# brudfors/UniRes

Hardware: AMD Instinct MI355X
Metric: cg_iters_per_sec (higher is better)
Workload: dtype f32; 1 GPU; cfg3_256c3_thick6z; channels=3, cg_iters_per_channel=20, cg_mode=fixed-iteration (tol=0), identity preconditioner, step=one y-update of one subject: C x (RHS + 20 CG iterations), channel_streams=True, channel_streams_setting=auto, parallelism=one subject per GPU, no data-path collective

## Files before the change

include/unires_hip.h:

```cpp
#ifndef UNIRES_HIP_H
#define UNIRES_HIP_H

#include <stdint.h>

#ifdef __cplusplus
extern "C" {
#endif

#define UNIRES_HIP_ABI_VERSION 1
#define UNIRES_MAX_TAPS 32

enum unires_status {
  UNIRES_OK = 0,
  UNIRES_ERR_NULL = 1,
  UNIRES_ERR_DIM = 2,
  UNIRES_ERR_ARG = 3,
  UNIRES_ERR_HIP = 4,
  UNIRES_ERR_ALLOC = 5,
  UNIRES_ERR_UNSUPPORTED = 6
};

enum unires_operator { UNIRES_OP_A = 0, UNIRES_OP_AT = 1, UNIRES_OP_ATA = 2 };

enum unires_regime {
  UNIRES_REGIME_IDENTITY = 0,
  UNIRES_REGIME_DENOISE = 1,
  UNIRES_REGIME_SUPERRES = 2
};

enum unires_cg_stop {
  UNIRES_STOP_RESIDUAL = 0,
  UNIRES_STOP_MAXGAIN = 1,
  UNIRES_STOP_MAXGAIN_RECURRED = 2,
  UNIRES_STOP_MAXGAIN_GUARDED = 3
};

enum unires_precond {
  UNIRES_PRECOND_IDENTITY = 0,
  UNIRES_PRECOND_JACOBI = 1,
  UNIRES_PRECOND_FFT = 2
};

const char *unires_last_error(void);
int unires_abi_version(void);


int unires_pull3d_affine(const float *src, const int32_t sdim[3], const float M[12], float *dst,
                         const int32_t gdim[3], float fov_tol, void *stream);

int unires_warp_label(const float *label, const int32_t ldim[3], const float M[12], float *dst,
                      const int32_t gdim[3], float fov_tol, void *stream);

int unires_pull3d_nearest(const float *src, const int32_t sdim[3], const float M[12], float *dst,
                          const int32_t gdim[3], float fov_tol, void *stream);

int unires_noise_hist(int32_t n_obs, const float *const *ptrs, const int64_t *sizes, const int32_t *ct,
                      uint32_t *counts, float *range, void *stream);

int unires_noise_fit(int32_t n_obs, const uint32_t *counts, const float *range, int32_t max_iter,
                     double *out, void *stream);

int unires_coreg_quantise(int32_t n_obs, const float *const *ptrs, const int64_t *sizes,
                          uint8_t *const *outs, uint32_t *counts, float *params, void *stream);

typedef struct {
  const uint8_t *G;
  const uint8_t *F;
  int32_t dim_g[3];
  int32_t dim_f[3];
  float M[12];
  float step[3];
} unires_coreg_job_t;

int unires_coreg_hist(int32_t n_jobs, const unires_coreg_job_t *jobs, uint64_t *hist, void *stream);

int unires_coreg_cost(int32_t n, const uint64_t *hist, int32_t cost_fun, double fwhm, double *work,
                      double *cost, void *stream);

int unires_pull_grad3d_affine(const float *src, const int32_t sdim[3], const float M[12],
                              float *dst3, const int32_t gdim[3], float fov_tol, void *stream);

int unires_push3d_affine(const float *src, const int32_t gdim[3], const float M[12], float *dst,
                         const int32_t ddim[3], float alpha, float fov_tol, int accumulate,
                         void *stream);

int unires_conv_down3d(const float *src, const int32_t sdim[3], const float *const taps[3],
                       const int32_t ntaps[3], const int32_t stride[3], float *dst,
                       const int32_t ddim[3], float scl, int32_t scl_dim, void *stream);

int unires_conv_up3d(const float *src, const int32_t sdim[3], const float *const taps[3],
                     const int32_t ntaps[3], const int32_t stride[3], float *dst,
                     const int32_t ddim[3], float scl, int32_t scl_dim, void *stream);

int unires_grad_fwd_zero(const float *src, const int32_t dim[3], const float vx[3], float *dst3,
                         void *stream);

int unires_div_fwd_zero(const float *src3, const int32_t dim[3], const float vx[3], float *dst,
                        void *stream);

int unires_dtd(const float *src, const int32_t dim[3], const float vx[3], float a, float c,
               float *dst, void *stream);

#define UNIRES_DIFF_FORWARD 0
#define UNIRES_DIFF_BACKWARD 1
#define UNIRES_DIFF_CENTRAL 2

int unires_grad_which(const float *src, const int32_t dim[3], const float vx[3], int32_t which,
                      float *dst3, void *stream);
int unires_div_which(const float *src3, const int32_t dim[3], const float vx[3], int32_t which,
                     float *dst, void *stream);
int unires_dtd_which(const float *src, const int32_t dim[3], const float vx[3], int32_t which, float a,
                     float c, float *dst, void *stream);


typedef struct unires_repeat {
  int32_t dim_x[3];
  int32_t dim_g[3];
  float M[12];
  int32_t ratio[3];
  int32_t ntaps[3];
  const float *taps[3];
  float scl;
  int32_t dim_thick;
  float tau;
} unires_repeat_t;

typedef struct unires_plan unires_plan_t;

int unires_plan_create(unires_plan_t **plan, const int32_t dim_y[3], const float vx_y[3],
                       int32_t regime, int32_t n_repeats, const unires_repeat_t *repeats,
                       float fov_tol);
int unires_plan_destroy(unires_plan_t *plan);
int unires_plan_set_repeat(unires_plan_t *plan, int32_t n, const unires_repeat_t *repeat);
int unires_plan_set_concurrency(unires_plan_t *plan, int32_t n_concurrent);
int unires_plan_set_diff(unires_plan_t *plan, int32_t which);
int unires_plan_set_missing(unires_plan_t *plan, int32_t n, const float *x, void *stream);
int unires_plan_set_slice_weights(unires_plan_t *plan, int32_t n, int32_t axis, const float *u_dev, void *stream);
int64_t unires_plan_workspace_bytes(const unires_plan_t *plan);
int unires_plan_repeat_info(const unires_plan_t *plan, int32_t n, int32_t info[8]);
int unires_orient_of(const float M[12], int32_t perm[3], int32_t flip[3]);
int unires_plan_time_matvecs(unires_plan_t *plan, int32_t on);
int unires_plan_matvec_time(unires_plan_t *plan, int32_t *launches, double *total_us);
int unires_plan_cg_ring(unires_plan_t *plan, int32_t k, int32_t *last);
int unires_plan_cg_ends(unires_plan_t *plan, int32_t *trimmed, int32_t *start_fused);

int unires_proj_apply(unires_plan_t *plan, int32_t n, int32_t op, const float *in, float *out,
                      void *stream);

int unires_ata_matvec(unires_plan_t *plan, float rho, float lam, const float *p, float *q,
                      double *dot_dev, void *stream);

int unires_rhs_assemble(unires_plan_t *plan, const float *const *x_ptrs, const float *w_c,
                        const float *z_c, float rho, float lam, float *b, void *stream);

int unires_atx_assemble(unires_plan_t *plan, const float *const *x_ptrs, float *atx,
                        void *stream);

int unires_rhs_from_atx(unires_plan_t *plan, const float *atx, const float *w_c,
                        const float *z_c, float rho, float lam, float *b, void *stream);

int unires_precond_build(unires_plan_t *plan, int32_t precond_mode, float rho, float lam,
                         float *m_out, void *stream);

int unires_precond_apply(unires_plan_t *plan, const float *in, float *out, void *stream);

int unires_cg_solve(unires_plan_t *plan, float rho, float lam, const float *b, float *x,
                    int32_t max_iter, double tol, int32_t stop_mode, int32_t precond_mode,
                    int32_t *iters_out, double *obj_trace, void *stream);

int unires_cg_solve_many(int32_t n, unires_plan_t *const *plans, const float *rho, const float *lam,
                         const float *const *b, float *const *x, int32_t max_iter, double tol,
                         int32_t stop_mode, int32_t precond_mode, int32_t *iters_out,
                         double *obj_trace, void *const *streams);


int unires_zw_update(const float *const *y_ptrs, const float *lam, int32_t n_channels,
                     const int32_t dim[3], const float vx[3], float rho, float alpha, float *z,
                     float *w, float *jtv, void *stream);

int unires_nll_prior(const float *const *y_ptrs, const float *lam, int32_t n_channels,
                     const int32_t dim[3], const float vx[3], double *out_dev, void *stream);

int unires_zw_update_which(const float *const *y_ptrs, const float *lam, int32_t n_channels,
                           const int32_t dim[3], const float vx[3], int32_t which, float rho, float alpha,
                           float *z, float *w, float *jtv, void *stream);
int unires_nll_prior_which(const float *const *y_ptrs, const float *lam, int32_t n_channels,
                           const int32_t dim[3], const float vx[3], int32_t which, double *out_dev,
                           void *stream);

int unires_masked_sse(const float *x, const float *ay, int64_t n, double *out_dev, void *stream);

int unires_slice_sums(const float *x, const float *ay, const int32_t dim[3], int32_t dim_thick, double *out_dev,
                      void *stream);

int unires_rigid_sums(const float *gr3, const float *diff, const float *ctc, const int32_t dim[3],
                      const float d_rigid[72], double *out_dev, void *stream);

int unires_clean_fov(float *y, const int32_t dim_y[3], const float M[12], const int32_t dim_x[3],
                     void *stream);

int unires_scaling_sums(const float *x, const float *ay, const int32_t dim[3], int32_t dim_thick,
                        double *out_dev, void *stream);

typedef struct unires_mark unires_mark_t;
int unires_mark_create(unires_mark_t **out);
int unires_mark_destroy(unires_mark_t *mark);
int unires_mark_signal(unires_mark_t *mark, uint64_t value, void *stream);
int unires_mark_read(const unires_mark_t *mark, uint64_t *value);

#ifdef __cplusplus
}
#endif
#endif
```

unires_amd/_lib.py:

```python
import ctypes as C
import os

_HERE = os.path.dirname(os.path.abspath(__file__))
LIB_PATH = os.environ.get('UNIRES_LIB') or os.path.join(_HERE, 'libunires_hip.so')

UNIRES_MAX_TAPS = 32
OP = {'A': 0, 'At': 1, 'AtA': 2}
REGIME_IDENTITY, REGIME_DENOISE, REGIME_SUPERRES = 0, 1, 2
STOP = {'e': 0, 'max_gain': 3, 'max_gain_guarded': 3, 'max_gain_fresh': 1, 'max_gain_recurred': 2}
PRECOND = {'none': 0, 'identity': 0, 'jacobi': 1, 'fft': 2}

c_i32x3 = C.c_int32 * 3
c_f32x3 = C.c_float * 3
c_f32x12 = C.c_float * 12
c_fptrx3 = C.POINTER(C.c_float) * 3


class Repeat(C.Structure):
    _fields_ = [('dim_x', c_i32x3), ('dim_g', c_i32x3), ('M', c_f32x12), ('ratio', c_i32x3),
                ('ntaps', c_i32x3), ('taps', c_fptrx3), ('scl', C.c_float),
                ('dim_thick', C.c_int32), ('tau', C.c_float)]


SIGNATURES = {
    'unires_last_error': (C.c_char_p, []),
    'unires_abi_version': (C.c_int, []),
    'unires_pull3d_affine': (C.c_int, [C.c_void_p, c_i32x3, c_f32x12, C.c_void_p, c_i32x3,
                                       C.c_float, C.c_void_p]),
    'unires_warp_label': (C.c_int, [C.c_void_p, c_i32x3, c_f32x12, C.c_void_p, c_i32x3,
                                    C.c_float, C.c_void_p]),
    'unires_pull3d_nearest': (C.c_int, [C.c_void_p, c_i32x3, c_f32x12, C.c_void_p, c_i32x3,
                                        C.c_float, C.c_void_p]),
    'unires_noise_hist': (C.c_int, [C.c_int32, C.POINTER(C.c_void_p), C.POINTER(C.c_int64),
                                    C.POINTER(C.c_int32), C.c_void_p, C.c_void_p, C.c_void_p]),
    'unires_noise_fit': (C.c_int, [C.c_int32, C.c_void_p, C.c_void_p, C.c_int32, C.c_void_p,
                                   C.c_void_p]),
    'unires_coreg_quantise': (C.c_int, [C.c_int32, C.POINTER(C.c_void_p), C.POINTER(C.c_int64),
                                        C.POINTER(C.c_void_p), C.c_void_p, C.c_void_p, C.c_void_p]),
    'unires_coreg_hist': (C.c_int, [C.c_int32, C.c_void_p, C.c_void_p, C.c_void_p]),
    'unires_coreg_cost': (C.c_int, [C.c_int32, C.c_void_p, C.c_int32, C.c_double, C.c_void_p,
                                    C.c_void_p, C.c_void_p]),
    'unires_pull_grad3d_affine': (C.c_int, [C.c_void_p, c_i32x3, c_f32x12, C.c_void_p, c_i32x3,
                                            C.c_float, C.c_void_p]),
    'unires_push3d_affine': (C.c_int, [C.c_void_p, c_i32x3, c_f32x12, C.c_void_p, c_i32x3,
                                       C.c_float, C.c_float, C.c_int, C.c_void_p]),
    'unires_conv_down3d': (C.c_int, [C.c_void_p, c_i32x3, c_fptrx3, c_i32x3, c_i32x3, C.c_void_p,
                                     c_i32x3, C.c_float, C.c_int32, C.c_void_p]),
    'unires_conv_up3d': (C.c_int, [C.c_void_p, c_i32x3, c_fptrx3, c_i32x3, c_i32x3, C.c_void_p,
                                   c_i32x3, C.c_float, C.c_int32, C.c_void_p]),
    'unires_grad_fwd_zero': (C.c_int, [C.c_void_p, c_i32x3, c_f32x3, C.c_void_p, C.c_void_p]),
    'unires_div_fwd_zero': (C.c_int, [C.c_void_p, c_i32x3, c_f32x3, C.c_void_p, C.c_void_p]),
    'unires_dtd': (C.c_int, [C.c_void_p, c_i32x3, c_f32x3, C.c_float, C.c_float, C.c_void_p,
                             C.c_void_p]),
    'unires_grad_which': (C.c_int, [C.c_void_p, c_i32x3, c_f32x3, C.c_int32, C.c_void_p, C.c_void_p]),
    'unires_div_which': (C.c_int, [C.c_void_p, c_i32x3, c_f32x3, C.c_int32, C.c_void_p, C.c_void_p]),
    'unires_dtd_which': (C.c_int, [C.c_void_p, c_i32x3, c_f32x3, C.c_int32, C.c_float, C.c_float, C.c_void_p,
                                   C.c_void_p]),
    'unires_plan_create': (C.c_int, [C.POINTER(C.c_void_p), c_i32x3, c_f32x3, C.c_int32,
                                     C.c_int32, C.POINTER(Repeat), C.c_float]),
    'unires_plan_destroy': (C.c_int, [C.c_void_p]),
    'unires_plan_set_repeat': (C.c_int, [C.c_void_p, C.c_int32, C.POINTER(Repeat)]),
    'unires_plan_set_concurrency': (C.c_int, [C.c_void_p, C.c_int32]),
    'unires_plan_set_diff': (C.c_int, [C.c_void_p, C.c_int32]),
    'unires_plan_set_missing': (C.c_int, [C.c_void_p, C.c_int32, C.c_void_p, C.c_void_p]),
    'unires_plan_set_slice_weights': (C.c_int, [C.c_void_p, C.c_int32, C.c_int32, C.c_void_p, C.c_void_p]),
    'unires_plan_workspace_bytes': (C.c_int64, [C.c_void_p]),
    'unires_orient_of': (C.c_int, [c_f32x12, c_i32x3, c_i32x3]),
    'unires_plan_repeat_info': (C.c_int, [C.c_void_p, C.c_int32, C.c_int32 * 8]),
    'unires_plan_time_matvecs': (C.c_int, [C.c_void_p, C.c_int32]),
    'unires_plan_matvec_time': (C.c_int, [C.c_void_p, C.POINTER(C.c_int32), C.POINTER(C.c_double)]),
    'unires_plan_cg_ring': (C.c_int, [C.c_void_p, C.c_int32, C.POINTER(C.c_int32)]),
    'unires_plan_cg_ends': (C.c_int, [C.c_void_p, C.POINTER(C.c_int32), C.POINTER(C.c_int32)]),
    'unires_proj_apply': (C.c_int, [C.c_void_p, C.c_int32, C.c_int32, C.c_void_p, C.c_void_p,
                                    C.c_void_p]),
    'unires_ata_matvec': (C.c_int, [C.c_void_p, C.c_float, C.c_float, C.c_void_p, C.c_void_p,
                                    C.c_void_p, C.c_void_p]),
    'unires_rhs_assemble': (C.c_int, [C.c_void_p, C.POINTER(C.c_void_p), C.c_void_p, C.c_void_p,
                                      C.c_float, C.c_float, C.c_void_p, C.c_void_p]),
    'unires_atx_assemble': (C.c_int, [C.c_void_p, C.POINTER(C.c_void_p), C.c_void_p, C.c_void_p]),
    'unires_rhs_from_atx': (C.c_int, [C.c_void_p, C.c_void_p, C.c_void_p, C.c_void_p, C.c_float,
                                      C.c_float, C.c_void_p, C.c_void_p]),
    'unires_precond_build': (C.c_int, [C.c_void_p, C.c_int32, C.c_float, C.c_float, C.c_void_p,
                                       C.c_void_p]),
    'unires_precond_apply': (C.c_int, [C.c_void_p, C.c_void_p, C.c_void_p, C.c_void_p]),
    'unires_cg_solve': (C.c_int, [C.c_void_p, C.c_float, C.c_float, C.c_void_p, C.c_void_p,
                                  C.c_int32, C.c_double, C.c_int32, C.c_int32,
                                  C.POINTER(C.c_int32), C.POINTER(C.c_double), C.c_void_p]),
    'unires_cg_solve_many': (C.c_int, [C.c_int32, C.POINTER(C.c_void_p), C.POINTER(C.c_float),
                                       C.POINTER(C.c_float), C.POINTER(C.c_void_p), C.POINTER(C.c_void_p),
                                       C.c_int32, C.c_double, C.c_int32, C.c_int32, C.POINTER(C.c_int32),
                                       C.POINTER(C.c_double), C.POINTER(C.c_void_p)]),
    'unires_zw_update': (C.c_int, [C.POINTER(C.c_void_p), C.POINTER(C.c_float), C.c_int32, c_i32x3,
                                   c_f32x3, C.c_float, C.c_float, C.c_void_p, C.c_void_p,
                                   C.c_void_p, C.c_void_p]),
    'unires_nll_prior': (C.c_int, [C.POINTER(C.c_void_p), C.POINTER(C.c_float), C.c_int32, c_i32x3,
                                   c_f32x3, C.c_void_p, C.c_void_p]),
    'unires_zw_update_which': (C.c_int, [C.POINTER(C.c_void_p), C.POINTER(C.c_float), C.c_int32, c_i32x3,
                                         c_f32x3, C.c_int32, C.c_float, C.c_float, C.c_void_p, C.c_void_p,
                                         C.c_void_p, C.c_void_p]),
    'unires_nll_prior_which': (C.c_int, [C.POINTER(C.c_void_p), C.POINTER(C.c_float), C.c_int32, c_i32x3,
                                         c_f32x3, C.c_int32, C.c_void_p, C.c_void_p]),
    'unires_scaling_sums': (C.c_int, [C.c_void_p, C.c_void_p, c_i32x3, C.c_int32, C.c_void_p,
                                      C.c_void_p]),
    'unires_rigid_sums': (C.c_int, [C.c_void_p, C.c_void_p, C.c_void_p, c_i32x3, C.c_float * 72,
                                    C.c_void_p, C.c_void_p]),
    'unires_clean_fov': (C.c_int, [C.c_void_p, c_i32x3, c_f32x12, c_i32x3, C.c_void_p]),
    'unires_masked_sse': (C.c_int, [C.c_void_p, C.c_void_p, C.c_int64, C.c_void_p, C.c_void_p]),
    'unires_slice_sums': (C.c_int, [C.c_void_p, C.c_void_p, c_i32x3, C.c_int32, C.c_void_p, C.c_void_p]),
    'unires_mark_create': (C.c_int, [C.POINTER(C.c_void_p)]),
    'unires_mark_destroy': (C.c_int, [C.c_void_p]),
    'unires_mark_signal': (C.c_int, [C.c_void_p, C.c_uint64, C.c_void_p]),
    'unires_mark_read': (C.c_int, [C.c_void_p, C.POINTER(C.c_uint64)]),
}

DIFF = {'forward': 0, 'backward': 1, 'central': 2}


def diff_code(which, arg='diff'):
    try:
        return DIFF[which]
    except (KeyError, TypeError):
        raise ValueError("%s must be 'forward', 'backward' or 'central', not %r" % (arg, which)) from None


_lib = None

_EXC = {1: ValueError, 2: ValueError, 3: ValueError, 4: RuntimeError, 5: MemoryError,
        6: NotImplementedError}


def load():
    global _lib
    if _lib is not None:
        return _lib
    if not os.path.exists(LIB_PATH):
        raise RuntimeError(
            'unires_amd: %s is missing. Build it with `python -c "import __graft_entry__ as g; '
            'g.build()"` (hipcc --offload-arch=gfx950). There is no CPU fallback.' % LIB_PATH)
    lib = C.CDLL(LIB_PATH)
    for name, (res, args) in SIGNATURES.items():
        fn = getattr(lib, name)
        fn.restype = res
        fn.argtypes = args
    if lib.unires_abi_version() != 1:
        raise RuntimeError('unires_amd: ABI version mismatch')
    _lib = lib
    return lib


def check(status):
    if status != 0:
        msg = load().unires_last_error().decode()
        raise _EXC.get(status, RuntimeError)(msg)


def i3(v):
    return c_i32x3(*[int(t) for t in v])


def f3(v):
    return c_f32x3(*[float(t) for t in v])


def f12(v):
    return c_f32x12(*[float(t) for t in v])
```

unires_amd/_plan.py:

```python
import ctypes as C

import numpy as np
import torch

from . import _lib
from ._lib import (REGIME_DENOISE, REGIME_IDENTITY, REGIME_SUPERRES, Repeat, check, f3, i3)
from ._ops import FOV_TOL, _ptr, _stream, _vol, on_device
from .spatial import _m12, voxel_size


def proj_matrix(po, method):
    if method == 'super-resolution':
        return torch.linalg.solve(po.mat_y, po.rigid.mm(po.mat_yx)), tuple(po.dim_yx)
    if method == 'denoising':
        return torch.linalg.solve(po.mat_y, po.rigid.mm(po.mat_x)), tuple(po.dim_x)
    raise ValueError('Undefined method')


def regime_of(method, do_proj):
    if method not in ('denoising', 'super-resolution'):
        raise ValueError('Undefined method')
    if not do_proj:
        return REGIME_IDENTITY
    return REGIME_SUPERRES if method == 'super-resolution' else REGIME_DENOISE


def _repeat_desc(po, tau, method, regime, keep):
    r = Repeat()
    r.tau = float(tau)
    if regime == REGIME_IDENTITY:
        return r
    mat, dim_g = proj_matrix(po, method)
    r.dim_x = i3(po.dim_x)
    r.dim_g = i3(dim_g)
    r.M = _lib.c_f32x12(*_m12(mat).tolist())
    if regime == REGIME_SUPERRES:
        taps = [np.ascontiguousarray(np.asarray(k, dtype=np.float32)) for k in po.smo_ker_1d]
        keep.extend(taps)
        r.ratio = i3(po.ratio)
        r.ntaps = i3([len(k) for k in taps])
        r.taps = _lib.c_fptrx3(*[k.ctypes.data_as(C.POINTER(C.c_float)) for k in taps])
        r.scl = float(po.scl)
        r.dim_thick = int(po.dim_thick)
    else:
        r.ratio = i3((1, 1, 1))
        r.ntaps = i3((1, 1, 1))
    return r


class ChannelPlan:

    def __init__(self, dim_y, vx_y, repeats, method, do_proj, fov_tol=FOV_TOL, device=None, diff='forward'):
        _lib.diff_code(diff, 'diff')
        self.lib = _lib.load()
        self.device = torch.device(device) if device is not None else torch.device('cuda', torch.cuda.current_device())
        if self.device.index is None:
            self.device = torch.device('cuda', torch.cuda.current_device())
        with torch.cuda.device(self.device):
            self._create(dim_y, vx_y, repeats, method, do_proj, fov_tol)
        self.set_diff(diff)

    def _create(self, dim_y, vx_y, repeats, method, do_proj, fov_tol):
        self.dim_y = tuple(int(d) for d in dim_y)
        self.regime = regime_of(method, do_proj)
        self.method = method
        self.n_repeats = len(repeats)
        keep = []
        arr = (Repeat * len(repeats))(*[_repeat_desc(po, tau, method, self.regime, keep)
                                       for po, tau in repeats])
        self._h = C.c_void_p()
        self._concurrency = 1
        self.diff = 'forward'
        self._missing = [None] * len(repeats)
        self.mask_zeros = False
        self._slice_w = [None] * len(repeats)
        self.weights = False
        check(self.lib.unires_plan_create(C.byref(self._h), i3(self.dim_y), f3(vx_y), self.regime,
                                          len(repeats), arr, fov_tol))
        self.dims_x = [self.dim_y if self.regime == REGIME_IDENTITY else tuple(po.dim_x)
                       for po, _ in repeats]

    def rhs_buffer(self, like):
        buf = getattr(self, '_rhs_buf', None)
        if buf is None or buf.shape != like.shape or buf.device != like.device:
            buf = torch.empty_like(like)
            self._rhs_buf = buf
        return buf

    def close(self):
        if getattr(self, '_h', None) is not None and self._h:
            try:
                with torch.cuda.device(self.device):
                    self.lib.unires_plan_destroy(self._h)
            except Exception:
                self.lib.unires_plan_destroy(self._h)
            self._h = None

    __del__ = close

    @property
    def workspace_bytes(self):
        return int(self.lib.unires_plan_workspace_bytes(self._h))

    def repeat_info(self, n):
        info = (C.c_int32 * 8)()
        check(self.lib.unires_plan_repeat_info(self._h, int(n), info))
        v = list(info)
        return dict(perm=tuple(v[:3]), flip=tuple((v[3] >> j) & 1 for j in range(3)), pull2=bool(v[4]),
                    splat2_axis=None if v[5] == 0 else v[5] - 2, shift=bool(v[6] & 1), separable=bool(v[7]),
                    fused=bool(v[6] & 2), masked=bool(v[6] & 4), weighted=bool(v[6] & 8))

    @on_device
    def time_matvecs(self, on=True):
        check(self.lib.unires_plan_time_matvecs(self._h, 2 if on == 2 else (1 if on else 0)))

    def cg_ring(self, k=0):
        last = C.c_int32(0)
        check(self.lib.unires_plan_cg_ring(self._h, int(k), C.byref(last)))
        return int(last.value)

    @on_device
    def matvec_time(self):
        n, us = C.c_int32(0), C.c_double(0.0)
        check(self.lib.unires_plan_matvec_time(self._h, C.byref(n), C.byref(us)))
        return int(n.value), float(us.value)

    @on_device
    def set_repeat(self, n, po, tau):
        keep = []
        r = _repeat_desc(po, tau, self.method, self.regime, keep)
        check(self.lib.unires_plan_set_repeat(self._h, n, C.byref(r)))

    @on_device
    def set_missing(self, n, dat):
        import weakref
        self._missing[n] = None
        if dat is None:
            check(self.lib.unires_plan_set_missing(self._h, int(n), None, _stream()))
            return
        d = _vol(dat, 'x')[0]
        if tuple(d.shape) != tuple(self.dims_x[n]):
            raise ValueError('unires_amd: observation shape mismatch')
        check(self.lib.unires_plan_set_missing(self._h, int(n), _ptr(d), _stream()))
        self._missing[n] = (weakref.ref(dat), dat._version)

    def sync_missing(self, x_dats):
        for n in range(self.n_repeats):
            if x_dats is None:
                if self._missing[n] is not None:
                    self.set_missing(n, None)
                continue
            t, key = x_dats[n], self._missing[n]
            if key is not None and key[0]() is t and key[1] == t._version:
                continue
            self.set_missing(n, t)

    @on_device
    def set_slice_weights(self, n, axis, w):
        import weakref
        n, axis = int(n), int(axis)
        if not 0 <= n < self.n_repeats:
            raise ValueError('unires_amd: repeat index out of range')
        if axis not in (0, 1, 2):
            raise ValueError('unires_amd: slice axis must be 0, 1 or 2')
        if w is not None and (not w.is_cuda or w.dtype != torch.float32
                              or tuple(w.shape) != (int(self.dims_x[n][axis]),)):
            raise ValueError('unires_amd: slice weights must be a float32 device tensor of shape (%d,)'
                             % int(self.dims_x[n][axis]))
        self._slice_w[n] = None
        self._atx = None
        if w is None:
            check(self.lib.unires_plan_set_slice_weights(self._h, n, axis, None, _stream()))
            return
        wc = w.contiguous()
        check(self.lib.unires_plan_set_slice_weights(self._h, int(n), axis, _ptr(wc), _stream()))
        self._slice_w[n] = (weakref.ref(w), w._version, axis)

    def sync_slice_weights(self, ws):
        for n in range(self.n_repeats):
            want = None if ws is None else ws[n]
            key = self._slice_w[n]
            if want is None:
                if key is not None:
                    self.set_slice_weights(n, key[2], None)
                continue
            axis, t = want
            if key is not None and key[0]() is t and key[1] == t._version and key[2] == int(axis):
                continue
            self.set_slice_weights(n, axis, t)

    def _slice_key(self):
        return tuple(None if k is None else (id(k[0]()), k[1]) for k in self._slice_w)

    def set_concurrency(self, n):
        n = max(1, int(n))
        if n != self._concurrency:
            check(self.lib.unires_plan_set_concurrency(self._h, n))
            self._concurrency = n

    def set_diff(self, diff):
        code = _lib.diff_code(diff, 'diff')
        if diff != self.diff:
            with torch.cuda.device(self.device):
                check(self.lib.unires_plan_set_diff(self._h, code))
            self.diff = diff

    def _y(self, t, name):
        v, _ = _vol(t, name)
        if tuple(v.shape) != self.dim_y:
            raise ValueError('unires_amd: %s has shape %s, expected %s'
                             % (name, tuple(v.shape), self.dim_y))
        return v

    @on_device
    def proj_apply(self, n, operator, dat):
        if operator not in _lib.OP:
            raise ValueError('Undefined operator')
        d, lead = _vol(dat)
        out_dim = self.dims_x[n] if operator == 'A' else self.dim_y
        in_dim = self.dims_x[n] if operator == 'At' else self.dim_y
        if tuple(d.shape) != tuple(in_dim):
            raise ValueError('unires_amd: input has shape %s, expected %s'
                             % (tuple(d.shape), tuple(in_dim)))
        out = torch.empty(out_dim, dtype=torch.float32, device=d.device)
        check(self.lib.unires_proj_apply(self._h, n, _lib.OP[operator], _ptr(d), _ptr(out),
                                         _stream()))
        return out.reshape(lead + tuple(out_dim))

    @on_device
    def matvec(self, p, rho, lam, out=None, dot=None):
        p = self._y(p, 'p')
        if out is None:
            out = torch.empty_like(p)
        check(self.lib.unires_ata_matvec(self._h, float(rho), float(lam), _ptr(p), _ptr(out),
                                         _ptr(dot) if dot is not None else None, _stream()))
        return out

    @on_device
    def rhs(self, x_dats, w_c, z_c, rho, lam, out=None):
        xs = [_vol(t, 'x')[0] for t in x_dats]
        for t, dx in zip(xs, self.dims_x):
            if tuple(t.shape) != tuple(dx):
                raise ValueError('unires_amd: observation shape mismatch')
        if len(xs) != self.n_repeats:
            raise ValueError('unires_amd: need one observation per repeat')
        for t in (w_c, z_c):
            if tuple(t.shape) != (3,) + self.dim_y or not t.is_cuda or t.dtype != torch.float32:
                raise ValueError('unires_amd: w/z must be (3,X,Y,Z) float32 device tensors')
        w_c, z_c = w_c.contiguous(), z_c.contiguous()
        if out is None:
            out = torch.empty(self.dim_y, dtype=torch.float32, device=w_c.device)
        ptrs = (C.c_void_p * len(xs))(*[t.data_ptr() for t in xs])
        check(self.lib.unires_rhs_assemble(self._h, ptrs, _ptr(w_c), _ptr(z_c), float(rho),
                                           float(lam), _ptr(out), _stream()))
        return out

    @on_device
    def rhs_cached(self, x_dats, w_c, z_c, rho, lam, out):
        xs = [_vol(t, 'x')[0] for t in x_dats]
        import weakref
        copied = any(v is not t and v.data_ptr() != t.data_ptr() for v, t in zip(xs, x_dats))
        key = None if copied else (tuple((id(t), t._version) for t in x_dats), self._slice_key())
        cache = getattr(self, '_atx', None)
        alive = cache is not None and all(r() is t for r, t in zip(cache[2], x_dats)) \
            and len(cache[2]) == len(x_dats)
        if cache is None or key is None or not alive or cache[0] != key:
            atx = cache[1] if cache is not None else torch.empty(self.dim_y, dtype=torch.float32,
                                                                 device=xs[0].device)
            ptrs = (C.c_void_p * len(xs))(*[t.data_ptr() for t in xs])
            check(self.lib.unires_atx_assemble(self._h, ptrs, _ptr(atx), _stream()))
            refs = [] if key is None else [weakref.ref(t) for t in x_dats]
            self._atx = cache = (key, atx, refs)
        w_c, z_c = w_c.contiguous(), z_c.contiguous()
        check(self.lib.unires_rhs_from_atx(self._h, _ptr(cache[1]), _ptr(w_c), _ptr(z_c),
                                           float(rho), float(lam), _ptr(out), _stream()))
        return out

    @on_device
    def precond_build(self, rho, lam, mode='jacobi', out=None):
        if mode not in _lib.PRECOND:
            raise ValueError('Undefined preconditioner')
        if out is not None:
            out = self._y(out, 'out')
        check(self.lib.unires_precond_build(self._h, _lib.PRECOND[mode], float(rho), float(lam),
                                            _ptr(out) if out is not None else None, _stream()))
        return out

    @on_device
    def precond_apply(self, v, out=None):
        v = self._y(v, 'v')
        if out is None:
            out = torch.empty_like(v)
        check(self.lib.unires_precond_apply(self._h, _ptr(v), _ptr(out), _stream()))
        return out

    @on_device
    def cg(self, b, x, rho, lam, max_iter=20, tolerance=1e-3, stop='max_gain', sync=True,
           precond='none'):
        if precond not in _lib.PRECOND:
            raise ValueError('Undefined preconditioner')
        pm = _lib.PRECOND[precond]
        b = self._y(b, 'b')
        if not x.is_contiguous():
            raise ValueError('unires_amd: cg updates x in place and needs it contiguous')
        self._y(x, 'x')
        s = stop if stop in _lib.STOP else stop[0].lower()
        mode = _lib.STOP[s] if s in _lib.STOP else (0 if s == 'e' else 3)
        max_iter = int(max_iter)
        if sync:
            it = C.c_int32(0)
            obj = (C.c_double * (min(max_iter, 4096) + 1))()
            check(self.lib.unires_cg_solve(self._h, float(rho), float(lam), _ptr(b), _ptr(x),
                                           int(max_iter), float(tolerance), mode, pm, C.byref(it),
                                           obj, _stream()))
            trace = _trace(list(obj), it.value) if tolerance else None
            return it.value, trace
        check(self.lib.unires_cg_solve(self._h, float(rho), float(lam), _ptr(b), _ptr(x),
                                       int(max_iter), float(tolerance), mode, pm, None, None,
                                       _stream()))
        return None


def _trace(ring, it):
    n = len(ring)
    if it < n:
        return ring[:it + 1]
    start = (it + 1) % n
    return ring[start:] + ring[:start]


def cg_many(plans, bs, xs, rho, lams, streams, max_iter=20, tolerance=1e-3, stop='max_gain', precond='none',
            sync=False):
    if precond not in _lib.PRECOND:
        raise ValueError('Undefined preconditioner')
    n = len(plans)
    lib = plans[0].lib
    s = stop if stop in _lib.STOP else stop[0].lower()
    mode = _lib.STOP[s] if s in _lib.STOP else (0 if s == 'e' else 3)
    for pl, b, x in zip(plans, bs, xs):
        pl._y(b, 'b')
        if not x.is_contiguous():
            raise ValueError('unires_amd: cg updates x in place and needs it contiguous')
        pl._y(x, 'x')
    max_iter = int(max_iter)
    nobj = min(max_iter, 4096) + 1
    it = (C.c_int32 * n)() if sync else None
    obj = (C.c_double * (n * nobj))() if sync else None
    with torch.cuda.device(plans[0].device):
        check(lib.unires_cg_solve_many(
            n, (C.c_void_p * n)(*[pl._h.value for pl in plans]), (C.c_float * n)(*[float(rho)] * n),
            (C.c_float * n)(*[float(v) for v in lams]), (C.c_void_p * n)(*[b.data_ptr() for b in bs]),
            (C.c_void_p * n)(*[x.data_ptr() for x in xs]), max_iter, float(tolerance), mode,
            _lib.PRECOND[precond], it, obj, (C.c_void_p * n)(*[st.cuda_stream for st in streams])))
    if not sync:
        return None
    return [(it[c], _trace(list(obj[c * nobj:(c + 1) * nobj]), it[c]) if tolerance else None) for c in range(n)]
```

unires_amd/csrc/api_cg.hip:

```cpp
#include <time.h>

#include <functional>

#include "api_internal.hpp"

using namespace unires;

static bool cg_start_fused_on() {
  static const bool on = !(getenv("UNIRES_CG_START_FUSED") && getenv("UNIRES_CG_START_FUSED")[0] == '0');
  return on;
}

static int cg_enqueue_start(unires_plan *pl, const CgSolve &s, unsigned long long *hostw, hipStream_t st) {
  const size_t ny = pl->dy.numel();
  const bool check = s.tol != 0.0;
  CgState *S = pl->state;
  const int gv = vec_num_blocks(ny);
  HIP_TRY(hipMemsetAsync(&S->done, 0, sizeof(int), st));
  const bool want_obj0 = check && s.stop != UNIRES_STOP_RESIDUAL;
  StartResidual res = {s.b, pl->r, pl->p, s.M, pl->part0, want_obj0 ? pl->part1 : nullptr, false};
  const bool ask = cg_start_fused_on() && !s.fft;
  int g0 = matvec(pl, s.rho, s.lam, s.x, pl->ap, nullptr, nullptr, st, nullptr, ask ? &res : nullptr);
  pl->last_fused = ask && res.served;
  if (!(ask && res.served)) {
    launch_residual_init(s.b, pl->ap, s.x, pl->r, pl->p, ny, pl->part0, want_obj0 ? pl->part1 : nullptr, s.M, st);
    g0 = gv;
  }
  if (s.fft) {
    if (fftpre_apply(pl->fft, pl->r, pl->fft.z, st)) return fail(UNIRES_ERR_HIP, "hipFFT execution failed");
    HIP_TRY(hipMemcpyAsync(pl->p, pl->fft.z, ny * sizeof(float), hipMemcpyDeviceToDevice, st));
    launch_dot(pl->r, pl->fft.z, ny, pl->part0, nullptr, st);
  }
  launch_sc_init(S, pl->part0, pl->part1, g0, s.stop, check ? 1 : 0, hostw, st);
  return UNIRES_OK;
}

static float *ring_slot(unires_plan *pl, int j) {
  return j == 0 ? pl->p : pl->ring + (size_t)(j - 1) * (align_up(pl->dy.numel() * 4) / 4);
}

static bool cg_trim_on() {
  static const bool on = !(getenv("UNIRES_CG_TRIM") && getenv("UNIRES_CG_TRIM")[0] == '0');
  return on;
}

static int cg_enqueue_iters(unires_plan *pl, const CgSolve &s, int k_first, int count, bool dev_k,
                            unsigned long long *hostw, hipStream_t st) {
  const size_t ny = pl->dy.numel();
  const bool check = s.tol != 0.0;
  const int ring = s.ring;
  CgState *S = pl->state;
  const int *done = &S->done;
  const int gv = vec_num_blocks(ny);
  if (ring > 1 && (check || s.fft || dev_k || ring > kMaxRing || ring - 1 > pl->ring_slots))
    return fail(UNIRES_ERR_ARG, "deferred iterate update outside its scope");
  const bool trim = cg_trim_on() && !check && !s.fft && !dev_k && k_first == 1 && count == s.max_iter;
  pl->last_trim = trim && count > 0;
  RingPtrs rp = {};
  for (int j = 0; j < ring && ring > 1; ++j) rp.p[j] = ring_slot(pl, j);
  for (int k = k_first; k < k_first + count; ++k) {
    const int kk = dev_k ? -1 : k;
    const int slot = ring > 1 ? (k - k_first) % ring : 0;
    float *p = ring > 1 ? ring_slot(pl, slot) : pl->p;
    hipEvent_t ev0 = nullptr, ev1 = nullptr;
    if (pl->timing && hipEventCreate(&ev0) == hipSuccess) {
      if (hipEventCreate(&ev1) == hipSuccess) {
        (void)hipEventRecord(ev0, st);
      } else {
        (void)hipEventDestroy(ev0);
        ev0 = nullptr;
      }
    }
    if (pl->twice) (void)matvec(pl, s.rho, s.lam, p, pl->ap, pl->part0, done, st);
    const int g = matvec(pl, s.rho, s.lam, p, pl->ap, pl->part0, done, st);
    if (ev0 && ev1) {
      (void)hipEventRecord(ev1, st);
      if (pl->tev.size() >= 65536) {
        (void)hipEventDestroy(pl->tev.front().first), (void)hipEventDestroy(pl->tev.front().second);
        pl->tev.erase(pl->tev.begin());
      }
      pl->tev.emplace_back(ev0, ev1);
    }
    const bool guarded = check && s.stop == UNIRES_STOP_MAXGAIN_GUARDED;
    const bool recur = check && (s.stop == UNIRES_STOP_MAXGAIN_RECURRED || guarded);
    int obj_kind = 0;
    if (check && s.stop == UNIRES_STOP_RESIDUAL) obj_kind = 1;
    if (recur) obj_kind = 2;
    const bool lazy_x = obj_kind == 0;
    if (trim && k == k_first + count - 1) {
      launch_sc_alpha(S, pl->part0, g, st, k);
      if (ring > 1)
        launch_update_x_flush(S, rp, slot + 1, ny, s.x, st);
      else
        launch_update_x(S, p, ny, s.x, st);
      break;
    }
    launch_sc_alpha(S, pl->part0, g, st);
    launch_update_xr(S, p, pl->ap, lazy_x ? nullptr : s.x, pl->r, s.b, ny, pl->part0,
                     recur ? pl->part1 : nullptr, s.M, st);
    if (s.fft) {
      if (fftpre_apply(pl->fft, pl->r, pl->fft.z, st)) return fail(UNIRES_ERR_HIP, "hipFFT execution failed");
      launch_dot(pl->r, pl->fft.z, ny, pl->part0, done, st);
    }
    if (guarded)
      launch_sc_beta_guarded(S, pl->part0, pl->part1, gv, kk, s.tol, hostw, st);
    else
      launch_sc_beta(S, pl->part0, pl->part1, gv, kk, obj_kind, s.tol, obj_kind ? hostw : nullptr, st);
    if (ring > 1 && (slot == ring - 1 || k == k_first + count - 1))
      launch_update_p_flush(S, pl->r, rp, slot + 1, ring_slot(pl, (slot + 1) % ring), ny, s.M, s.x, st);
    else if (ring > 1)
      launch_update_p_ring(S, pl->r, p, ring_slot(pl, slot + 1), slot, ny, s.M, st);
    else
      launch_update_p(S, s.fft ? pl->fft.z : pl->r, pl->p, ny, s.M, lazy_x ? s.x : nullptr, st);
    if (check && s.stop == UNIRES_STOP_MAXGAIN) {
      const int go = matvec(pl, s.rho, s.lam, s.x, pl->ax, pl->part1, done, st, s.b);
      launch_sc_obj(S, pl->part1, go, kk, s.tol, hostw, st);
    }
    if (guarded) {
      const int go = matvec(pl, s.rho, s.lam, s.x, pl->ax, pl->part1, &S->skip_fresh, st, s.b);
      launch_sc_obj_guarded(S, pl->part1, go, kk, s.tol, hostw, st);
    }
  }
  return UNIRES_OK;
}

static int cg_enqueue(unires_plan *pl, const CgSolve &s, hipStream_t st) {
  const int rc = cg_enqueue_start(pl, s, nullptr, st);
  if (rc) return rc;
  return cg_enqueue_iters(pl, s, 1, s.max_iter, false, nullptr, st);
}

static int cg_ring_prepare(unires_plan *pl, hipStream_t st) {
  static const int env_k = [] {
    const char *e = getenv("UNIRES_CG_RING");
    return e ? atoi(e) : 8;
  }();
  int want = pl->ring_req > 0 ? pl->ring_req : env_k;
  want = std::max(1, std::min(want, kMaxRing));
  if (want <= 1) return 1;
  if (!pl->ring_tried) {
    if (stream_capturing(st)) return 1;
    pl->ring_tried = true;
    const size_t slot = align_up(pl->dy.numel() * 4);
    size_t budget = 0;
    if (const char *e = getenv("UNIRES_CG_RING_MB")) {
      budget = (size_t)std::max(0.0, atof(e) * 1048576.0);
    } else {
      size_t free_b = 0, total_b = 0;
      if (hipMemGetInfo(&free_b, &total_b) == hipSuccess) budget = free_b / 8;
      (void)hipGetLastError();
    }
    const int n = (int)std::min<size_t>((size_t)(want - 1), budget / slot);
    if (n < 1) return 1;
    if (hipMalloc((void **)&pl->ring, (size_t)n * slot) != hipSuccess) {
      (void)hipGetLastError();
      pl->ring = nullptr;
      return 1;
    }
    pl->ring_slots = n;
  }
  return std::min(want, pl->ring_slots + 1);
}

struct CgRun {
  unires_plan *pl = nullptr;
  CgSolve s;
  hipStream_t st = nullptr;
  int enqueued = 0;
  unsigned gen = 0;
  bool finished = false;
  bool use_graph = false;
};

static void cg_resync_gen(unires_plan *pl) {
  (void)hipDeviceSynchronize();
  (void)hipGetLastError();
  unsigned g = pl->cg_gen;
  if (pl->state && hipMemcpy(&g, &pl->state->gen, sizeof(g), hipMemcpyDeviceToHost) == hipSuccess) pl->cg_gen = g;
  (void)hipGetLastError();
}

static int cg_chunk_env() {
  static const int v = [] {
    const char *e = getenv("UNIRES_CG_CHUNK");
    return e ? atoi(e) : 2;
  }();
  return v;
}
static int cg_chunk_size() { return std::max(1, std::min(cg_chunk_env(), 64)); }

static int capture_graph(hipStream_t st, hipGraphExec_t *exec, const std::function<int()> &body) {
  *exec = nullptr;
  if (hipStreamBeginCapture(st, hipStreamCaptureModeThreadLocal) != hipSuccess) {
    (void)hipGetLastError();
    return -1;
  }
  const int rc = body();
  hipGraph_t graph = nullptr;
  const hipError_t ce = hipStreamEndCapture(st, &graph);
  if (rc) {
    if (graph) (void)hipGraphDestroy(graph);
    return rc;
  }
  if (ce != hipSuccess || !graph) return fail(UNIRES_ERR_HIP, "hipStreamEndCapture failed");
  const hipError_t ge = hipGraphInstantiate(exec, graph, nullptr, nullptr, 0);
  (void)hipGraphDestroy(graph);
  if (ge != hipSuccess) {
    *exec = nullptr;
    return fail(UNIRES_ERR_HIP, "hipGraphInstantiate failed");
  }
  return UNIRES_OK;
}

static int cg_run_enqueue_chunk(CgRun &R) {
  unires_plan *pl = R.pl;
  const int n = std::min(R.s.chunk, R.s.max_iter - R.enqueued);
  if (n <= 0) return UNIRES_OK;
  if (R.use_graph && n == R.s.chunk && pl->cg_chunk_exec) {
    HIP_TRY(hipGraphLaunch(pl->cg_chunk_exec, R.st));
  } else {
    const int rc = cg_enqueue_iters(pl, R.s, R.enqueued + 1, n, true, pl->progress_dev, R.st);
    if (rc) return rc;
  }
  R.enqueued += n;
  return UNIRES_OK;
}

static int cg_run_start_impl(CgRun &R) {
  unires_plan *pl = R.pl;
  if (!pl->progress) {
    HIP_TRY(hipHostMalloc((void **)&pl->progress, 64, hipHostMallocMapped));
    *pl->progress = 0ull;
    HIP_TRY(hipHostGetDevicePointer((void **)&pl->progress_dev, (void *)pl->progress, 0));
  }
  R.gen = ++pl->cg_gen;
  R.enqueued = 0;
  R.finished = false;
  CgSolve key = R.s;
  key.max_iter = 0;
  key.pre = R.s.M ? UNIRES_PRECOND_JACOBI : UNIRES_PRECOND_IDENTITY;
  if (R.use_graph && !(pl->cg_start_exec && pl->cg_chunk_exec && pl->cg_chunk_key.same_graph(key))) {
    drop_cg_chunk_graphs(pl);
    int rc = capture_graph(R.st, &pl->cg_start_exec, [&] { return cg_enqueue_start(pl, R.s, pl->progress_dev, R.st); });
    if (rc > 0) return rc;
    if (rc == 0)
      rc = capture_graph(R.st, &pl->cg_chunk_exec, [&] {
        return cg_enqueue_iters(pl, R.s, 1, R.s.chunk, true, pl->progress_dev, R.st);
      });
    if (rc > 0) return rc;
    if (rc < 0 || !pl->cg_start_exec || !pl->cg_chunk_exec) {
      drop_cg_chunk_graphs(pl);
      R.use_graph = false;
    } else {
      pl->cg_chunk_key = key;
      pl->chunk_fused = pl->last_fused;
    }
  }
  pl->last_trim = 0;
  if (R.use_graph) {
    pl->last_fused = pl->chunk_fused;
    HIP_TRY(hipGraphLaunch(pl->cg_start_exec, R.st));
  } else {
    const int rc = cg_enqueue_start(pl, R.s, pl->progress_dev, R.st);
    if (rc) return rc;
  }
  int rc = cg_run_enqueue_chunk(R);
  if (!rc) rc = cg_run_enqueue_chunk(R);
  if (rc) return rc;
  if (R.enqueued >= R.s.max_iter) R.finished = true;
  pl->last_trim = 0;
  return UNIRES_OK;
}

static int cg_run_start(CgRun &R) {
  const int rc = cg_run_start_impl(R);
  if (rc) cg_resync_gen(R.pl);
  return rc;
}

static int cg_run_poll(CgRun &R) {
  if (R.finished) return UNIRES_OK;
  const unsigned long long w = __atomic_load_n(R.pl->progress, __ATOMIC_ACQUIRE);
  if ((unsigned)(w >> 32) != R.gen) return UNIRES_OK;
  if (w & 0x80000000ull) {
    R.finished = true;
    return UNIRES_OK;
  }
  const int iters = (int)(w & 0x7fffffffull);
  while (!R.finished && iters >= R.enqueued - R.s.chunk) {
    const int rc = cg_run_enqueue_chunk(R);
    if (rc) return rc;
    if (R.enqueued >= R.s.max_iter) R.finished = true;
  }
  return UNIRES_OK;
}

static int cg_runs_drive(std::vector<CgRun> &runs) {
  unsigned spins = 0;
  for (;;) {
    bool all = true;
    for (CgRun &R : runs) {
      if (R.finished) continue;
      const int rc = cg_run_poll(R);
      if (rc) return rc;
      all = all && R.finished;
    }
    if (all) return UNIRES_OK;
    if (++spins > 256) {
      const struct timespec nap = {0, 50000};
      (void)nanosleep(&nap, nullptr);
    }
    if ((spins <= 256 && (spins & 0xff) == 0) || (spins > 256 && (spins & 0x1ff) == 0)) {
      for (CgRun &R : runs) {
        if (R.finished) continue;
        const hipError_t q = hipStreamQuery(R.st);
        if (q == hipSuccess) {
          const int before = R.enqueued;
          const int rc = cg_run_poll(R);
          if (rc) return rc;
          if (!R.finished && R.enqueued == before)
            return fail(UNIRES_ERR_HIP, "chunked CG: the stream drained without the expected progress");
        } else if (q != hipErrorNotReady) {
          g_err = std::string("chunked CG: ") + hipGetErrorString(q);
          return UNIRES_ERR_HIP;
        }
      }
    }
  }
}

static int cg_check_args(unires_plan *plan, float rho, float lam, const float *b, float *x, int32_t max_iter,
                         double tol, int32_t stop_mode, int32_t precond_mode) {
  if (!plan || !b || !x) return fail(UNIRES_ERR_NULL, "null argument");
  if (b == x) return fail(UNIRES_ERR_ARG, "b and x must not alias");
  if (max_iter < 0) return fail(UNIRES_ERR_ARG, "max_iter out of range");
  if (max_iter > kMaxCgIter && !(tol > 0.0))
    return fail(UNIRES_ERR_ARG, "max_iter beyond 4096 needs a tolerance (the solve is then enqueued in chunks)");
  if (stop_mode < 0 || stop_mode > 3) return fail(UNIRES_ERR_ARG, "bad stop mode");
  if (precond_mode < UNIRES_PRECOND_IDENTITY || precond_mode > UNIRES_PRECOND_FFT)
    return fail(UNIRES_ERR_UNSUPPORTED, "preconditioner modes: identity (0), Jacobi (1), FFT (2)");
  if (precond_mode != UNIRES_PRECOND_IDENTITY &&
      (!plan->prec_ready || plan->prec_mode != precond_mode || plan->prec_rho != rho ||
       plan->prec_lam != lam))
    return fail(UNIRES_ERR_ARG, "call unires_precond_build with this mode, rho and lam first");
  if (!(tol >= 0.0)) return fail(UNIRES_ERR_ARG, "tolerance must be >= 0");
  return UNIRES_OK;
}

static bool cg_graphs_on() {
  static const bool on = !(getenv("UNIRES_CG_GRAPH") && getenv("UNIRES_CG_GRAPH")[0] == '0');
  return on;
}

static bool cg_chunked(double tol, int max_iter) {
  const bool off = cg_chunk_env() == 0;
  return tol != 0.0 && max_iter > 0 && (!off || max_iter > kMaxCgIter);
}

static CgSolve cg_describe(const unires_plan *pl, float rho, float lam, const float *b, float *x, int max_iter,
                           double tol, int stop_mode, int precond_mode) {
  CgSolve s;
  s.b = b, s.x = x, s.rho = rho, s.lam = lam, s.max_iter = max_iter, s.stop = stop_mode, s.pre = precond_mode;
  s.tol = tol;
  s.M = precond_mode == UNIRES_PRECOND_JACOBI ? pl->precM : nullptr;
  s.fft = precond_mode == UNIRES_PRECOND_FFT;
  return s;
}

static CgRun cg_make_run(unires_plan *pl, CgSolve s, hipStream_t st) {
  CgRun R;
  R.pl = pl, R.s = s, R.st = st;
  R.s.chunk = cg_chunk_size();
  R.use_graph = cg_graphs_on() && !s.fft && !pl->timing;
  return R;
}

static int cg_read_back(unires_plan *pl, int max_iter, double tol, int32_t *iters_out, double *obj_trace,
                        hipStream_t st) {
  CgState *S = pl->state;
  int it = 0;
  HIP_TRY(hipMemcpyAsync(&it, &S->iters, sizeof(int), hipMemcpyDeviceToHost, st));
  if (obj_trace && tol != 0.0)
    HIP_TRY(hipMemcpyAsync(obj_trace, S->obj, sizeof(double) * (size_t)(std::min(max_iter, kMaxCgIter) + 1),
                           hipMemcpyDeviceToHost, st));
  HIP_TRY(hipStreamSynchronize(st));
  *iters_out = it;
  return UNIRES_OK;
}

extern "C" int unires_cg_solve(unires_plan_t *plan, float rho, float lam, const float *b, float *x,
                               int32_t max_iter, double tol, int32_t stop_mode,
                               int32_t precond_mode, int32_t *iters_out, double *obj_trace,
                               void *stream) {
  int rc = cg_check_args(plan, rho, lam, b, x, max_iter, tol, stop_mode, precond_mode);
  if (rc) return rc;
  hipStream_t st = (hipStream_t)stream;
  unires_plan *pl = plan;
  CgSolve s = cg_describe(pl, rho, lam, b, x, max_iter, tol, stop_mode, precond_mode);
  mark_use(pl, st);

  if (stream_capturing(st) && tol != 0.0 && max_iter > kMaxCgIter)
    return fail(UNIRES_ERR_ARG, "a solve with a tolerance and more than 4096 iterations cannot join a stream capture "
                                "(it is fed to the device chunk by chunk, following its progress)");
  if (cg_chunked(tol, max_iter) && !(stream_capturing(st) && max_iter <= kMaxCgIter)) {
    pl->last_ring = 1;
    std::vector<CgRun> runs(1, cg_make_run(pl, s, st));
    if ((rc = cg_run_start(runs[0]))) return rc;
    if ((rc = cg_runs_drive(runs))) return rc;
    mark_use(pl, st);
    CHECK_LAUNCH();
    return iters_out ? cg_read_back(pl, max_iter, tol, iters_out, obj_trace, st) : UNIRES_OK;
  }
  ++pl->cg_gen;
  s.ring = tol == 0.0 && !s.fft && max_iter > 0 ? cg_ring_prepare(pl, st) : 1;
  pl->last_ring = s.ring;

  const bool graphable = cg_graphs_on() && !s.fft && max_iter > 0 && !pl->timing;
  if (graphable && pl->cg_exec && pl->cg_key.same_graph(s)) {
    pl->last_trim = pl->graph_trim, pl->last_fused = pl->graph_fused;
    HIP_TRY(hipGraphLaunch(pl->cg_exec, st));
  } else {
    if (graphable && pl->cg_exec) drop_cg_graph(pl);
    rc = graphable ? capture_graph(st, &pl->cg_exec, [&] { return cg_enqueue(pl, s, st); }) : -1;
    if (rc > 0) {
      cg_resync_gen(pl);
      return rc;
    }
    if (rc == 0) {
      pl->cg_key = s;
      pl->graph_trim = pl->last_trim, pl->graph_fused = pl->last_fused;
      if (hipGraphLaunch(pl->cg_exec, st) != hipSuccess) {
        cg_resync_gen(pl);
        return fail(UNIRES_ERR_HIP, "hipGraphLaunch failed");
      }
    } else if ((rc = cg_enqueue(pl, s, st))) {
      cg_resync_gen(pl);
      return rc;
    }
  }
  mark_use(pl, st);
  CHECK_LAUNCH();
  return iters_out ? cg_read_back(pl, max_iter, tol, iters_out, obj_trace, st) : UNIRES_OK;
}

extern "C" int unires_cg_solve_many(int32_t n, unires_plan_t *const *plans, const float *rho, const float *lam,
                                    const float *const *b, float *const *x, int32_t max_iter, double tol,
                                    int32_t stop_mode, int32_t precond_mode, int32_t *iters_out,
                                    double *obj_trace, void *const *streams) {
  if (n < 1 || !plans || !rho || !lam || !b || !x || !streams) return fail(UNIRES_ERR_NULL, "null argument");
  for (int c = 0; c < n; ++c) {
    const int rc = cg_check_args(plans[c], rho[c], lam[c], b[c], x[c], max_iter, tol, stop_mode, precond_mode);
    if (rc) return rc;
    for (int d = 0; d < c; ++d)
      if (plans[d] == plans[c]) return fail(UNIRES_ERR_ARG, "one plan per solve");
  }
  bool capturing = false;
  for (int c = 0; c < n; ++c) capturing = capturing || stream_capturing((hipStream_t)streams[c]);
  if (capturing && tol != 0.0 && max_iter > kMaxCgIter)
    return fail(UNIRES_ERR_ARG, "a solve with a tolerance and more than 4096 iterations cannot join a stream capture "
                                "(it is fed to the device chunk by chunk, following its progress)");
  for (int c = 0; c < n; ++c) mark_use(plans[c], (hipStream_t)streams[c]);
  if (!cg_chunked(tol, max_iter) || (capturing && max_iter <= kMaxCgIter)) {
    for (int c = 0; c < n; ++c) {
      const int rc = unires_cg_solve(plans[c], rho[c], lam[c], b[c], x[c], max_iter, tol, stop_mode, precond_mode,
                                     nullptr, nullptr, streams[c]);
      if (rc) return rc;
    }
  } else {
    std::vector<CgRun> runs;
    for (int c = 0; c < n; ++c) plans[c]->last_ring = 1;
    for (int c = 0; c < n; ++c)
      runs.push_back(cg_make_run(plans[c], cg_describe(plans[c], rho[c], lam[c], b[c], x[c], max_iter, tol, stop_mode,
                                                       precond_mode), (hipStream_t)streams[c]));
    for (CgRun &R : runs) {
      const int rc = cg_run_start(R);
      if (rc) return rc;
    }
    const int rc = cg_runs_drive(runs);
    if (rc) return rc;
    for (int c = 0; c < n; ++c) mark_use(plans[c], (hipStream_t)streams[c]);
    CHECK_LAUNCH();
  }
  if (iters_out)
    for (int c = 0; c < n; ++c) {
      const int rc = cg_read_back(plans[c], max_iter, tol, iters_out + c,
                                  obj_trace ? obj_trace + (size_t)c * (std::min(max_iter, kMaxCgIter) + 1) : nullptr,
                                  (hipStream_t)streams[c]);
      if (rc) return rc;
    }
  return UNIRES_OK;
}
```

unires_amd/csrc/api_internal.hpp:

```cpp
#pragma once
#include <math.h>
#include <stdlib.h>
#include <string.h>

#include <algorithm>
#include <string>
#include <utility>
#include <vector>

#include "../../include/unires_hip.h"
#include "ata1.hpp"
#include "cg.hpp"
#include "fftpre.hpp"
#include "fused.hpp"
#include "mask.hpp"
#include "orient.hpp"
#include "pull2.hpp"
#include "shift.hpp"
#include "slice.hpp"
#include "splat2.hpp"

namespace unires {

extern thread_local std::string g_err;

inline int fail(int code, const char *msg) {
  g_err = msg;
  return code;
}

#define HIP_TRY(expr)                                                               \
  do {                                                                              \
    hipError_t e_ = (expr);                                                         \
    if (e_ != hipSuccess) {                                                         \
      unires::g_err = std::string(#expr) + ": " + hipGetErrorString(e_);            \
      return UNIRES_ERR_HIP;                                                        \
    }                                                                               \
  } while (0)

#define CHECK_LAUNCH()                                                              \
  do {                                                                              \
    hipError_t e_ = hipGetLastError();                                              \
    if (e_ != hipSuccess) {                                                         \
      unires::g_err = std::string("kernel launch: ") + hipGetErrorString(e_);       \
      return UNIRES_ERR_HIP;                                                        \
    }                                                                               \
  } while (0)

inline bool dims_ok(const int32_t d[3]) {
  return d[0] > 0 && d[1] > 0 && d[2] > 0 && d[0] <= 65535 &&
         (long long)d[0] * d[1] * d[2] < (1ll << 40);
}
inline bool vx_ok(const float vx[3]) { return vx && vx[0] > 0 && vx[1] > 0 && vx[2] > 0; }
inline Dim3i mk(const int32_t d[3]) { return Dim3i{d[0], d[1], d[2]}; }
inline size_t align_up(size_t v) { return (v + 255) & ~(size_t)255; }

int make_taps(const float *const taps[3], const int32_t ntaps[3], const int32_t stride[3], Taps &T);
int check_conv_dims(const Dim3i &hi, const Dim3i &lo, const Taps &T);
bool invert_affine(const Affine &A, Affine &out);

inline Scaling make_scaling(float scl, int dim) {
  if (scl == 0.f) return kNoScaling;
  return Scaling{expf(scl), expf(-scl), dim};
}

enum class PushMode { kDefault, kTile, kNoSchedule };
inline PushMode push_mode() {
  static const PushMode mode = [] {
    const char *e = getenv("UNIRES_PUSH");
    return !e ? PushMode::kDefault : !strcmp(e, "tile") ? PushMode::kTile : PushMode::kNoSchedule;
  }();
  return mode;
}

struct RepeatDesc {
  Orient orient;
  bool oriented = false;
  Dim3i dim_xu;
  Dim3i dim_x, dim_g;
  Affine A;
  Taps T;
  float scl;
  int dim_thick;
  float tau;
  Dim3i dim_gf;
  Affine Af, Afinv;
  Taps Tf;
  SplatSafety safe;
  bool sep = false;
  bool sep0 = false;
  bool hyb = false;
  bool hybf = false;
  Taps Tz, Txy;
  Dim3i dim_h;
};

struct RepeatTables {
  SplatSched sched;
  float *ctab_dev[2] = {nullptr, nullptr};
  int ctab_n = 0, ctab_cap = 0;
  unsigned ctab_step = 1, src_stride = 1;
  float *xytab_dev[2] = {nullptr, nullptr};
  int xytab_cap[2] = {0, 0};
  PullPlan pplan;
  ShiftPlan shift;
  F1Sched f1;
};

struct RepeatMask {
  bool masked = false;
  uint8_t *mask_u = nullptr, *mask_c = nullptr;
  size_t mask_cap = 0;
};

struct RepeatWeights {
  bool weighted = false;
  float *w_dev = nullptr;
  int w_axis = 0;
  size_t w_cap = 0;
};

struct Repeat : RepeatDesc, RepeatTables, RepeatMask, RepeatWeights {
  const uint8_t *mask() const { return oriented ? mask_c : mask_u; }
  bool mid() const { return masked || weighted; }
  int w_caxis() const {
    for (int j = 0; j < 3; ++j)
      if (orient.perm[j] == w_axis) return j;
    return w_axis;
  }
  bool w_flip() const { return orient.flip[w_caxis()] != 0; }
};

struct CgSolve {
  const float *b = nullptr;
  float *x = nullptr;
  float rho = 0.f, lam = 0.f;
  int max_iter = -1, stop = -1, pre = -1;
  double tol = -1.0;
  int ring = 1;
  int chunk = 0;
  const float *M = nullptr;
  bool fft = false;
  bool same_graph(const CgSolve &o) const {
    return b == o.b && x == o.x && rho == o.rho && lam == o.lam && max_iter == o.max_iter && stop == o.stop &&
           pre == o.pre && ring == o.ring && chunk == o.chunk && tol == o.tol;
  }
};

}

struct unires_plan {
  unires::Dim3i dy;
  float vx[3];
  int regime;
  float fov_tol;
  int diff = UNIRES_DIFF_FORWARD;
  std::vector<unires::Repeat> reps;
  char *ws = nullptr;
  size_t ws_bytes = 0;
  float *r = nullptr, *p = nullptr, *ap = nullptr, *ax = nullptr;
  bool timing = false;
  bool twice = false;
  std::vector<std::pair<hipEvent_t, hipEvent_t>> tev;
  float *gbuf = nullptr;
  float *gbuf2 = nullptr;
  float *xbuf = nullptr;
  float *xperm = nullptr;
  double *part0 = nullptr, *part1 = nullptr;
  unires::CgState *state = nullptr;
  size_t cap_g = 0, cap_x = 0;
  unires::CgSolve cg_key;
  hipGraphExec_t cg_exec = nullptr;
  unires::CgSolve cg_chunk_key;
  hipGraphExec_t cg_start_exec = nullptr, cg_chunk_exec = nullptr;
  unsigned long long *progress = nullptr, *progress_dev = nullptr;
  unsigned cg_gen = 0;
  float *precM = nullptr;
  float *ring = nullptr;
  int ring_slots = 0;
  bool ring_tried = false;
  int ring_req = 0;
  int last_ring = 1;
  int last_trim = 0, last_fused = 0, graph_trim = 0, graph_fused = 0, chunk_fused = 0;
  unires::FftPre fft;
  float prec_rho = 0.f, prec_lam = 0.f;
  int prec_mode = UNIRES_PRECOND_IDENTITY;
  bool prec_ready = false;
  hipEvent_t last_use = nullptr;
  std::vector<hipStream_t> use_streams;
  bool captured_use = false;
  int concurrency = 1;
  int cap_s2 = 0, cap_f1 = 0;
};

namespace unires {

bool stream_capturing(hipStream_t st);
void mark_use(unires_plan *pl, hipStream_t st);
void await_use(unires_plan *pl);
void drop_cg_chunk_graphs(unires_plan *pl);
void drop_cg_graph(unires_plan *pl);

struct StartResidual {
  const float *b;
  float *r, *p;
  const float *M;
  double *partials;
  double *obj_partials;
  bool served;
};
int matvec(unires_plan *pl, float rho, float lam, const float *p, float *q, double *part, const int *done,
           hipStream_t st, const float *objb = nullptr, StartResidual *res = nullptr);

}
```

unires_amd/csrc/api_operator.hip:

```cpp
#include "aligned.hpp"
#include "api_internal.hpp"
#include "conv.hpp"
#include "pull.hpp"
#include "stencil.hpp"

using namespace unires;

static PushSrc push_src(const Repeat &R, const float *data, bool convup, float scl) {
  PushSrc src;
  src.data = data;
  src.convup = convup ? 1 : 0;
  src.xd = R.dim_x;
  src.gd = convup ? R.dim_gf : R.dim_g;
  src.T = R.Tf;
  src.S = make_scaling(scl, R.dim_thick);
  return src;
}

static Scaling scaling_z(const Scaling &S) { return S.dim == 2 ? S : kNoScaling; }
static Scaling scaling_xy(const Scaling &S) { return S.dim == 2 ? kNoScaling : S; }

static void forward(unires_plan *pl, const Repeat &R, const float *in, const Scaling &S, float *out,
                    const int *done, hipStream_t st) {
  if (pl->regime == UNIRES_REGIME_DENOISE) {
    if (launch_pull_conv2(R.pplan, in, pl->dy, R.A, R.T, kNoScaling, out, R.dim_g, R.dim_g, pl->fov_tol, done, st))
      launch_pull(in, pl->dy, R.A, out, R.dim_g, pl->fov_tol, done, st);
    return;
  }
  if ((R.hyb || R.hybf) && pl->gbuf2 && R.pplan.valid &&
      !launch_pull_conv2(R.pplan, in, pl->dy, R.Af, R.Tz, scaling_z(S), pl->gbuf, R.dim_h, R.dim_gf, pl->fov_tol,
                         done, st)) {
    launch_conv_down_sep(pl->gbuf, R.dim_h, R.Txy, scaling_xy(S), out, R.dim_x, pl->gbuf, pl->gbuf2, done, st);
    return;
  }
  if (R.sep && pl->gbuf2) {
    launch_pull(in, pl->dy, R.Af, pl->gbuf, R.dim_gf, pl->fov_tol, done, st);
    launch_conv_down_sep(pl->gbuf, R.dim_gf, R.Tf, S, out, R.dim_x, pl->gbuf, pl->gbuf2, done, st);
    return;
  }
  if (launch_pull_conv2(R.pplan, in, pl->dy, R.Af, R.Tf, S, out, R.dim_x, R.dim_gf, pl->fov_tol, done, st) &&
      launch_pull_conv(in, pl->dy, R.Af, R.Tf, S, out, R.dim_x, R.dim_gf, pl->fov_tol, done, st)) {
    launch_pull(in, pl->dy, R.A, pl->gbuf, R.dim_g, pl->fov_tol, done, st);
    launch_conv_down(pl->gbuf, R.dim_g, R.T, S, out, R.dim_x, done, st);
  }
}

static void mid_pass(const Repeat &R, float *buf, bool weights, const int *done, hipStream_t st) {
  if (R.weighted && weights)
    launch_slice_apply(buf, buf, R.masked ? R.mask() : nullptr, R.w_dev, R.dim_x, R.w_caxis(), R.w_flip(), done, st);
  else if (R.masked)
    launch_mask_apply(buf, R.mask(), R.dim_x.numel(), done, st);
}

static PushSrc ata_forward(unires_plan *pl, const Repeat &R, const float *in, const int *done,
                           hipStream_t st, bool weights = true) {
  if (pl->regime == UNIRES_REGIME_DENOISE) {
    forward(pl, R, in, kNoScaling, pl->gbuf, done, st);
    mid_pass(R, pl->gbuf, weights, done, st);
    return push_src(R, pl->gbuf, false, 0.f);
  }
  const Scaling S2 = make_scaling(2.f * R.scl, R.dim_thick);
  const bool fwd_only = R.hybf && !R.hyb && R.sep && !(R.sched.valid && R.sched.axis >= 0);
  const bool both = R.hyb && R.sched.valid && R.sched.axis == 2 && R.Tf.s[1] == 2;
  if (!R.mid() && push_mode() == PushMode::kDefault && (fwd_only || both) && pl->gbuf2 && R.pplan.valid && R.Tf.s[0] == 2 &&
      !(R.Tf.n[0] == 1)) {
    Taps Ty = R.Txy;
    set_dirac(Ty, 0);
    const Dim3i dxy = Dim3i{R.dim_h.x, R.dim_x.y, R.dim_x.z};
    const Scaling Sx = S2.dim == 0 ? S2 : kNoScaling, Srest = S2.dim == 0 ? kNoScaling : S2;
    const bool y_active = !is_dirac(Ty, 1) || Srest.dim == 1;
    if (y_active && !launch_pull_conv2(R.pplan, in, pl->dy, R.Af, R.Tz, scaling_z(Srest), pl->gbuf, R.dim_h, R.dim_gf,
                                       pl->fov_tol, done, st)) {
      const int gy = both ? R.dim_h.y : 0;
      if (!launch_conv_ydown_xdownup2(pl->gbuf, R.dim_h, R.Txy, scaling_xy(S2), R.dim_x.x, R.dim_x.y, gy, pl->gbuf2,
                                      done, st)) {
        PushSrc src = push_src(R, pl->gbuf2, true, 0.f);
        src.xd = both ? Dim3i{R.dim_h.x, R.dim_h.y, R.dim_x.z} : dxy;
        set_dirac(src.T, 0);
        if (both) set_dirac(src.T, 1);
        return src;
      }
      if (both && R.Tf.n[0] * R.Tf.n[1] <= 16) {
        launch_conv_down_sep(pl->gbuf, R.dim_h, R.Txy, scaling_xy(S2), pl->xbuf, R.dim_x, pl->gbuf, pl->gbuf2, done, st);
        return push_src(R, pl->xbuf, true, 0.f);
      }
      launch_conv_down_sep(pl->gbuf, R.dim_h, Ty, scaling_xy(Srest), pl->gbuf2, dxy, pl->gbuf, pl->gbuf2, done, st);
      if (!launch_conv_downup2(pl->gbuf2, dxy, R.Tf, Sx, 0, R.dim_x.x, pl->gbuf, done, st)) {
        PushSrc src = push_src(R, pl->gbuf, true, 0.f);
        src.xd = dxy;
        set_dirac(src.T, 0);
        return src;
      }
      Taps Tx = R.Txy;
      set_dirac(Tx, 1);
      launch_conv_down_sep(pl->gbuf2, dxy, Tx, Sx, pl->xbuf, R.dim_x, pl->gbuf, pl->gbuf, done, st);
      return push_src(R, pl->xbuf, true, 0.f);
    }
  }
  forward(pl, R, in, S2, pl->xbuf, done, st);
  mid_pass(R, pl->xbuf, weights, done, st);
  return push_src(R, pl->xbuf, true, 0.f);
}

static PushEpilogue without_residual(PushEpilogue ep) {
  if (ep.res_r) ep.partials = nullptr;
  ep.res_b = nullptr, ep.res_r = nullptr, ep.res_p = nullptr, ep.res_M = nullptr, ep.res_obj = nullptr;
  return ep;
}

static int push_any(unires_plan *pl, const PushSrc &src, const Repeat &R, float alpha,
                     const PushEpilogue &ep_in, float *out, const int *done, hipStream_t st, bool *served = nullptr) {
  const Affine &A = src.convup ? R.Af : R.A;
  const PushEpilogue ep = without_residual(ep_in);
  const PushEpilogue &ep2 = R.mid() ? ep : ep_in;
  const auto s2_done = [&] {
    if (served) *served = ep2.res_r != nullptr;
    return ep2.partials ? splat2_blocks(pl->dy, ep2.grid_cap) : 0;
  };
  if (served) *served = false;
  const bool use_tile = push_mode() == PushMode::kTile, sched_ok = push_mode() == PushMode::kDefault;
  if (sched_ok && R.hyb && src.convup && R.sched.valid && R.sched.axis == 2 && pl->gbuf2) {
    Taps Txy = src.T;
    set_dirac(Txy, 2);
    const Scaling Sxy = scaling_xy(src.S);
    const bool xy_done = Sxy.dim < 0 && is_dirac(Txy, 0) && is_dirac(Txy, 1);
    const float *h = xy_done ? src.data : launch_conv_up_sep(src.data, src.xd, Txy, Sxy, R.dim_h, pl->gbuf, pl->gbuf2, st);
    const float4 *tab = (const float4 *)R.ctab_dev[src.S.dim == 2 ? 1 : 0];
    if (!launch_splat2(R.sched, h, R.dim_h.numel(), tab, R.ctab_n, R.src_stride, R.ctab_step, R.src_stride,
                       R.ctab_step, A, alpha, ep2, out, pl->dy, done, st))
      return s2_done();
  }
  if (sched_ok && !R.hyb && R.sched.valid && (src.convup != 0) == (R.sched.axis >= 0)) {
    const float4 *tab = src.convup ? (const float4 *)R.ctab_dev[src.S.dim >= 0 ? 1 : 0] : nullptr;
    const size_t numel = src.convup ? src.xd.numel() : src.gd.numel();
    if (!launch_splat2(R.sched, src.data, numel, tab, R.ctab_n, R.src_stride, R.ctab_step, R.src_stride,
                       R.ctab_step, A, alpha, ep2, out, pl->dy, done, st))
      return s2_done();
  }
  if (!use_tile &&
      !launch_splat(src, A, R.Afinv, R.safe, alpha, pl->fov_tol, ep, out, pl->dy, done, st))
    return ep.partials ? splat_blocks(pl->dy, A) : 0;
  if (!use_tile && src.convup && R.sep && pl->gbuf2) {
    PushSrc d = src;
    d.data = launch_conv_up_sep(src.data, src.xd, src.T, src.S, src.gd, pl->gbuf, pl->gbuf2, st);
    d.convup = 0;
    if (sched_ok && R.sched.valid && R.sched.axis < 0 &&
        !launch_splat2(R.sched, d.data, d.gd.numel(), nullptr, 0, R.src_stride, 1, 0, 0, A, alpha, ep2, out,
                       pl->dy, done, st))
      return s2_done();
    if (!launch_splat(d, A, R.Afinv, R.safe, alpha, pl->fov_tol, ep, out, pl->dy, done, st))
      return ep.partials ? splat_blocks(pl->dy, A) : 0;
    (void)launch_push_tile(d, A, R.Afinv, R.safe, alpha, pl->fov_tol, ep, out, pl->dy, done, st);
    return ep.partials ? push_tile_blocks(pl->dy) : 0;
  }
  if (launch_push_tile(src, A, R.Afinv, R.safe, alpha, pl->fov_tol, ep, out, pl->dy, done, st)) {
    launch_conv_up(src.data, src.xd, src.T, src.S, pl->gbuf, src.gd, st);
    PushSrc d = src;
    d.data = pl->gbuf;
    d.convup = 0;
    (void)launch_push_tile(d, A, R.Afinv, R.safe, alpha, pl->fov_tol, ep, out, pl->dy, done, st);
  }
  return ep.partials ? push_tile_blocks(pl->dy) : 0;
}

static void at_accumulate(unires_plan *pl, const Repeat &R, const float *x, float *out, float alpha,
                          bool accumulate, hipStream_t st, bool weights = false) {
  if (pl->regime == UNIRES_REGIME_IDENTITY) {
    launch_axpy(alpha, x, out, pl->dy.numel(), st);
    return;
  }
  const bool w = weights && R.weighted;
  if (R.oriented) {
    launch_to_canonical(R.orient, x, R.dim_xu, pl->xperm, st);
    if (w) launch_slice_apply(pl->xperm, pl->xperm, nullptr, R.w_dev, R.dim_x, R.w_caxis(), R.w_flip(), nullptr, st);
    x = pl->xperm;
  } else if (w) {
    launch_slice_apply(x, pl->xperm, nullptr, R.w_dev, R.dim_x, R.w_axis, false, nullptr, st);
    x = pl->xperm;
  }
  PushEpilogue ep;
  ep.accumulate = accumulate ? 1 : 0;
  ep.grid_cap = pl->cap_s2;
  const bool sr = pl->regime == UNIRES_REGIME_SUPERRES;
  push_any(pl, push_src(R, x, sr, sr ? R.scl : 0.f), R, alpha, ep, out, nullptr, st);
}

static int ata_apply(unires_plan *pl, const Repeat &R, const float *in, float alpha, PushEpilogue ep, bool share,
                     float *out, const int *done, hipStream_t st, bool *served = nullptr, bool weights = true) {
  if (served) *served = false;
  if (pl->regime == UNIRES_REGIME_DENOISE && R.f1.valid && !R.mid()) {
    PushEpilogue e1 = without_residual(ep);
    e1.grid_cap = share ? pl->cap_f1 : 0;
    if (!launch_ata1(R.f1, in, R.Af, alpha, e1, out, pl->dy, done, st)) return e1.partials ? ata1_blocks(pl->dy, e1.grid_cap) : 0;
  }
  ep.grid_cap = share ? pl->cap_s2 : 0;
  const PushSrc src = ata_forward(pl, R, in, done, st, weights);
  return push_any(pl, src, R, alpha, ep, out, done, st, served);
}

extern "C" int unires_proj_apply(unires_plan_t *plan, int32_t n, int32_t op, const float *in,
                                 float *out, void *stream) {
  if (!plan || !in || !out) return fail(UNIRES_ERR_NULL, "null argument");
  if (n < 0 || n >= (int)plan->reps.size()) return fail(UNIRES_ERR_ARG, "repeat index");
  if (op != UNIRES_OP_A && op != UNIRES_OP_AT && op != UNIRES_OP_ATA)
    return fail(UNIRES_ERR_ARG, "Undefined operator");
  if (in == out) return fail(UNIRES_ERR_ARG, "proj_apply cannot run in place");
  hipStream_t st = (hipStream_t)stream;
  mark_use(plan, st);
  const Repeat &R = plan->reps[n];
  const size_t ny = plan->dy.numel();
  if (plan->regime == UNIRES_REGIME_IDENTITY) {
    HIP_TRY(hipMemcpyAsync(out, in, ny * sizeof(float), hipMemcpyDeviceToDevice, st));
    return UNIRES_OK;
  }
  if (op == UNIRES_OP_A) {
    forward(plan, R, in, make_scaling(R.scl, R.dim_thick), R.oriented ? plan->xperm : out, nullptr, st);
    if (R.oriented) launch_from_canonical(R.orient, plan->xperm, out, R.dim_xu, st);
  } else if (op == UNIRES_OP_AT) {
    at_accumulate(plan, R, in, out, 1.f, false, st);
  } else {
    ata_apply(plan, R, in, 1.f, PushEpilogue(), false, out, nullptr, st, nullptr, false);
  }
  CHECK_LAUNCH();
  return UNIRES_OK;
}

static bool no_aligned() {
  static const bool v = getenv("UNIRES_NO_ALIGNED") != nullptr;
  return v;
}

static int stencil_close(unires_plan *pl, float c, const float wr[3], const float wq[3], float a0, bool accumulate,
                         const float *p, float *q, double *part, const int *done, hipStream_t st, const float *objb) {
  static const bool no_flat = getenv("UNIRES_NO_FLAT") != nullptr;
  const bool fwd = !diff_nonforward(pl->diff);
  const float h = diff_dtd_scale(pl->diff);
  if (!(fwd && no_flat) && !launch_dtd_flat(pl->diff, accumulate, p, q, pl->dy, a0, wr[0] * h, wr[1] * h, wr[2] * h, part,
                                            objb, done, st))
    return part ? dtd_flat_blocks(pl->dy, pl->diff) : 0;
  if (fwd && !no_aligned() && !launch_dtd_lines(p, q, pl->dy, a0, wq[0], wq[1], wq[2], part, objb, done, st))
    return part ? aligned_blocks(pl->dy) : 0;
  launch_dtd(p, pl->dy, pl->vx, a0, c, q, part, objb, done, st, pl->diff, accumulate);
  return part ? dtd_num_blocks(pl->dy) : 0;
}

int unires::matvec(unires_plan *pl, float rho, float lam, const float *p, float *q, double *part, const int *done,
                   hipStream_t st, const float *objb, StartResidual *res) {
  if (res) res->served = false;
  const float c = rho * (lam * lam);
  float wr[3], wq[3];
  for (int d = 0; d < 3; ++d) {
    const float v2 = pl->vx[d] * pl->vx[d];
    wr[d] = c * (1.f / v2), wq[d] = c / v2;
  }
  if (pl->regime == UNIRES_REGIME_IDENTITY) {
    float a0 = 0.f;
    for (const Repeat &R : pl->reps) a0 += R.tau;
    return stencil_close(pl, c, wr, wq, a0, false, p, q, part, done, st, objb);
  }
  const bool fwd = !diff_nonforward(pl->diff);
  const float zero[3] = {0.f, 0.f, 0.f};
  const float *kw = fwd ? wr : zero;
  double *kpart = fwd ? part : nullptr;
  const float *kobjb = fwd ? objb : nullptr;
  const size_t nrep = pl->reps.size();
  const auto one_kernel = [&]() -> int {
    const Repeat &R = pl->reps[0];
    if (nrep != 1 || no_aligned() || R.mid()) return -1;
    const auto shift = [&] {
      return launch_ata_shift(R.shift, p, q, pl->dy, R.Af, R.tau, 0.f, kw[0], kw[1], kw[2], kpart, kobjb, done, st);
    };
    if (shift_fast(R.shift, pl->dy) && !shift()) return kpart ? shift_blocks(pl->dy) : 0;
    if (!launch_ata_aligned(p, q, pl->dy, R.dim_gf, R.dim_x, R.Tf, make_scaling(2.f * R.scl, R.dim_thick), R.Af, R.tau,
                            0.f, kw[0], kw[1], kw[2], kpart, kobjb, done, st))
      return kpart ? aligned_blocks(pl->dy) : 0;
    if (!shift()) return kpart ? shift_blocks(pl->dy) : 0;
    return -1;
  };
  const bool ask = res && fwd && !part && !objb;
  int npart = one_kernel();
  if (npart < 0) {
    npart = 0;
    for (size_t n = 0; n < nrep; ++n) {
      const Repeat &R = pl->reps[n];
      PushEpilogue ep;
      ep.accumulate = n > 0;
      if (fwd) {
        ep.p = p;
        if (n == 0) ep.cx = wq[0], ep.cy = wq[1], ep.cz = wq[2];
        if (n + 1 == nrep) ep.partials = part, ep.objb = objb;
        if (n + 1 == nrep && ask)
          ep.partials = res->partials, ep.res_obj = res->obj_partials, ep.res_b = res->b, ep.res_r = res->r,
          ep.res_p = res->p, ep.res_M = res->M;
      }
      npart = ata_apply(pl, R, p, R.tau, ep, true, q, done, st, n + 1 == nrep && ask ? &res->served : nullptr);
    }
  }
  return fwd ? npart : stencil_close(pl, c, wr, wq, 0.f, true, p, q, part, done, st, objb);
}

extern "C" int unires_ata_matvec(unires_plan_t *plan, float rho, float lam, const float *p,
                                 float *q, double *dot_dev, void *stream) {
  if (!plan || !p || !q) return fail(UNIRES_ERR_NULL, "null argument");
  if (p == q) return fail(UNIRES_ERR_ARG, "matvec cannot run in place");
  hipStream_t st = (hipStream_t)stream;
  mark_use(plan, st);
  const int g = matvec(plan, rho, lam, p, q, dot_dev ? plan->part0 : nullptr, nullptr, st);
  if (dot_dev) launch_sum_to(plan->part0, g, dot_dev, st);
  CHECK_LAUNCH();
  return UNIRES_OK;
}

extern "C" int unires_precond_build(unires_plan_t *plan, int32_t precond_mode, float rho,
                                    float lam, float *m_out, void *stream) {
  if (!plan) return fail(UNIRES_ERR_NULL, "null plan");
  if (precond_mode == UNIRES_PRECOND_IDENTITY) {
    plan->prec_ready = false;
    return UNIRES_OK;
  }
  if (plan->prec_ready && plan->prec_mode == precond_mode && plan->prec_rho == rho && plan->prec_lam == lam &&
      !m_out)
    return UNIRES_OK;
  if (precond_mode != UNIRES_PRECOND_JACOBI && precond_mode != UNIRES_PRECOND_FFT)
    return fail(UNIRES_ERR_UNSUPPORTED, "preconditioner modes: identity (0), Jacobi (1), FFT (2)");
  hipStream_t st = (hipStream_t)stream;
  mark_use(plan, st);
  const size_t ny = plan->dy.numel();
  if (precond_mode == UNIRES_PRECOND_FFT) {
    if (int rc = fftpre_setup(plan->fft, plan->dy, plan->diff))
      return fail(rc == 2 ? UNIRES_ERR_ALLOC : UNIRES_ERR_HIP, "hipFFT plan / buffer creation failed");
    FftPre &F = plan->fft;
    double a = 0.0;
    if (plan->regime == UNIRES_REGIME_IDENTITY) {
      for (const Repeat &R : plan->reps) a += R.tau;
    } else {
      launch_fill(1.f, plan->ax, ny, st);
      for (size_t n = 0; n < plan->reps.size(); ++n) {
        const Repeat &R = plan->reps[n];
        const PushSrc src = ata_forward(plan, R, plan->ax, nullptr, st);
        PushEpilogue ep;
        ep.accumulate = n > 0;
        push_any(plan, src, R, R.tau, ep, F.z, nullptr, st);
      }
      launch_dot(F.z, plan->ax, ny, plan->part0, nullptr, st);
      launch_sum_to(plan->part0, vec_num_blocks(ny), &plan->state->rz, st);
      HIP_TRY(hipMemcpyAsync(&a, &plan->state->rz, sizeof(double), hipMemcpyDeviceToHost, st));
      HIP_TRY(hipStreamSynchronize(st));
      a /= (double)ny;
    }
    if (!(a > 0.0)) return fail(UNIRES_ERR_ARG, "data term has an empty diagonal");
    F.a = (float)a;
    for (int d = 0; d < 3; ++d) F.c[d] = rho * (lam * lam) / (plan->vx[d] * plan->vx[d]);
    if (m_out) return fail(UNIRES_ERR_ARG, "m_out is only defined for the Jacobi diagonal");
    CHECK_LAUNCH();
    plan->prec_rho = rho, plan->prec_lam = lam, plan->prec_mode = precond_mode, plan->prec_ready = true;
    return UNIRES_OK;
  }
  if (plan->reps.size() != 1)
    return fail(UNIRES_ERR_ARG, "CG pre-conditioning only supports one repeat per contrast.");
  if (!plan->precM) HIP_TRY(hipMalloc((void **)&plan->precM, ny * sizeof(float)));
  const Repeat &R = plan->reps[0];
  float c = 0.f;
  for (int d = 0; d < 3; ++d) c += 1.f / (plan->vx[d] * plan->vx[d]);
  c = 2.f * rho * (lam * lam) * c;
  if (plan->regime == UNIRES_REGIME_IDENTITY) {
    launch_fill(R.tau + c, plan->precM, ny, st);
  } else {
    launch_fill(1.f, plan->ax, ny, st);
    const PushSrc src = ata_forward(plan, R, plan->ax, nullptr, st);
    push_any(plan, src, R, 1.f, PushEpilogue(), plan->precM, nullptr, st);
    launch_scale_shift(R.tau, c, plan->precM, ny, st);
  }
  if (m_out)
    HIP_TRY(hipMemcpyAsync(m_out, plan->precM, ny * sizeof(float), hipMemcpyDeviceToDevice, st));
  CHECK_LAUNCH();
  plan->prec_rho = rho, plan->prec_lam = lam, plan->prec_mode = precond_mode, plan->prec_ready = true;
  return UNIRES_OK;
}

extern "C" int unires_precond_apply(unires_plan_t *plan, const float *in, float *out, void *stream) {
  if (!plan || !in || !out) return fail(UNIRES_ERR_NULL, "null argument");
  if (in == out) return fail(UNIRES_ERR_ARG, "precond_apply cannot run in place");
  hipStream_t st = (hipStream_t)stream;
  mark_use(plan, st);
  const size_t ny = plan->dy.numel();
  if (!plan->prec_ready || plan->prec_mode == UNIRES_PRECOND_IDENTITY) {
    HIP_TRY(hipMemcpyAsync(out, in, ny * sizeof(float), hipMemcpyDeviceToDevice, st));
  } else if (plan->prec_mode == UNIRES_PRECOND_FFT) {
    if (fftpre_apply(plan->fft, in, out, st)) return fail(UNIRES_ERR_HIP, "hipFFT execution failed");
  } else {
    launch_div(in, plan->precM, out, ny, st);
  }
  CHECK_LAUNCH();
  return UNIRES_OK;
}

extern "C" int unires_rhs_assemble(unires_plan_t *plan, const float *const *x_ptrs,
                                   const float *w_c, const float *z_c, float rho, float lam,
                                   float *b, void *stream) {
  if (!plan || !x_ptrs || !w_c || !z_c || !b) return fail(UNIRES_ERR_NULL, "null argument");
  for (size_t n = 0; n < plan->reps.size(); ++n)
    if (!x_ptrs[n]) return fail(UNIRES_ERR_NULL, "null observation pointer");
  hipStream_t st = (hipStream_t)stream;
  mark_use(plan, st);
  launch_div(w_c, z_c, 1.f, -rho, plan->dy, plan->vx, -lam, nullptr, b, st, plan->diff);
  for (size_t n = 0; n < plan->reps.size(); ++n)
    at_accumulate(plan, plan->reps[n], x_ptrs[n], b, plan->reps[n].tau, true, st, true);
  CHECK_LAUNCH();
  return UNIRES_OK;
}

extern "C" int unires_atx_assemble(unires_plan_t *plan, const float *const *x_ptrs, float *atx,
                                   void *stream) {
  if (!plan || !x_ptrs || !atx) return fail(UNIRES_ERR_NULL, "null argument");
  for (size_t n = 0; n < plan->reps.size(); ++n)
    if (!x_ptrs[n]) return fail(UNIRES_ERR_NULL, "null observation pointer");
  hipStream_t st = (hipStream_t)stream;
  mark_use(plan, st);
  if (plan->regime == UNIRES_REGIME_IDENTITY)
// ... 17 lines not shown
```

unires_amd/csrc/api_plan.hip:

```cpp
#include <stdio.h>
#include <time.h>

#include <new>

#include "api_internal.hpp"

using namespace unires;

static void drop_timing(unires_plan *pl) {
  for (auto &e : pl->tev) (void)hipEventDestroy(e.first), (void)hipEventDestroy(e.second);
  pl->tev.clear();
}

bool unires::stream_capturing(hipStream_t st) {
  hipStreamCaptureStatus cs = hipStreamCaptureStatusNone;
  if (hipStreamIsCapturing(st, &cs) != hipSuccess) {
    (void)hipGetLastError();
    return false;
  }
  return cs != hipStreamCaptureStatusNone;
}

void unires::mark_use(unires_plan *pl, hipStream_t st) {
  if (stream_capturing(st)) {
// ... 148 lines not shown
  out.dim_thick = in->dim_thick;
  if (pl->regime == UNIRES_REGIME_IDENTITY) {
    out.dim_x = out.dim_xu = pl->dy;
    out.dim_g = pl->dy;
    return UNIRES_OK;
  }
  if (!dims_ok(in->dim_x) || !dims_ok(in->dim_g)) return fail(UNIRES_ERR_DIM, "bad repeat dims");
  out.dim_x = mk(in->dim_x);
  out.dim_g = mk(in->dim_g);
  memcpy(out.A.m, in->M, sizeof(out.A.m));
  for (int i = 0; i < 12; ++i)
    if (!isfinite(out.A.m[i])) return fail(UNIRES_ERR_ARG, "non-finite affine");
  if (pl->regime == UNIRES_REGIME_SUPERRES) {
    int rc = make_taps(in->taps, in->ntaps, in->ratio, out.T);
    if (rc) return rc;
    if ((rc = check_conv_dims(out.dim_g, out.dim_x, out.T))) return rc;
    if (out.scl != 0.f && (out.dim_thick < 0 || out.dim_thick > 2))
      return fail(UNIRES_ERR_ARG, "bad dim_thick");
  } else {
    if (out.dim_g.x != out.dim_x.x || out.dim_g.y != out.dim_x.y || out.dim_g.z != out.dim_x.z)
      return fail(UNIRES_ERR_DIM, "denoising regime needs dim_g == dim_x");
    for (int d = 0; d < 3; ++d) set_dirac(out.T, d);
  }
  out.dim_xu = out.dim_x;
  canonicalise(out);
  trim_taps(out.T, out.A, out.dim_g, out.Tf, out.Af, out.dim_gf);
  choose_family(pl, out, masked);
  if (!invert_affine(out.Af, out.Afinv)) return fail(UNIRES_ERR_ARG, "singular affine");
  splat_safety(out.Af, out.safe.row_sep, out.safe.use_atomics);
  return UNIRES_OK;
}

static int build_sched(unires_plan *pl, Repeat &R, bool tables_only = false) {
  const bool was_valid = R.sched.valid;
  R.sched.valid = false;
  if (pl->regime == UNIRES_REGIME_IDENTITY) return UNIRES_OK;
  int axis = -1;
  int rows_y = R.dim_gf.y;
  R.src_stride = (unsigned)R.dim_gf.z;
  R.ctab_step = 1;
  const bool direct = pl->regime == UNIRES_REGIME_DENOISE || R.sep;
  if (!direct) {
    int nconv = 0;
    for (int d = 0; d < 3; ++d) {
      if (is_dirac(R.Tf, d)) continue;
      ++nconv;
      axis = d;
    }
    const int xdv[3] = {R.dim_x.x, R.dim_x.y, R.dim_x.z}, gdv[3] = {R.dim_gf.x, R.dim_gf.y, R.dim_gf.z};
    if (R.dim_x.numel() >= (1ull << 30)) return UNIRES_OK;
    if (R.hyb) {
      axis = 2;
    } else if (nconv > 1) {
      for (int d = 0; d < 3; ++d)
        if (fan_in(R.Tf, d) > 2 || xdv[d] < 2) return UNIRES_OK;
      if (R.scl != 0.f && R.dim_thick != 2) return UNIRES_OK;
      axis = 3;
    } else {
      if (axis < 0) axis = 2;
      if (fan_in(R.Tf, axis) > 2 || xdv[axis] < 2) return UNIRES_OK;
      if (R.scl != 0.f && R.dim_thick != axis && !R.hyb) return UNIRES_OK;
    }
    const unsigned xyz = (unsigned)R.dim_x.y * (unsigned)R.dim_x.z, xz = (unsigned)R.dim_x.z;
    const int taxis = axis == 3 ? 2 : axis;
    if (axis == 2) rows_y = R.hyb ? R.dim_h.y : R.dim_x.y, R.src_stride = xz, R.ctab_step = 1;
    if (axis == 1) R.src_stride = xyz, R.ctab_step = xz;
    if (axis == 0) R.src_stride = xz, R.ctab_step = xyz;
    if (axis == 3) R.src_stride = xz, R.ctab_step = xyz;
    const int gn = gdv[taxis];
    if (gn + 128 > 1400) return UNIRES_OK;
    std::vector<float> host((size_t)gn * 4);
    for (int v = 0; v < 2; ++v) {
      if (!R.ctab_dev[v] || R.ctab_cap < gn) {
        if (R.ctab_dev[v]) (void)hipFree(R.ctab_dev[v]);
        R.ctab_dev[v] = nullptr;
        if (hipMalloc((void **)&R.ctab_dev[v], host.size() * sizeof(float)) != hipSuccess)
          return fail(UNIRES_ERR_ALLOC, "hipMalloc conv table");
      }
      splat2_convtab(R.Tf, v ? make_scaling(R.scl, R.dim_thick) : kNoScaling, taxis, gn, xdv[taxis], host.data());
      if (hipMemcpy(R.ctab_dev[v], host.data(), host.size() * sizeof(float), hipMemcpyHostToDevice) !=
          hipSuccess)
        return fail(UNIRES_ERR_HIP, "hipMemcpy conv table");
    }
    R.ctab_n = gn;
    R.ctab_cap = std::max(R.ctab_cap, gn);
    if (axis == 3) {
      for (int d = 0; d < 2; ++d) {
        std::vector<float> hx((size_t)gdv[d] * 4);
        if (!R.xytab_dev[d] || R.xytab_cap[d] < gdv[d]) {
          if (R.xytab_dev[d]) (void)hipFree(R.xytab_dev[d]);
          R.xytab_dev[d] = nullptr;
          if (hipMalloc((void **)&R.xytab_dev[d], hx.size() * sizeof(float)) != hipSuccess)
            return fail(UNIRES_ERR_ALLOC, "hipMalloc conv table");
          R.xytab_cap[d] = gdv[d];
        }
        splat2_convtab(R.Tf, kNoScaling, d, gdv[d], xdv[d], hx.data());
        if (hipMemcpy(R.xytab_dev[d], hx.data(), hx.size() * sizeof(float), hipMemcpyHostToDevice) != hipSuccess)
          return fail(UNIRES_ERR_HIP, "hipMemcpy conv table");
      }
    }
  }
  if (tables_only) {
    R.sched.valid = was_valid;
    return UNIRES_OK;
  }
  (void)splat2_build(R.sched, R.Af, R.Afinv, R.dim_gf, pl->dy, pl->fov_tol, R.safe, axis, rows_y,
                     (const float4 *)R.xytab_dev[0], (const float4 *)R.xytab_dev[1], R.dim_x);
  (void)hipGetLastError();
  return UNIRES_OK;
}

static void build_shift(unires_plan *pl, Repeat &R) {
  R.shift.valid = false;
  if (pl->reps.size() == 1 && pl->regime != UNIRES_REGIME_IDENTITY)
    (void)shift_build(R.shift, pl->dy, R.dim_gf, R.dim_x, R.Tf, make_scaling(2.f * R.scl, R.dim_thick), R.Af,
                      pl->fov_tol);
  (void)hipGetLastError();
}

static void build_pull(unires_plan *pl, Repeat &R) {
  R.pplan.valid = false;
  if (pl->regime == UNIRES_REGIME_DENOISE)
    (void)pull2_build(R.pplan, pl->dy, R.A, R.T, R.dim_g, R.dim_g, pl->fov_tol);
  else if (pl->regime == UNIRES_REGIME_SUPERRES && (R.hyb || R.hybf))
    (void)pull2_build(R.pplan, pl->dy, R.Af, R.Tz, R.dim_h, R.dim_gf, pl->fov_tol);
  else if (pl->regime == UNIRES_REGIME_SUPERRES && !R.sep)
    (void)pull2_build(R.pplan, pl->dy, R.Af, R.Tf, R.dim_x, R.dim_gf, pl->fov_tol);
  build_shift(pl, R);
}

static int build_repeat_kernels(unires_plan *pl, Repeat &R) {
  int rc = build_sched(pl, R);
  if (rc) return rc;
  build_pull(pl, R);
  R.f1.valid = false;
  if (pl->regime == UNIRES_REGIME_DENOISE) {
    (void)ata1_build(R.f1, R.Af, R.Afinv, R.dim_gf, pl->dy, pl->fov_tol, R.safe);
    (void)hipGetLastError();
  }
  if (R.hyb && !(R.pplan.valid && R.sched.valid && R.sched.axis == 2)) {
    R.hyb = false;
    R.sep = R.sep0;
    R.hybf = R.sep0 && R.pplan.valid;
    rc = build_sched(pl, R);
    if (rc) return rc;
    if (!R.hybf) build_pull(pl, R);
  }
  return UNIRES_OK;
}

static void free_tables(RepeatTables &R) {
  splat2_free(R.sched);
  pull2_free(R.pplan);
  shift_free(R.shift);
  ata1_free(R.f1);
  for (int v = 0; v < 2; ++v) {
    if (R.ctab_dev[v]) (void)hipFree(R.ctab_dev[v]), R.ctab_dev[v] = nullptr;
    if (R.xytab_dev[v]) (void)hipFree(R.xytab_dev[v]), R.xytab_dev[v] = nullptr;
    R.xytab_cap[v] = 0;
  }
  R.ctab_n = R.ctab_cap = 0;
}

static void free_mask(RepeatMask &R) {
  if (R.mask_u) (void)hipFree(R.mask_u);
  if (R.mask_c) (void)hipFree(R.mask_c);
  R.mask_u = R.mask_c = nullptr;
  R.mask_cap = 0, R.masked = false;
}

static void free_weights(RepeatWeights &R) {
  if (R.w_dev) (void)hipFree(R.w_dev);
  R.w_dev = nullptr;
  R.w_cap = 0, R.weighted = false;
}

static int canonical_mask(Repeat &R, hipStream_t st) {
  if (!R.masked || !R.oriented) return UNIRES_OK;
  if (!R.mask_c && hipMalloc((void **)&R.mask_c, R.mask_cap) != hipSuccess) {
    R.mask_c = nullptr;
    return fail(UNIRES_ERR_ALLOC, "hipMalloc mask");
  }
  launch_mask_permute(R.mask_u, R.orient, R.dim_xu, R.mask_c, st);
  return UNIRES_OK;
}

extern "C" int unires_plan_create(unires_plan_t **plan, const int32_t dim_y[3],
                                  const float vx_y[3], int32_t regime, int32_t n_repeats,
                                  const unires_repeat_t *repeats, float fov_tol) {
  if (!plan || !dim_y) return fail(UNIRES_ERR_NULL, "null argument");
  *plan = nullptr;
  if (!dims_ok(dim_y)) return fail(UNIRES_ERR_DIM, "bad dim_y");
  if (!vx_ok(vx_y)) return fail(UNIRES_ERR_ARG, "voxel size must be positive");
  if (regime < 0 || regime > 2) return fail(UNIRES_ERR_ARG, "Undefined method");
  if (n_repeats < 1 || !repeats) return fail(UNIRES_ERR_ARG, "need at least one repeat");
  unires_plan *pl = new (std::nothrow) unires_plan();
  if (!pl) return fail(UNIRES_ERR_ALLOC, "host allocation failed");
  pl->dy = mk(dim_y);
  memcpy(pl->vx, vx_y, sizeof(pl->vx));
  pl->regime = regime;
  pl->fov_tol = fov_tol;
  pl->reps.resize(n_repeats);
  bool need_sep = false;
  for (int n = 0; n < n_repeats; ++n) {
    if (int rc = fill_repeat(pl, &repeats[n], pl->reps[n])) {
      unires_plan_destroy(pl);
      return rc;
    }
    if (regime != UNIRES_REGIME_IDENTITY) {
      pl->cap_g = std::max(pl->cap_g, pl->reps[n].dim_g.numel());
      pl->cap_x = std::max(pl->cap_x, pl->reps[n].dim_x.numel());
    }
    need_sep = need_sep || (regime == UNIRES_REGIME_SUPERRES && (pl->reps[n].sep || pl->reps[n].hyb));
  }
  const size_t ny = pl->dy.numel();
  size_t off = 0;
  auto carve = [&](size_t bytes) {
    size_t o = off;
    off += align_up(bytes);
    return o;
  };
  const size_t o_r = carve(ny * 4), o_p = carve(ny * 4), o_ap = carve(ny * 4), o_ax = carve(ny * 4);
  const size_t o_g = carve(pl->cap_g * 4), o_x = carve(pl->cap_x * 4), o_xp = carve(pl->cap_x * 4);
  const size_t o_g2 = carve(need_sep ? pl->cap_g * 4 : 0);
  const size_t o_p0 = carve(kMaxPartials * 8), o_p1 = carve(kMaxPartials * 8);
  const size_t o_st = carve(sizeof(CgState));
  pl->ws_bytes = off;
  hipError_t e = hipMalloc((void **)&pl->ws, pl->ws_bytes);
  if (e != hipSuccess) {
    g_err = std::string("hipMalloc workspace: ") + hipGetErrorString(e);
    pl->ws = nullptr;
    unires_plan_destroy(pl);
    return UNIRES_ERR_ALLOC;
  }
  pl->r = (float *)(pl->ws + o_r);
  pl->p = (float *)(pl->ws + o_p);
  pl->ap = (float *)(pl->ws + o_ap);
  pl->ax = (float *)(pl->ws + o_ax);
  pl->gbuf = (float *)(pl->ws + o_g);
  pl->xbuf = (float *)(pl->ws + o_x);
  pl->xperm = (float *)(pl->ws + o_xp);
  pl->gbuf2 = need_sep ? (float *)(pl->ws + o_g2) : nullptr;
  pl->part0 = (double *)(pl->ws + o_p0);
  pl->part1 = (double *)(pl->ws + o_p1);
  pl->state = (CgState *)(pl->ws + o_st);
  e = hipMemset(pl->state, 0, sizeof(CgState));
  if (e != hipSuccess) {
    g_err = std::string("hipMemset: ") + hipGetErrorString(e);
    unires_plan_destroy(pl);
    return UNIRES_ERR_HIP;
  }
  for (Repeat &R : pl->reps)
    if (int rc = build_repeat_kernels(pl, R)) {
      unires_plan_destroy(pl);
      return rc;
    }
  *plan = pl;
  return UNIRES_OK;
}

extern "C" int unires_plan_destroy(unires_plan_t *plan) {
  if (!plan) return UNIRES_OK;
  if (plan->ws) (void)hipFree(plan->ws);
  if (plan->precM) (void)hipFree(plan->precM);
  if (plan->ring) (void)hipFree(plan->ring);
  if (plan->cg_exec) (void)hipGraphExecDestroy(plan->cg_exec);
  if (plan->cg_start_exec) (void)hipGraphExecDestroy(plan->cg_start_exec);
  if (plan->cg_chunk_exec) (void)hipGraphExecDestroy(plan->cg_chunk_exec);
  if (plan->progress) (void)hipHostFree(plan->progress);
  if (plan->last_use) (void)hipEventDestroy(plan->last_use);
  drop_timing(plan);
  fftpre_destroy(plan->fft);
  for (Repeat &R : plan->reps) free_tables(R), free_mask(R), free_weights(R);
  delete plan;
  return UNIRES_OK;
}

extern "C" int unires_plan_time_matvecs(unires_plan_t *plan, int32_t on) {
  if (!plan) return fail(UNIRES_ERR_NULL, "null argument");
  const bool twice = on == 2;
  if (twice != plan->twice) drop_cg_graph(plan);
  plan->twice = twice;
  plan->timing = on == 1;
  if (!plan->timing) drop_timing(plan);
  return UNIRES_OK;
}

extern "C" int unires_plan_cg_ring(unires_plan_t *plan, int32_t k, int32_t *last) {
  if (!plan) return fail(UNIRES_ERR_NULL, "null argument");
  if (k < 0) return fail(UNIRES_ERR_ARG, "ring size must be >= 0");
  if (k > 0) {
    const int v = std::min<int>(k, kMaxRing);
    if (v != plan->ring_req) drop_cg_graph(plan);
    plan->ring_req = v;
  }
  if (last) *last = plan->last_ring;
  return UNIRES_OK;
}

extern "C" int unires_plan_cg_ends(unires_plan_t *plan, int32_t *trimmed, int32_t *start_fused) {
  if (!plan) return fail(UNIRES_ERR_NULL, "null argument");
  if (trimmed) *trimmed = plan->last_trim;
  if (start_fused) *start_fused = plan->last_fused;
  return UNIRES_OK;
}

extern "C" int unires_plan_matvec_time(unires_plan_t *plan, int32_t *launches, double *total_us) {
  if (!plan || !launches || !total_us) return fail(UNIRES_ERR_NULL, "null argument");
  *launches = 0, *total_us = 0.0;
  for (auto &e : plan->tev) {
    float ms = 0.f;
    HIP_TRY(hipEventSynchronize(e.second));
    HIP_TRY(hipEventElapsedTime(&ms, e.first, e.second));
    *total_us += 1e3 * (double)ms;
    ++*launches;
  }
  drop_timing(plan);
  return UNIRES_OK;
}

static bool same_but_scaling(const RepeatDesc &a, const RepeatDesc &b) {
  auto taps_equal = [](const Taps &p, const Taps &q) {
    for (int d = 0; d < 3; ++d) {
      if (p.n[d] != q.n[d] || p.s[d] != q.s[d]) return false;
      for (int t = 0; t < p.n[d]; ++t)
        if (p.t[d][t] != q.t[d][t]) return false;
    }
    return true;
  };
  return !memcmp(&a.A, &b.A, sizeof(Affine)) && taps_equal(a.T, b.T) && !memcmp(&a.Af, &b.Af, sizeof(Affine)) &&
         taps_equal(a.Tf, b.Tf) && !memcmp(&a.dim_x, &b.dim_x, sizeof(Dim3i)) &&
         !memcmp(&a.dim_g, &b.dim_g, sizeof(Dim3i)) && !memcmp(&a.dim_gf, &b.dim_gf, sizeof(Dim3i)) &&
         !memcmp(&a.dim_xu, &b.dim_xu, sizeof(Dim3i)) && !memcmp(&a.orient, &b.orient, sizeof(Orient)) &&
         a.oriented == b.oriented && a.dim_thick == b.dim_thick && (a.scl != 0.f) == (b.scl != 0.f) &&
         a.sep0 == b.sep0;
}

extern "C" int unires_plan_set_repeat(unires_plan_t *plan, int32_t n,
                                      const unires_repeat_t *repeat) {
  if (!plan || !repeat) return fail(UNIRES_ERR_NULL, "null argument");
  if (n < 0 || n >= (int)plan->reps.size()) return fail(UNIRES_ERR_ARG, "repeat index");
  RepeatDesc tmp;
  int rc = fill_repeat(plan, repeat, tmp, plan->reps[n].mid());
  if (rc) return rc;
  if (plan->reps[n].masked && memcmp(&tmp.dim_xu, &plan->reps[n].dim_xu, sizeof(Dim3i)))
    return fail(UNIRES_ERR_DIM, "a masked repeat keeps its observation's dims (clear the mask first)");
  if (plan->reps[n].weighted && memcmp(&tmp.dim_xu, &plan->reps[n].dim_xu, sizeof(Dim3i)))
    return fail(UNIRES_ERR_DIM, "a weighted repeat keeps its observation's dims (clear the weights first)");
  if (plan->regime != UNIRES_REGIME_IDENTITY &&
      (tmp.dim_g.numel() > plan->cap_g || tmp.dim_x.numel() > plan->cap_x))
    return fail(UNIRES_ERR_DIM, "new repeat exceeds the plan's workspace");
  if (plan->regime == UNIRES_REGIME_SUPERRES && (tmp.sep || tmp.hyb) && !plan->gbuf2)
    return fail(UNIRES_ERR_DIM, "new repeat needs the separable-conv scratch the plan was built without");
  await_use(plan);
  drop_cg_graph(plan);
  plan->prec_ready = false;
  Repeat &R = plan->reps[n];
  static const bool no_fast = getenv("UNIRES_SET_REPEAT_FULL") != nullptr;
  const bool same = !no_fast && same_but_scaling(tmp, R);
  static const bool verbose = getenv("UNIRES_SET_REPEAT_VERBOSE") != nullptr;
  if (verbose) fprintf(stderr, "[set_repeat] %s (scl %g -> %g)\n", same ? "scaling only" : "full rebuild", (double)R.scl, (double)tmp.scl);
  if (same) {
    R.scl = tmp.scl, R.tau = tmp.tau;
    rc = build_sched(plan, R, true);
    if (!rc) build_shift(plan, R);
    return rc;
  }
  static_cast<RepeatDesc &>(R) = tmp;
  R.ctab_n = 0;
  sched_set_thorough(false);
  rc = build_repeat_kernels(plan, R);
  sched_set_thorough(true);
  if (!rc && R.masked && R.oriented) {
    rc = canonical_mask(R, nullptr);
    if (!rc) HIP_TRY(hipStreamSynchronize(nullptr));
  }
  return rc;
}

static int refamily(unires_plan *pl, Repeat &R) {
  const bool hyb = R.hyb, hybf = R.hybf, sep = R.sep;
  choose_family(pl, R, R.mid());
  if (hyb == R.hyb && hybf == R.hybf && sep == R.sep) return UNIRES_OK;
  R.ctab_n = 0;
  return build_repeat_kernels(pl, R);
}

extern "C" int unires_plan_set_missing(unires_plan_t *plan, int32_t n, const float *x, void *stream) {
  if (!plan) return fail(UNIRES_ERR_NULL, "null plan");
  if (n < 0 || n >= (int)plan->reps.size()) return fail(UNIRES_ERR_ARG, "repeat index");
  if (plan->regime == UNIRES_REGIME_IDENTITY)
    return fail(UNIRES_ERR_UNSUPPORTED,
                "regime A = I has no x-space intermediate to mask: build the plan in the denoising regime with the "
                "identity affine");
  Repeat &R = plan->reps[n];
  if (!x && !R.masked) return UNIRES_OK;
  hipStream_t st = (hipStream_t)stream;
  await_use(plan);
  drop_cg_graph(plan);
  plan->prec_ready = false;
  const bool was = R.masked, was_mid = R.mid();
  if (x) {
    const size_t nx = R.dim_xu.numel();
    if (R.mask_cap < nx) {
      free_mask(R);
      if (was_mid != R.mid()) (void)refamily(plan, R);
      if (hipMalloc((void **)&R.mask_u, nx) != hipSuccess) {
        R.mask_u = nullptr;
        return fail(UNIRES_ERR_ALLOC, "hipMalloc mask");
      }
      R.mask_cap = nx;
    }
    if (R.oriented && !R.mask_c && hipMalloc((void **)&R.mask_c, R.mask_cap) != hipSuccess) {
      R.mask_c = nullptr;
      return fail(UNIRES_ERR_ALLOC, "hipMalloc mask");
    }
    mark_use(plan, st);
    launch_mask_build(x, Orient(), R.dim_xu, R.mask_u, st);
    R.masked = true;
    (void)canonical_mask(R, st);
  } else {
    R.masked = false;
  }
  if (was_mid != R.mid()) {
    if (int rc = refamily(plan, R)) {
      R.masked = was;
      (void)refamily(plan, R);
      return rc;
    }
  }
  CHECK_LAUNCH();
  return UNIRES_OK;
}

extern "C" int unires_plan_set_slice_weights(unires_plan_t *plan, int32_t n, int32_t axis, const float *u_dev,
                                             void *stream) {
  if (!plan) return fail(UNIRES_ERR_NULL, "null plan");
  if (n < 0 || n >= (int)plan->reps.size()) return fail(UNIRES_ERR_ARG, "repeat index");
  if (axis < 0 || axis > 2) return fail(UNIRES_ERR_ARG, "slice axis: 0, 1 or 2");
  if (plan->regime == UNIRES_REGIME_IDENTITY)
    return fail(UNIRES_ERR_UNSUPPORTED,
                "regime A = I has no x-space intermediate to weight: build the plan in the denoising regime with the "
                "identity affine");
  Repeat &R = plan->reps[n];
  if (!u_dev && !R.weighted) return UNIRES_OK;
  hipStream_t st = (hipStream_t)stream;
  const bool was = R.weighted, was_mid = R.mid();
  const int was_axis = R.w_axis;
  const bool values_only = u_dev && was && axis == R.w_axis;
  plan->prec_ready = false;
  if (!values_only) {
    await_use(plan);
    drop_cg_graph(plan);
  }
  if (u_dev) {
    const int du[3] = {R.dim_xu.x, R.dim_xu.y, R.dim_xu.z};
    const size_t cap = (size_t)std::max(du[0], std::max(du[1], du[2]));
    if (R.w_cap < cap) {
      if (R.w_dev) (void)hipFree(R.w_dev);
      R.w_dev = nullptr, R.w_cap = 0;
      if (hipMalloc((void **)&R.w_dev, cap * sizeof(float)) != hipSuccess) {
        R.w_dev = nullptr;
        return fail(UNIRES_ERR_ALLOC, "hipMalloc slice weights");
      }
      R.w_cap = cap;
    }
    mark_use(plan, st);
    HIP_TRY(hipMemcpyAsync(R.w_dev, u_dev, (size_t)du[axis] * sizeof(float), hipMemcpyDeviceToDevice, st));
    R.weighted = true, R.w_axis = axis;
  } else {
    R.weighted = false;
  }
  if (was_mid != R.mid()) {
    if (int rc = refamily(plan, R)) {
      R.weighted = was, R.w_axis = was_axis;
      (void)refamily(plan, R);
      return rc;
    }
  }
  return UNIRES_OK;
}

extern "C" int unires_plan_set_concurrency(unires_plan_t *plan, int32_t n_concurrent) {
  if (!plan) return fail(UNIRES_ERR_NULL, "null argument");
  if (n_concurrent < 1 || n_concurrent > 64) return fail(UNIRES_ERR_ARG, "concurrency out of range (1 .. 64)");
  if (n_concurrent == plan->concurrency) return UNIRES_OK;
  int cap_s2 = 0, cap_f1 = 0;
  if (n_concurrent > 1 && plan->dy.numel() <= (1ull << 25)) {
    int dev = 0, ncu = 0;
    HIP_TRY(hipGetDevice(&dev));
    HIP_TRY(hipDeviceGetAttribute(&ncu, hipDeviceAttributeMultiprocessorCount, dev));
    static const int s2_16 = getenv("UNIRES_SHARE_S2") ? atoi(getenv("UNIRES_SHARE_S2")) : 28;
    static const int f1_16 = getenv("UNIRES_SHARE_F1") ? atoi(getenv("UNIRES_SHARE_F1")) : 48;
    cap_s2 = std::max(8, ncu * s2_16 / 16 / 8 * 8);
    cap_f1 = std::max(8, ncu * f1_16 / 16 / 8 * 8);
  }
  if (cap_s2 != plan->cap_s2 || cap_f1 != plan->cap_f1) drop_cg_graph(plan);
  plan->concurrency = n_concurrent, plan->cap_s2 = cap_s2, plan->cap_f1 = cap_f1;
  return UNIRES_OK;
}

extern "C" int unires_plan_set_diff(unires_plan_t *plan, int32_t which) {
  if (!plan) return fail(UNIRES_ERR_NULL, "null argument");
  if (!diff_ok(which)) return fail(UNIRES_ERR_ARG, "which: forward (0), backward (1) or central (2)");
  if (which == plan->diff) return UNIRES_OK;
  await_use(plan);
  drop_cg_graph(plan);
  plan->prec_ready = false;
  plan->diff = which;
  return UNIRES_OK;
}

extern "C" int64_t unires_plan_workspace_bytes(const unires_plan_t *plan) {
  return plan ? (int64_t)plan->ws_bytes : 0;
}

extern "C" int unires_orient_of(const float M[12], int32_t perm[3], int32_t flip[3]) {
  if (!M || !perm || !flip) return fail(UNIRES_ERR_NULL, "null argument");
  Affine A;
  memcpy(A.m, M, sizeof(A.m));
  for (int i = 0; i < 12; ++i)
    if (!isfinite(A.m[i])) return fail(UNIRES_ERR_ARG, "non-finite affine");
  const Orient O = orient_of(A);
  for (int j = 0; j < 3; ++j) perm[j] = O.perm[j], flip[j] = O.flip[j];
  return UNIRES_OK;
}

extern "C" int unires_plan_repeat_info(const unires_plan_t *plan, int32_t n, int32_t info[8]) {
  if (!plan || !info) return fail(UNIRES_ERR_NULL, "null argument");
  if (n < 0 || n >= (int)plan->reps.size()) return fail(UNIRES_ERR_ARG, "repeat index");
  const Repeat &R = plan->reps[n];
  const bool id = plan->regime == UNIRES_REGIME_IDENTITY;
  for (int j = 0; j < 3; ++j) info[j] = id ? j : R.orient.perm[j];
  info[3] = id ? 0 : (R.orient.flip[0] | (R.orient.flip[1] << 1) | (R.orient.flip[2] << 2));
  info[4] = R.pplan.valid ? 1 : 0;
  info[5] = R.sched.valid ? 2 + R.sched.axis : 0;
  info[6] = (R.shift.valid && !R.mid() ? 1 : 0) | (R.f1.valid && !R.mid() ? 2 : 0) | (R.masked ? 4 : 0) |
            (R.weighted ? 8 : 0);
  info[7] = R.sep ? 1 : 0;
  return UNIRES_OK;
}
```

unires_amd/csrc/cg.hip:

```cpp
#include "cg.hpp"

namespace unires {

static inline int vec_blocks(size_t n) {
  size_t b = (n / 4 + kBlock - 1) / kBlock;
  if (b < 1) b = 1;
  const size_t cap = 4096;
  return (int)(b < cap ? b : cap);
}

#define GRID_STRIDE_VEC4(n)                                                   \
  const size_t n4 = (n) / 4;                                                  \
  const size_t stride = (size_t)gridDim.x * blockDim.x;                       \
  const size_t tid0 = (size_t)blockIdx.x * blockDim.x + threadIdx.x

__device__ __forceinline__ float4 ld4(const float *p, size_t i) {
  return reinterpret_cast<const float4 *>(p)[i];
}
__device__ __forceinline__ void st4(float *p, size_t i, float4 v) {
  reinterpret_cast<float4 *>(p)[i] = v;
}
typedef float f4v __attribute__((ext_vector_type(4)));
__device__ __forceinline__ float4 ld4_stream(const float *p, size_t i) {
#ifdef UNIRES_CG_X_PLAIN
  return ld4(p, i);
#else
  const f4v v = __builtin_nontemporal_load(reinterpret_cast<const f4v *>(p) + i);
  return make_float4(v.x, v.y, v.z, v.w);
#endif
}
__device__ __forceinline__ void st4_stream(float *p, size_t i, float4 v) {
#ifdef UNIRES_CG_X_PLAIN
  st4(p, i, v);
#else
  __builtin_nontemporal_store(f4v{v.x, v.y, v.z, v.w}, reinterpret_cast<f4v *>(p) + i);
#endif
}


__device__ __forceinline__ float4 zval4(float4 r, const float *__restrict__ M, size_t i) {
  if (!M) return r;
  const float4 m = ld4(M, i);
  return make_float4(__fdiv_rn(r.x, m.x), __fdiv_rn(r.y, m.y), __fdiv_rn(r.z, m.z),
                     __fdiv_rn(r.w, m.w));
}
__device__ __forceinline__ float zval1(float r, const float *__restrict__ M, size_t i) {
  return M ? __fdiv_rn(r, M[i]) : r;
}

__global__ void __launch_bounds__(kBlock)
    k_residual_init(const float *__restrict__ b, const float *__restrict__ ax,
                    const float *__restrict__ x, float *__restrict__ r, float *__restrict__ p,
                    size_t n, double *__restrict__ part_rr, double *__restrict__ part_obj,
                    const float *__restrict__ M) {
  GRID_STRIDE_VEC4(n);
  double rr = 0.0, ob = 0.0;
  for (size_t i = tid0; i < n4; i += stride) {
    const float4 vb = ld4(b, i), va = ld4(ax, i);
    float4 vr;
    vr.x = __fsub_rn(vb.x, va.x);
    vr.y = __fsub_rn(vb.y, va.y);
    vr.z = __fsub_rn(vb.z, va.z);
    vr.w = __fsub_rn(vb.w, va.w);
    st4(r, i, vr);
    const float4 vz = zval4(vr, M, i);
    st4(p, i, vz);
    rr += (double)__fmul_rn(vr.x, vz.x) + (double)__fmul_rn(vr.y, vz.y) +
          (double)__fmul_rn(vr.z, vz.z) + (double)__fmul_rn(vr.w, vz.w);
    if (part_obj) {
      const float4 vx = ld4(x, i);
      ob += (double)obj_term(va.x, vb.x, vx.x) + (double)obj_term(va.y, vb.y, vx.y) +
            (double)obj_term(va.z, vb.z, vx.z) + (double)obj_term(va.w, vb.w, vx.w);
    }
  }
  for (size_t i = n4 * 4 + tid0; i < n; i += stride) {
    const float vr = __fsub_rn(b[i], ax[i]);
    r[i] = vr;
    const float vz = zval1(vr, M, i);
    p[i] = vz;
    rr += (double)__fmul_rn(vr, vz);
    if (part_obj) ob += (double)obj_term(ax[i], b[i], x[i]);
  }
  const double t = block_sum(rr);
  if (threadIdx.x == 0) part_rr[blockIdx.x] = t;
  if (part_obj) {
    const double t2 = block_sum(ob);
    if (threadIdx.x == 0) part_obj[blockIdx.x] = t2;
  }
}

__global__ void __launch_bounds__(kBlock)
    k_dot(const float *__restrict__ a, const float *__restrict__ b, size_t n,
          double *__restrict__ part, const int *__restrict__ done) {
  if (done && *done) return;
  GRID_STRIDE_VEC4(n);
  double acc = 0.0;
  for (size_t i = tid0; i < n4; i += stride) {
    const float4 va = ld4(a, i), vb = ld4(b, i);
    acc += (double)__fmul_rn(va.x, vb.x) + (double)__fmul_rn(va.y, vb.y) +
           (double)__fmul_rn(va.z, vb.z) + (double)__fmul_rn(va.w, vb.w);
  }
  for (size_t i = n4 * 4 + tid0; i < n; i += stride) acc += (double)__fmul_rn(a[i], b[i]);
  const double t = block_sum(acc);
  if (threadIdx.x == 0) part[blockIdx.x] = t;
}

template <bool XUPD>
__global__ void __launch_bounds__(kBlock)
    k_update_xr(const CgState *__restrict__ st, const float *__restrict__ p,
                const float *__restrict__ ap, float *__restrict__ x, float *__restrict__ r,
                const float *__restrict__ b, size_t n, double *__restrict__ part_rr,
                double *__restrict__ part_obj, const float *__restrict__ M) {
  if (st->done) return;
  const float alpha = (float)st->alpha;
  GRID_STRIDE_VEC4(n);
  double rr = 0.0, ob = 0.0;
  for (size_t i = tid0; i < n4; i += stride) {
    const float4 va = ld4(ap, i);
    float4 vx = make_float4(0.f, 0.f, 0.f, 0.f), vr = ld4(r, i);
    if (XUPD) {
      const float4 vp = ld4(p, i);
      vx = ld4(x, i);
      vx.x = __fadd_rn(vx.x, __fmul_rn(alpha, vp.x));
      vx.y = __fadd_rn(vx.y, __fmul_rn(alpha, vp.y));
      vx.z = __fadd_rn(vx.z, __fmul_rn(alpha, vp.z));
      vx.w = __fadd_rn(vx.w, __fmul_rn(alpha, vp.w));
      st4(x, i, vx);
    }
    vr.x = __fsub_rn(vr.x, __fmul_rn(alpha, va.x));
    vr.y = __fsub_rn(vr.y, __fmul_rn(alpha, va.y));
    vr.z = __fsub_rn(vr.z, __fmul_rn(alpha, va.z));
    vr.w = __fsub_rn(vr.w, __fmul_rn(alpha, va.w));
    st4(r, i, vr);
    const float4 vz = zval4(vr, M, i);
    rr += (double)__fmul_rn(vr.x, vz.x) + (double)__fmul_rn(vr.y, vz.y) +
          (double)__fmul_rn(vr.z, vz.z) + (double)__fmul_rn(vr.w, vz.w);
    if (XUPD && part_obj) {
      const float4 vb = ld4(b, i);
      ob += (double)__fmul_rn(vx.x, __fadd_rn(vb.x, vr.x)) +
            (double)__fmul_rn(vx.y, __fadd_rn(vb.y, vr.y)) +
            (double)__fmul_rn(vx.z, __fadd_rn(vb.z, vr.z)) +
            (double)__fmul_rn(vx.w, __fadd_rn(vb.w, vr.w));
    }
  }
  for (size_t i = n4 * 4 + tid0; i < n; i += stride) {
    float vx = 0.f;
    if (XUPD) {
      vx = __fadd_rn(x[i], __fmul_rn(alpha, p[i]));
      x[i] = vx;
    }
    const float vr = __fsub_rn(r[i], __fmul_rn(alpha, ap[i]));
    r[i] = vr;
    rr += (double)__fmul_rn(vr, zval1(vr, M, i));
    if (XUPD && part_obj) ob += (double)__fmul_rn(vx, __fadd_rn(b[i], vr));
  }
  const double t = block_sum(rr);
  if (threadIdx.x == 0) part_rr[blockIdx.x] = t;
  if (XUPD && part_obj) {
    const double t2 = block_sum(ob);
    if (threadIdx.x == 0) part_obj[blockIdx.x] = t2;
  }
}

template <bool XUPD>
__global__ void __launch_bounds__(kBlock)
    k_update_p(const CgState *__restrict__ st, const float *__restrict__ r, float *__restrict__ p,
               size_t n, const float *__restrict__ M, float *__restrict__ x) {
  if (st->done) return;
  const float beta = (float)st->beta, alpha = (float)st->alpha;
  GRID_STRIDE_VEC4(n);
  for (size_t i = tid0; i < n4; i += stride) {
    const float4 vr = zval4(ld4(r, i), M, i);
    float4 vp = ld4(p, i);
    if (XUPD) {
      float4 vx = ld4_stream(x, i);
      vx.x = __fadd_rn(vx.x, __fmul_rn(alpha, vp.x));
      vx.y = __fadd_rn(vx.y, __fmul_rn(alpha, vp.y));
      vx.z = __fadd_rn(vx.z, __fmul_rn(alpha, vp.z));
      vx.w = __fadd_rn(vx.w, __fmul_rn(alpha, vp.w));
      st4_stream(x, i, vx);
    }
    vp.x = __fadd_rn(__fmul_rn(beta, vp.x), vr.x);
    vp.y = __fadd_rn(__fmul_rn(beta, vp.y), vr.y);
    vp.z = __fadd_rn(__fmul_rn(beta, vp.z), vr.z);
    vp.w = __fadd_rn(__fmul_rn(beta, vp.w), vr.w);
    st4(p, i, vp);
  }
  for (size_t i = n4 * 4 + tid0; i < n; i += stride) {
    const float vp = p[i];
    if (XUPD) x[i] = __fadd_rn(x[i], __fmul_rn(alpha, vp));
    p[i] = __fadd_rn(__fmul_rn(beta, vp), zval1(r[i], M, i));
  }
}


__global__ void __launch_bounds__(kBlock)
    k_update_p_ring(CgState *__restrict__ st, const float *__restrict__ r, const float *__restrict__ p_in,
                    float *__restrict__ p_out, int slot, size_t n, const float *__restrict__ M) {
  const int done = st->done;
  if (blockIdx.x == 0 && threadIdx.x == 0) st->ahist[slot] = st->alpha, st->committed[slot] = done ? 0 : 1;
  if (done) return;
  const float beta = (float)st->beta;
  GRID_STRIDE_VEC4(n);
  for (size_t i = tid0; i < n4; i += stride) {
    const float4 vz = zval4(ld4(r, i), M, i);
    float4 vp = ld4_stream(p_in, i);
    vp.x = __fadd_rn(__fmul_rn(beta, vp.x), vz.x);
    vp.y = __fadd_rn(__fmul_rn(beta, vp.y), vz.y);
    vp.z = __fadd_rn(__fmul_rn(beta, vp.z), vz.z);
    vp.w = __fadd_rn(__fmul_rn(beta, vp.w), vz.w);
    st4(p_out, i, vp);
  }
  for (size_t i = n4 * 4 + tid0; i < n; i += stride)
    p_out[i] = __fadd_rn(__fmul_rn(beta, p_in[i]), zval1(r[i], M, i));
}

template <bool PUPD>
__global__ void __launch_bounds__(kBlock)
    k_update_p_flush(CgState *__restrict__ st, const float *__restrict__ r, RingPtrs ring, int m, float *p_out,
                     size_t n, const float *__restrict__ M, float *__restrict__ x) {
  const int done = st->done;
  const float beta = PUPD ? (float)st->beta : 0.f;
  float a[kMaxRing];
  bool c[kMaxRing];
  bool any = false;
#pragma unroll
  for (int j = 0; j < kMaxRing; ++j) {
    c[j] = false, a[j] = 0.f;
    if (j < m - 1) c[j] = st->committed[j] != 0, a[j] = (float)st->ahist[j];
    if (j == m - 1) c[j] = !done, a[j] = (float)st->alpha;
    any = any || c[j];
  }
  if (!any) return;
  GRID_STRIDE_VEC4(n);
  for (size_t i = tid0; i < n4; i += stride) {
    float4 vz = make_float4(0.f, 0.f, 0.f, 0.f);
    if (PUPD && !done) vz = zval4(ld4(r, i), M, i);
    float4 vx = ld4_stream(x, i);
    float4 vp[kMaxRing];
#pragma unroll
    for (int j = 0; j < kMaxRing; ++j)
      if (c[j]) vp[j] = ld4_stream(ring.p[j], i);
#pragma unroll
    for (int j = 0; j < kMaxRing; ++j) {
      if (!c[j]) continue;
      vx.x = __fadd_rn(vx.x, __fmul_rn(a[j], vp[j].x));
      vx.y = __fadd_rn(vx.y, __fmul_rn(a[j], vp[j].y));
      vx.z = __fadd_rn(vx.z, __fmul_rn(a[j], vp[j].z));
      vx.w = __fadd_rn(vx.w, __fmul_rn(a[j], vp[j].w));
      if (PUPD && j == m - 1) {
        float4 b = vp[j];
        b.x = __fadd_rn(__fmul_rn(beta, b.x), vz.x);
        b.y = __fadd_rn(__fmul_rn(beta, b.y), vz.y);
        b.z = __fadd_rn(__fmul_rn(beta, b.z), vz.z);
        b.w = __fadd_rn(__fmul_rn(beta, b.w), vz.w);
        st4(p_out, i, b);
      }
    }
    st4_stream(x, i, vx);
  }
  for (size_t i = n4 * 4 + tid0; i < n; i += stride) {
    float vx = x[i], own = 0.f;
#pragma unroll
    for (int j = 0; j < kMaxRing; ++j) {
      if (!c[j]) continue;
      const float pj = ring.p[j][i];
      vx = __fadd_rn(vx, __fmul_rn(a[j], pj));
      if (j == m - 1) own = pj;
    }
    x[i] = vx;
    if (PUPD && !done) p_out[i] = __fadd_rn(__fmul_rn(beta, own), zval1(r[i], M, i));
  }
}

__global__ void __launch_bounds__(kBlock)
    k_update_x(const CgState *__restrict__ st, const float *__restrict__ p, size_t n, float *__restrict__ x) {
  if (st->done) return;
  const float alpha = (float)st->alpha;
  GRID_STRIDE_VEC4(n);
  for (size_t i = tid0; i < n4; i += stride) {
    const float4 vp = ld4_stream(p, i);
    float4 vx = ld4_stream(x, i);
    vx.x = __fadd_rn(vx.x, __fmul_rn(alpha, vp.x));
    vx.y = __fadd_rn(vx.y, __fmul_rn(alpha, vp.y));
    vx.z = __fadd_rn(vx.z, __fmul_rn(alpha, vp.z));
    vx.w = __fadd_rn(vx.w, __fmul_rn(alpha, vp.w));
    st4_stream(x, i, vx);
  }
  for (size_t i = n4 * 4 + tid0; i < n; i += stride) x[i] = __fadd_rn(x[i], __fmul_rn(alpha, p[i]));
}

__global__ void __launch_bounds__(kBlock)
    k_axpy(float a, const float *__restrict__ x, float *__restrict__ y, size_t n) {
  const size_t stride = (size_t)gridDim.x * blockDim.x;
  for (size_t i = (size_t)blockIdx.x * blockDim.x + threadIdx.x; i < n; i += stride)
    y[i] = fmaf(a, x[i], y[i]);
}

__device__ __forceinline__ double sum_partials(const double *part, int g) {
  double v = 0.0;
  int i = threadIdx.x;
  for (; i + 7 * kBlock < g; i += 8 * kBlock) {
    double t[8];
#pragma unroll
    for (int u = 0; u < 8; ++u) t[u] = part[i + u * kBlock];
#pragma unroll
    for (int u = 0; u < 8; ++u) v += t[u];
  }
  for (; i < g; i += kBlock) v += part[i];
  return block_sum(v);
}

constexpr int kPartDeep = 16;
struct PartLoad {
  double t[kPartDeep];
};
__device__ __forceinline__ void part_issue(const double *part, int g, PartLoad &L) {
#pragma unroll
  for (int u = 0; u < kPartDeep; ++u) {
    const int i = min((int)threadIdx.x + u * kBlock, max(g - 1, 0));
    L.t[u] = part[i];
  }
}
__device__ __forceinline__ double part_finish(const double *part, int g, const PartLoad &L) {
  double v = 0.0;
#pragma unroll
  for (int u = 0; u < kPartDeep; ++u)
    if ((int)threadIdx.x + u * kBlock < g) v += L.t[u];
  for (int i = (int)threadIdx.x + kPartDeep * kBlock; i < g; i += kBlock) v += part[i];
  return block_sum(v);
}

__device__ __forceinline__ void publish(const CgState *st, unsigned long long *hostw) {
  if (hostw)
    __hip_atomic_store(hostw, cg_progress_word(st->gen, st->done, st->iters), __ATOMIC_RELAXED,
                       __HIP_MEMORY_SCOPE_SYSTEM);
}

__device__ __forceinline__ void record_obj(CgState *st, int k, double obj, double tol) {
  constexpr int kRing = kMaxCgIter + 1;
  const double prev = k > 0 ? st->obj[(k - 1) % kRing] : 0.0;
  st->obj[k % kRing] = obj;
  if (k == 0) {
    st->obj_max = obj;
    st->obj_min = obj;
    return;
  }
  st->obj_max = fmax(st->obj_max, obj);
  st->obj_min = fmin(st->obj_min, obj);
  const double gain = (prev - obj) / (st->obj_max - st->obj_min);
  if (fabs(gain) < tol) st->done = 1;
  if (!isfinite(obj)) st->done = 1;
}

__global__ void __launch_bounds__(kBlock)
    k_sc_init(CgState *st, const double *part_rr, const double *part_obj, int g, int mode,
              int check, unsigned long long *hostw) {
  const double rr = sum_partials(part_rr, g);
  double ob = 0.0;
  if (check && mode != UNIRES_STOP_RESIDUAL) ob = sum_partials(part_obj, g);
  if (threadIdx.x == 0) {
    st->rz = rr;
    st->rzpp[0] = rr;
    st->rzpp[1] = rr;
    st->done = 0;
    st->iters = 0;
    st->alpha = 0.0;
    st->beta = 0.0;
    st->gen += 1u;
    if (check) record_obj(st, 0, mode == UNIRES_STOP_RESIDUAL ? sqrt(rr) : 0.5 * ob, 0.0);
    st->skip_fresh = 1, st->fresh_prev_ok = 1, st->rec_prev = 0.5 * ob, st->fresh_prev = 0.5 * ob, st->gain_rec = 0.0;
    publish(st, hostw);
  }
}

__global__ void __launch_bounds__(kBlock) k_sc_alpha(CgState *st, const double *part_pap, int g, int iters_end) {
  PartLoad L;
  part_issue(part_pap, g, L);
  const int done = st->done;
  const double rz = st->rz;
  const double pap = part_finish(part_pap, g, L);
  if (threadIdx.x == 0 && !done) {
    st->pAp = pap;
    st->alpha = rz / pap;
    if (iters_end > 0) st->iters = iters_end;
  }
}

__global__ void __launch_bounds__(kBlock)
    k_sc_beta(CgState *st, const double *part_rr, const double *part_obj, int g, int k,
              int obj_kind, double tol, unsigned long long *hostw) {
  PartLoad Lr, Lo;
  part_issue(part_rr, g, Lr);
  if (obj_kind == 2) part_issue(part_obj, g, Lo);
  const int done = st->done, iters = st->iters;
  const double rz0 = st->rz;
  if (k < 0) k = iters + 1;
  const double rr = part_finish(part_rr, g, Lr);
  double ob = 0.0;
  if (obj_kind == 2) ob = part_finish(part_obj, g, Lo);
  if (threadIdx.x == 0 && !done) {
    st->rz = rr;
    st->rzpp[k & 1] = rr;
    st->beta = rr / rz0;
    st->iters = k;
    if (obj_kind == 1) record_obj(st, k, sqrt(rr), tol);
    if (obj_kind == 2) record_obj(st, k, -0.5 * ob, tol);
    publish(st, hostw);
  }
}

__global__ void __launch_bounds__(kBlock)
    k_sc_obj(CgState *st, const double *part_obj, int g, int k, double tol, unsigned long long *hostw) {
  PartLoad L;
  part_issue(part_obj, g, L);
  const int done = st->done, iters = st->iters;
  if (k < 0) k = iters;
  const double ob = part_finish(part_obj, g, L);
  if (threadIdx.x == 0 && !done) {
    record_obj(st, k, 0.5 * ob, tol);
    publish(st, hostw);
  }
}

constexpr double kGuardHi = 4.0, kGuardLo = 0.5, kGuardNear = 1.5;
__global__ void __launch_bounds__(kBlock)
    k_sc_beta_guarded(CgState *st, const double *part_rr, const double *part_obj, int g, int k, double tol,
                      unsigned long long *hostw) {
  PartLoad Lr, Lo;
  part_issue(part_rr, g, Lr);
  part_issue(part_obj, g, Lo);
  const int done = st->done, iters = st->iters;
  const double rz0 = st->rz;
  if (k < 0) k = iters + 1;
  const double rr = part_finish(part_rr, g, Lr);
  const double ob = part_finish(part_obj, g, Lo);
  if (threadIdx.x == 0 && !done) {
    constexpr int kRing = kMaxCgIter + 1;
    st->rz = rr;
    st->rzpp[k & 1] = rr;
    st->beta = rr / rz0;
    st->iters = k;
    const double rec = -0.5 * ob;
    st->obj[k % kRing] = rec;
    st->obj_max = fmax(st->obj_max, rec);
    st->obj_min = fmin(st->obj_min, rec);
    const double gain = (st->rec_prev - rec) / (st->obj_max - st->obj_min);
    const double gain_before = fabs(st->gain_rec);
    st->gain_rec = gain;
    st->rec_prev = rec;
    double hi = kGuardHi;
    if (gain_before > 0.0 && isfinite(gain_before) && isfinite(gain)) {
      const double rho = fabs(gain) / gain_before;
      hi = fmin(kGuardHi, fmax(kGuardNear, kGuardNear / fmax(rho, 1e-6)));
    }
    const bool far = fabs(gain) >= hi * tol;
    const bool under = fabs(gain) < kGuardLo * tol;
    st->skip_fresh = (far || under) ? 1 : 0;
    if (far) st->fresh_prev_ok = 0;
    if (under) st->done = 1;
    if (!isfinite(rec)) st->done = 1, st->skip_fresh = 1;
    publish(st, hostw);
  }
}

__global__ void __launch_bounds__(kBlock)
    k_sc_obj_guarded(CgState *st, const double *part_obj, int g, int k, double tol, unsigned long long *hostw) {
  PartLoad L;
  part_issue(part_obj, g, L);
  const int done = st->done, skip = st->skip_fresh, iters = st->iters;
  if (k < 0) k = iters;
  const double ob = part_finish(part_obj, g, L);
  if (threadIdx.x == 0 && !done && !skip) {
    constexpr int kRing = kMaxCgIter + 1;
    const double fresh = 0.5 * ob;
    st->obj[k % kRing] = fresh;
    st->obj_max = fmax(st->obj_max, fresh);
    st->obj_min = fmin(st->obj_min, fresh);
    const double gain = st->fresh_prev_ok ? (st->fresh_prev - fresh) / (st->obj_max - st->obj_min) : st->gain_rec;
    st->fresh_prev = fresh, st->fresh_prev_ok = 1;
    if (fabs(gain) < tol || !isfinite(fresh)) st->done = 1, st->skip_fresh = 1;
    publish(st, hostw);
  }
}

__global__ void __launch_bounds__(kBlock) k_sum_to(const double *part, int g, double *out) {
  const double v = sum_partials(part, g);
  if (threadIdx.x == 0) *out = v;
}

int vec_num_blocks(size_t n) { return vec_blocks(n); }

void launch_residual_init(const float *b, const float *ax, const float *x, float *r, float *p,
                          size_t n, double *part_rr, double *part_obj, const float *M,
                          hipStream_t st) {
  hipLaunchKernelGGL(k_residual_init, dim3(vec_blocks(n)), dim3(kBlock), 0, st, b, ax, x, r, p, n,
                     part_rr, part_obj, M);
}
void launch_dot(const float *a, const float *b, size_t n, double *part, const int *done,
                hipStream_t st) {
  hipLaunchKernelGGL(k_dot, dim3(vec_blocks(n)), dim3(kBlock), 0, st, a, b, n, part, done);
}
void launch_update_xr(const CgState *s, const float *p, const float *ap, float *x, float *r,
                      const float *b, size_t n, double *part_rr, double *part_obj,
                      const float *M, hipStream_t st) {
  if (x)
    hipLaunchKernelGGL(k_update_xr<true>, dim3(vec_blocks(n)), dim3(kBlock), 0, st, s, p, ap, x, r, b,
                       n, part_rr, part_obj, M);
  else
    hipLaunchKernelGGL(k_update_xr<false>, dim3(vec_blocks(n)), dim3(kBlock), 0, st, s, p, ap, x, r,
                       b, n, part_rr, part_obj, M);
}
void launch_update_p(const CgState *s, const float *r, float *p, size_t n, const float *M, float *x,
                     hipStream_t st) {
  if (x)
    hipLaunchKernelGGL(k_update_p<true>, dim3(vec_blocks(n)), dim3(kBlock), 0, st, s, r, p, n, M, x);
  else
    hipLaunchKernelGGL(k_update_p<false>, dim3(vec_blocks(n)), dim3(kBlock), 0, st, s, r, p, n, M, x);
}
void launch_update_p_ring(CgState *s, const float *r, const float *p_in, float *p_out, int slot, size_t n,
                          const float *M, hipStream_t st) {
  hipLaunchKernelGGL(k_update_p_ring, dim3(vec_blocks(n)), dim3(kBlock), 0, st, s, r, p_in, p_out, slot, n, M);
}
void launch_update_p_flush(CgState *s, const float *r, const RingPtrs &ring, int m, float *p_out, size_t n,
                           const float *M, float *x, hipStream_t st) {
  hipLaunchKernelGGL(k_update_p_flush<true>, dim3(vec_blocks(n)), dim3(kBlock), 0, st, s, r, ring, m, p_out, n, M, x);
}
void launch_update_x_flush(CgState *s, const RingPtrs &ring, int m, size_t n, float *x, hipStream_t st) {
  hipLaunchKernelGGL(k_update_p_flush<false>, dim3(vec_blocks(n)), dim3(kBlock), 0, st, s, (const float *)nullptr, ring, m,
                     (float *)nullptr, n, (const float *)nullptr, x);
}
void launch_update_x(const CgState *s, const float *p, size_t n, float *x, hipStream_t st) {
  hipLaunchKernelGGL(k_update_x, dim3(vec_blocks(n)), dim3(kBlock), 0, st, s, p, n, x);
}
__global__ void __launch_bounds__(kBlock) k_scale_shift(float a, float c, float *__restrict__ y, size_t n) {
  const size_t stride = (size_t)gridDim.x * blockDim.x;
  for (size_t i = (size_t)blockIdx.x * blockDim.x + threadIdx.x; i < n; i += stride)
    y[i] = __fadd_rn(__fmul_rn(a, y[i]), c);
}
void launch_scale_shift(float a, float c, float *y, size_t n, hipStream_t st) {
  hipLaunchKernelGGL(k_scale_shift, dim3(vec_blocks(n) * 4 > 4096 ? 4096 : vec_blocks(n) * 4),
                     dim3(kBlock), 0, st, a, c, y, n);
}
__global__ void __launch_bounds__(kBlock) k_fill(float v, float *__restrict__ y, size_t n) {
  const size_t stride = (size_t)gridDim.x * blockDim.x;
  for (size_t i = (size_t)blockIdx.x * blockDim.x + threadIdx.x; i < n; i += stride) y[i] = v;
}
void launch_fill(float v, float *y, size_t n, hipStream_t st) {
  hipLaunchKernelGGL(k_fill, dim3(vec_blocks(n) * 4 > 4096 ? 4096 : vec_blocks(n) * 4), dim3(kBlock), 0,
                     st, v, y, n);
}
__global__ void __launch_bounds__(kBlock)
    k_divide(const float *__restrict__ a, const float *__restrict__ m, float *__restrict__ y, size_t n) {
  const size_t stride = (size_t)gridDim.x * blockDim.x;
  for (size_t i = (size_t)blockIdx.x * blockDim.x + threadIdx.x; i < n; i += stride)
    y[i] = __fdiv_rn(a[i], m[i]);
}
void launch_div(const float *a, const float *m, float *y, size_t n, hipStream_t st) {
  hipLaunchKernelGGL(k_divide, dim3(vec_blocks(n) * 4 > 4096 ? 4096 : vec_blocks(n) * 4), dim3(kBlock), 0,
                     st, a, m, y, n);
}
void launch_axpy(float a, const float *x, float *y, size_t n, hipStream_t st) {
  hipLaunchKernelGGL(k_axpy, dim3(vec_blocks(n) * 4 > 4096 ? 4096 : vec_blocks(n) * 4),
                     dim3(kBlock), 0, st, a, x, y, n);
}
void launch_sc_init(CgState *s, const double *part_rr, const double *part_obj, int g, int mode,
                    int check, unsigned long long *hostw, hipStream_t st) {
  hipLaunchKernelGGL(k_sc_init, dim3(1), dim3(kBlock), 0, st, s, part_rr, part_obj, g, mode,
                     check, hostw);
}
void launch_sc_alpha(CgState *s, const double *part, int g, hipStream_t st, int iters_end) {
  hipLaunchKernelGGL(k_sc_alpha, dim3(1), dim3(kBlock), 0, st, s, part, g, iters_end);
}
void launch_sc_beta(CgState *s, const double *part_rr, const double *part_obj, int g, int k,
                    int obj_kind, double tol, unsigned long long *hostw, hipStream_t st) {
  hipLaunchKernelGGL(k_sc_beta, dim3(1), dim3(kBlock), 0, st, s, part_rr, part_obj, g, k,
                     obj_kind, tol, hostw);
}
void launch_sc_obj(CgState *s, const double *part, int g, int k, double tol, unsigned long long *hostw,
                   hipStream_t st) {
  hipLaunchKernelGGL(k_sc_obj, dim3(1), dim3(kBlock), 0, st, s, part, g, k, tol, hostw);
}
void launch_sc_beta_guarded(CgState *s, const double *part_rr, const double *part_obj, int g, int k, double tol,
                            unsigned long long *hostw, hipStream_t st) {
  hipLaunchKernelGGL(k_sc_beta_guarded, dim3(1), dim3(kBlock), 0, st, s, part_rr, part_obj, g, k, tol, hostw);
}
void launch_sc_obj_guarded(CgState *s, const double *part, int g, int k, double tol, unsigned long long *hostw,
                           hipStream_t st) {
  hipLaunchKernelGGL(k_sc_obj_guarded, dim3(1), dim3(kBlock), 0, st, s, part, g, k, tol, hostw);
}
void launch_sum_to(const double *part, int g, double *out, hipStream_t st) {
  hipLaunchKernelGGL(k_sum_to, dim3(1), dim3(kBlock), 0, st, part, g, out);
}

}
```

unires_amd/csrc/cg.hpp:

```cpp
#pragma once
#include "common.hpp"

namespace unires {

constexpr int kMaxCgIter = 4096;
constexpr int kMaxRing = 8;

struct CgState {
  double rz, pAp, alpha, beta, obj_max, obj_min;
  int done, iters;
  unsigned gen, pad_;
  double rzpp[2];
  double obj[kMaxCgIter + 1];
  int skip_fresh;
  int fresh_prev_ok;
  double rec_prev, fresh_prev, gain_rec;
  double ahist[kMaxRing];
  int committed[kMaxRing];
};
struct RingPtrs {
  const float *p[kMaxRing];
};

__host__ __device__ inline unsigned long long cg_progress_word(unsigned gen, int done, int iters) {
  return ((unsigned long long)gen << 32) | (done ? 0x80000000ull : 0ull) | (unsigned)(iters & 0x7fffffff);
}

int vec_num_blocks(size_t n);
void launch_residual_init(const float *b, const float *ax, const float *x, float *r, float *p,
                          size_t n, double *part_rr, double *part_obj, const float *M,
                          hipStream_t st);
void launch_dot(const float *a, const float *b, size_t n, double *part, const int *done,
                hipStream_t st);
void launch_update_xr(const CgState *s, const float *p, const float *ap, float *x, float *r,
                      const float *b, size_t n, double *part_rr, double *part_obj, const float *M,
                      hipStream_t st);
void launch_update_p(const CgState *s, const float *r, float *p, size_t n, const float *M, float *x,
                     hipStream_t st);
void launch_update_p_ring(CgState *s, const float *r, const float *p_in, float *p_out, int slot, size_t n,
                          const float *M, hipStream_t st);
void launch_update_p_flush(CgState *s, const float *r, const RingPtrs &ring, int m, float *p_out, size_t n,
                           const float *M, float *x, hipStream_t st);
void launch_update_x_flush(CgState *s, const RingPtrs &ring, int m, size_t n, float *x, hipStream_t st);
void launch_update_x(const CgState *s, const float *p, size_t n, float *x, hipStream_t st);
void launch_scale_shift(float a, float c, float *y, size_t n, hipStream_t st);
void launch_fill(float v, float *y, size_t n, hipStream_t st);
void launch_div(const float *a, const float *m, float *y, size_t n, hipStream_t st);
void launch_axpy(float a, const float *x, float *y, size_t n, hipStream_t st);
void launch_sc_init(CgState *s, const double *part_rr, const double *part_obj, int g, int mode,
                    int check, unsigned long long *hostw, hipStream_t st);
void launch_sc_alpha(CgState *s, const double *part, int g, hipStream_t st, int iters_end = 0);
void launch_sc_beta(CgState *s, const double *part_rr, const double *part_obj, int g, int k,
                    int obj_kind, double tol, unsigned long long *hostw, hipStream_t st);
void launch_sc_obj(CgState *s, const double *part, int g, int k, double tol, unsigned long long *hostw,
                   hipStream_t st);
void launch_sc_beta_guarded(CgState *s, const double *part_rr, const double *part_obj, int g, int k, double tol,
                            unsigned long long *hostw, hipStream_t st);
void launch_sc_obj_guarded(CgState *s, const double *part, int g, int k, double tol, unsigned long long *hostw,
                           hipStream_t st);
void launch_sum_to(const double *part, int g, double *out, hipStream_t st);

}
```

unires_amd/csrc/splat2.hip:

```cpp
#include "splat2.hpp"

#include <math.h>
#include <stdio.h>
#include <stdlib.h>
#include <string.h>

#include <algorithm>
#include <type_traits>
#include <map>
#include <mutex>
#include <utility>
#include <vector>

namespace unires {

struct S2Tile {
  static constexpr int TX = 8, TY = 4, TZ = 30, L = 32;
  static constexpr int SX = TX + 2, SY = TY + 2, SZ = TZ + 2, N = SX * SY * SZ;
  static constexpr int XS = SY * SZ, YS = SZ;
};
constexpr int kS2Waves = 4;
constexpr int kS2MaxSeg = 8;

#define S2_FENCE() asm volatile("" ::: "memory")
// ... 814 lines not shown
      switch ((hw_slot + round) & 3) {
        case 0: __builtin_amdgcn_s_setprio(0); break;
        case 1: __builtin_amdgcn_s_setprio(1); break;
        case 2: __builtin_amdgcn_s_setprio(2); break;
        default: __builtin_amdgcn_s_setprio(3); break;
      }
    }
    const int x0 = (int)(rec.x & 1023u) * TX, y0 = (int)((rec.x >> 10) & 1023u) * TY, z0 = (int)(rec.x >> 20) * T::TZ;
    const int ex = min(TX, dd.x - x0), ey = min(TY, dd.y - y0), ez = min(T::TZ, dd.z - z0);
    const int ninstr = AXIS == 2 ? ((int)(rec.w & 0xffu) + kS2Batch - 1) / kS2Batch * kS2Batch : (int)(rec.w & 0xffu);
    const int tab_base = (int)(rec.w >> 8);
    const unsigned ent0 = rec.y;
    const uint4 *E = reinterpret_cast<const uint4 *>(P.entries) + ent0;
    const int t_next = t + slots;
    const u4v rec_next = t_next < t_hi ? recs[t_next] : rec_none;
    int lp = lane;
    asm volatile("" : "+v"(lp));
    const ulonglong2 mymask = h_mk;
    const int mlo_v = (int)(unsigned)mymask.x, mhi_v = (int)(unsigned)(mymask.x >> 32);
    const int alo_v = (int)(unsigned)mymask.y, ahi_v = (int)(unsigned)(mymask.y >> 32);
    const int bw_v = (int)h_bw;
    if (AXIS == 2)
      asm volatile("" ::"v"(mlo_v), "v"(mhi_v), "v"(alo_v), "v"(ahi_v), "v"(bw_v) : "memory");
    else
      asm volatile("" ::"v"(mlo_v), "v"(mhi_v), "v"(alo_v), "v"(ahi_v) : "memory");
    uint4 pre = make_uint4(0u, 0u, 0u, 0u);
    if (lp < 32) pre = E[64 + lp];
    if (CONV) {
      const unsigned step4 = (AXIS == 2 || AXIS == 3) ? 4u : P.tab_step4;
      const float4 raw = tabs[lp];
      tabs[lp] = make_float4((float)(tab_base + lp), __int_as_float((int)(step4 * (unsigned)__float_as_int(raw.x))),
                             P.alpha * raw.y, P.alpha * raw.z);
    }
#ifdef UNIRES_S2_PROF
    asm volatile("s_waitcnt vmcnt(0) lgkmcnt(0)" ::: "memory");
    if (pw && lane == 0 && ptile < 5) pw[3 + 5 * ptile] = wall_clock64();
#endif
    const uint4 *X = reinterpret_cast<const uint4 *>(P.ext) + 2 * (size_t)ent0;
    uint4 pre2 = make_uint4(0u, 0u, 0u, 0u);
    if (AXIS == 3) {
      ring2[lane] = X[lane], ring2[kWave + lane] = X[kWave + lane];
      pre2 = X[2 * kWave + lane];
    }
    {
      int lz = lane;
      float zr = 0.f;
      asm volatile("" : "+v"(lz), "+v"(zr));
      for (int i = lz; i < N / 4; i += kWave) reinterpret_cast<float4 *>(acc)[i] = make_float4(zr, zr, zr, zr);
    }
    typedef __attribute__((address_space(3))) float *LdsF1;
    unsigned acc_addr = (unsigned)(__UINTPTR_TYPE__)(LdsF1)(void *)acc - 4u * (unsigned)(((x0 - 1) * SY + (y0 - 1)) * SZ + (z0 - 1));
    asm volatile("" : "+s"(acc_addr));
    int chunk_lo = 0;
    int eb = 0;
    S2_FENCE();
    constexpr int kU = kS2Batch;
    struct Batch {
      float w0[kU], w1[kU], s0[kU], s1[kU], gx[kU], gy[kU], gz[kU];
      unsigned long long amask[kU];
    };
    auto advance = [&](unsigned bw) {
      if (bw & kS2BatchAdv) {
        S2_FENCE();
        if (lane < 32) ring[(chunk_lo & 1) * 32 + lane] = pre;
        if (AXIS == 3) ring2[(chunk_lo & 1) * 64 + lane] = pre2;
        ++chunk_lo;
        int la = lane;
        asm volatile("" : "+v"(la));
        if (la < 32) pre = E[32 * (chunk_lo + 2) + la];
        if (AXIS == 3) pre2 = X[64 * (chunk_lo + 2) + lane];
        S2_FENCE();
      }
    };
    auto load = [&](Batch &Bt, int u, int sl) {
      {
        const u4r e = *(LdsU4)(__UINTPTR_TYPE__)((((unsigned)sl << 4) & m3f0) | ring_b);
        const float rx = __uint_as_float(e.x), ry = __uint_as_float(e.y), rz = __uint_as_float(e.z);
        float kf;
        const unsigned code = e.w & kS2RowIdle;
        const int k = (int)(e.w >> kS2RowBits) + lane_m64;
        kf = (float)k;
        Bt.w0[u] = P.alpha, Bt.w1[u] = 0.f, Bt.s0[u] = 1.f, Bt.s1[u] = 0.f;
        if (S2_ABL(8)) {
        } else if (AXIS == 3) {
          const uint4 xa = ring2[2 * (sl & 63)], xb = ring2[2 * (sl & 63) + 1];
          const f4r tb = *(LdsF4)(__UINTPTR_TYPE__)((((unsigned)k << 4) & m3f0) | tabs_b);
          const unsigned a = xa.x + (unsigned)__float_as_int(tb.y);
          const uint2 p00 = __builtin_bit_cast(uint2, __builtin_amdgcn_raw_buffer_load_b64(rsrc, a, 0, 0));
          const uint2 p01 = __builtin_bit_cast(uint2, __builtin_amdgcn_raw_buffer_load_b64(rsrc, a + P.xs_sy4, 0, 0));
          const uint2 p10 = __builtin_bit_cast(uint2, __builtin_amdgcn_raw_buffer_load_b64(rsrc, a + P.xs_sx4, 0, 0));
          const uint2 p11 =
              __builtin_bit_cast(uint2, __builtin_amdgcn_raw_buffer_load_b64(rsrc, a + P.xs_sx4 + P.xs_sy4, 0, 0));
          const float z00 = tb.z * __uint_as_float(p00.x) + tb.w * __uint_as_float(p00.y);
          const float z01 = tb.z * __uint_as_float(p01.x) + tb.w * __uint_as_float(p01.y);
          const float z10 = tb.z * __uint_as_float(p10.x) + tb.w * __uint_as_float(p10.y);
          const float z11 = tb.z * __uint_as_float(p11.x) + tb.w * __uint_as_float(p11.y);
          Bt.w0[u] = 1.f;
          kf = tb.x;
          Bt.s0[u] = __uint_as_float(xa.y) * z00 + __uint_as_float(xa.z) * z01 + __uint_as_float(xa.w) * z10 +
                     __uint_as_float(xb.x) * z11;
          (void)code;
        } else if (AXIS == 2) {
          const f4r tb = *(LdsF4)(__UINTPTR_TYPE__)((((unsigned)k << 4) & m3f0) | tabs_b);
          kf = tb.x;
          const unsigned a = __umul24(code, P.row_stride4) + (unsigned)__float_as_int(tb.y);
          const uint2 pr = __builtin_bit_cast(uint2, __builtin_amdgcn_raw_buffer_load_b64(rsrc, a, 0, 0));
          Bt.w0[u] = tb.z, Bt.w1[u] = tb.w, Bt.s0[u] = __uint_as_float(pr.x), Bt.s1[u] = __uint_as_float(pr.y);
        } else if (AXIS == 0 || AXIS == 1) {
          const unsigned ui = code >> 9, uj = code & 511u;
          const float4 tb = tabs[((int)(AXIS == 0 ? ui : uj) - tab_base) & 63];
          const unsigned a = __umul24(AXIS == 0 ? uj : ui, P.row_stride4) + (unsigned)__float_as_int(tb.y) +
                             4u * (unsigned)k;
          Bt.w0[u] = tb.z, Bt.w1[u] = tb.w;
          Bt.s0[u] = buf_load(rsrc, a, 0), Bt.s1[u] = buf_load(rsrc, a + P.tab_step4, 0);
        } else {
          Bt.s0[u] = buf_load(rsrc, __umul24(code, P.row_stride4) + 4u * (unsigned)k, 0);
        }
#ifndef UNIRES_S2_NO_PKXY
        {
          typedef float v2f __attribute__((ext_vector_type(2)));
          const v2f cxy = {c0, c1}, txy = {t0, t1}, rxy = {rx, ry}, kk = {kf, kf};
          const v2f gxy = __builtin_elementwise_fma(cxy, kk, rxy) + txy;
          Bt.gx[u] = gxy.x, Bt.gy[u] = gxy.y;
        }
#else
        Bt.gx[u] = fmaf(c0, kf, rx) + t0;
        Bt.gy[u] = fmaf(c1, kf, ry) + t1;
#endif
        Bt.gz[u] = fmaf(c2, kf, rz) + t2;
      }
    };
    auto fetch = [&](Batch &Bt, int p0, unsigned bw) {
#pragma unroll
      for (int u = 0; u < kU; ++u) {
        const int pi = p0 + u;
        const unsigned mlo = (unsigned)__builtin_amdgcn_readlane(mlo_v, pi), mhi = (unsigned)__builtin_amdgcn_readlane(mhi_v, pi);
        Bt.amask[u] = ((unsigned long long)(unsigned)__builtin_amdgcn_readlane(ahi_v, pi) << 32) |
                      (unsigned)__builtin_amdgcn_readlane(alo_v, pi);
        load(Bt, u, (int)((bw >> (6 * u)) & 63u) + (int)__builtin_amdgcn_mbcnt_hi(mhi, __builtin_amdgcn_mbcnt_lo(mlo, 0u)));
      }
    };
    auto fetch_run = [&](Batch &Bt, int p0) {
      unsigned mlo[kU], mhi[kU];
      int ebu[kU];
      int need = eb;
#pragma unroll
      for (int u = 0; u < kU; ++u) {
        const int pi = min(p0 + u, ninstr - 1);
        mlo[u] = (unsigned)__builtin_amdgcn_readlane(mlo_v, pi);
        mhi[u] = (unsigned)__builtin_amdgcn_readlane(mhi_v, pi);
        Bt.amask[u] = p0 + u < ninstr ? ((unsigned long long)(unsigned)__builtin_amdgcn_readlane(ahi_v, pi) << 32) |
                                            (unsigned)__builtin_amdgcn_readlane(alo_v, pi)
                                      : 0ull;
        ebu[u] = (p0 + u < ninstr || u == 0) ? need : ebu[u > 0 ? u - 1 : 0];
        if (p0 + u < ninstr) need += __popc(mlo[u]) + __popc(mhi[u]) + 1;
      }
      advance(need > 32 * (chunk_lo + 2) ? kS2BatchAdv : 0u);
      eb = need;
#pragma unroll
      for (int u = 0; u < kU; ++u)
        load(Bt, u, ebu[u] + (int)__builtin_amdgcn_mbcnt_hi(mhi[u], __builtin_amdgcn_mbcnt_lo(mlo[u], 0u)));
    };
    auto splat = [&](const Batch &Bt, auto second_tag) {
      constexpr bool SECOND = decltype(second_tag)::value;
#pragma unroll
      for (int u = 0; u < kU; ++u) {
        const float gx = Bt.gx[u], gy = Bt.gy[u], gz = Bt.gz[u];
#ifndef UNIRES_S2_NO_PKW
        typedef float v2f __attribute__((ext_vector_type(2)));
        const float fx = floorf(gx), fy = floorf(gy), fz = floorf(gz);
        const v2f gxy = {gx, gy}, fxy = {fx, fy};
        const v2f w1 = gxy - fxy;
        const float wz1 = gz - fz, wz0 = 1.f - wz1;
        const v2f m11 = {-1.f, 1.f}, one0 = k_one0;
        const v2f wx = __builtin_elementwise_fma(m11, (v2f){w1.x, w1.x}, one0);
        const v2f wy = __builtin_elementwise_fma(m11, (v2f){w1.y, w1.y}, one0);
        const float cf = fmaf(fx, (float)XS, fmaf(fy, (float)YS, fz));
        const int cell = (int)cf;
        float v;
        if (AXIS < 0 || AXIS == 3)
          v = Bt.w0[u] * Bt.s0[u] + Bt.w1[u] * Bt.s1[u];
        else if (!SECOND && u > 0)
          v = fmaf(Bt.w0[u], Bt.s0[u], Bt.w1[u] * Bt.s1[u]);
        else
          v = fmaf(Bt.w1[u], Bt.s1[u], Bt.w0[u] * Bt.s0[u]);
        const v2f vx = (v2f){v, v} * wx;
        const v2f a0 = (v2f){vx.x, vx.x} * wy, a1 = (v2f){vx.y, vx.y} * wy;
        S2_FENCE();
        if (S2_ABL(4)) dot += (double)(a0.x + a0.y + a1.x + a1.y + (float)cell);
        if (__builtin_amdgcn_inverse_ballot_w64(Bt.amask[u]) && !S2_ABL(4)) {
          const LdsF1 q = (LdsF1)(__UINTPTR_TYPE__)(acc_addr + 4u * (unsigned)cell);
          {
            const v2f o0 = {q[0], q[YS]}, o1 = {q[XS], q[XS + YS]};
            const v2f r0 = __builtin_elementwise_fma(a0, (v2f){wz0, wz0}, o0), r1 = __builtin_elementwise_fma(a1, (v2f){wz0, wz0}, o1);
            q[0] = r0.x, q[YS] = r0.y, q[XS] = r1.x, q[XS + YS] = r1.y;
          }
          S2_FENCE();
          {
            const v2f o0 = {q[1], q[YS + 1]}, o1 = {q[XS + 1], q[XS + YS + 1]};
            const v2f r0 = __builtin_elementwise_fma(a0, (v2f){wz1, wz1}, o0), r1 = __builtin_elementwise_fma(a1, (v2f){wz1, wz1}, o1);
            q[1] = r0.x, q[YS + 1] = r0.y, q[XS + 1] = r1.x, q[XS + YS + 1] = r1.y;
          }
        }
#else
        const float fx = floorf(gx), fy = floorf(gy), fz = floorf(gz);
        const float wx1 = gx - fx, wy1 = gy - fy, wz1 = gz - fz;
        const float wx0 = 1.f - wx1, wy0 = 1.f - wy1, wz0 = 1.f - wz1;
        const float cf = fmaf(fx, (float)XS, fmaf(fy, (float)YS, fz));
        const int cell = (int)cf;
        const float v = Bt.w0[u] * Bt.s0[u] + Bt.w1[u] * Bt.s1[u];
        const float vx0 = v * wx0, vx1 = v * wx1;
        const float a00 = vx0 * wy0, a01 = vx0 * wy1, a10 = vx1 * wy0, a11 = vx1 * wy1;
        S2_FENCE();
        if (S2_ABL(4)) dot += (double)(a00 + a01 + a10 + a11 + (float)cell);
        if (__builtin_amdgcn_inverse_ballot_w64(Bt.amask[u]) && !S2_ABL(4)) {
          const LdsF1 q = (LdsF1)(__UINTPTR_TYPE__)(acc_addr + 4u * (unsigned)cell);
          {
            const float o00 = q[0], o01 = q[YS], o10 = q[XS], o11 = q[XS + YS];
            q[0] = o00 + a00 * wz0, q[YS] = o01 + a01 * wz0, q[XS] = o10 + a10 * wz0,
            q[XS + YS] = o11 + a11 * wz0;
          }
          S2_FENCE();
#ifdef S2_EXP_MASKB
          if ((lane & (S2_EXP_MASKB - 1)) == 0)
#endif
          {
            const float o00 = q[1], o01 = q[YS + 1], o10 = q[XS + 1], o11 = q[XS + YS + 1];
            q[1] = o00 + a00 * wz1, q[YS + 1] = o01 + a01 * wz1, q[XS + 1] = o10 + a10 * wz1,
            q[XS + YS + 1] = o11 + a11 * wz1;
          }
        }
#endif
        S2_FENCE();
      }
    };
    if (ninstr > 0 && !S2_ABL(1)) {
      Batch ba, bb;
      auto step = [&](Batch &Bt, int p0) {
        if (AXIS == 2) {
          const unsigned bw = (unsigned)__builtin_amdgcn_readlane(bw_v, p0 / kU);
          advance(bw);
          fetch(Bt, p0, bw);
        } else {
          fetch_run(Bt, p0);
        }
      };
      step(ba, 0);
      for (int p0 = 0; p0 < ninstr; p0 += 2 * kU) {
        const bool more = p0 + kU < ninstr;
        if (more) step(bb, p0 + kU);
        splat(ba, std::false_type{});
        if (more) {
          if (p0 + 2 * kU < ninstr) step(ba, p0 + 2 * kU);
          splat(bb, std::true_type{});
        }
      }
    }
    S2_FENCE();
#ifdef UNIRES_S2_PROF
    if (pw && lane == 0 && ptile < 5) pw[4 + 5 * ptile] = wall_clock64(), pw[7 + 5 * ptile] = (unsigned long long)ninstr;
#endif
    const KArgs K = kargs();
    const Hdr H = load_hdr(K);
    const float *__restrict__ pin = K->p;
    float *__restrict__ dst = K->dst;
    const float *objb = OBJK ? K->objb : nullptr;
    const int accumulate = K->accumulate;
    const float kcx = K->cx, kcy = K->cy, kcz = K->cz, ka0 = K->a0;
    asm volatile("" ::"s"(H.entries), "s"(H.ent_bytes), "s"(H.tab), "s"(H.gn), "s"(H.masks), "s"(H.bwords), "s"(pin), "s"(dst), "s"(objb),
                 "s"(accumulate), "s"(kcx), "s"(kcy), "s"(kcz), "s"(ka0));
    float *res_r = OBJK ? K->res_r : nullptr, *res_p = OBJK ? K->res_p : nullptr;
    const float *res_M = OBJK ? K->res_M : nullptr;
    const bool res_obj = OBJK && K->partials2 != nullptr;
    if (OBJK) asm volatile("" ::"s"(res_r), "s"(res_p), "s"(res_M));
    {
      asm volatile("" ::"v"(pre.x), "v"(pre.y), "v"(pre.z), "v"(pre.w));
      if (AXIS == 3) asm volatile("" ::"v"(pre2.x), "v"(pre2.y), "v"(pre2.z), "v"(pre2.w));
      int lh = lane;
      asm volatile("" : "+v"(lh));
      if (rec_next.x != 0xffffffffu) issue_header(H, rec_next, lh);
    }
    double dtile = 0.0;
    double dtile2 = 0.0;
    const bool fast_xy = !S2_ABL(2) && pin != nullptr && !accumulate && ex == TX && ey == TY && dd.numel() < (1ull << 29);
    if (fast_xy) {
      static_assert(TX == 8 && TY == 4 && G == 2, "epilogue register window is written for 8 x 4 tiles");
      int le = lane;
      asm volatile("" : "+v"(le));
      const int gl = le & (L - 1), grp = le / L;
      const int kz = z0 - 1 + gl;
      const bool out_z = gl >= 1 && gl <= ez;
      unsigned sxb = 4u * (unsigned)(dd.y * dd.z), syb = 4u * (unsigned)dd.z;
      asm volatile("" : "+s"(sxb), "+s"(syb));
      constexpr unsigned kOob = 0x80000000u;
      const int xg = x0 + 4 * grp;
      const unsigned e0 = 4u * (unsigned)((xg * dd.y + y0) * dd.z + max(kz, 0));
      const unsigned e1 = kz < dd.z ? e0 : kOob;
      const unsigned elo = xg > 0 ? e1 - sxb : e1, ehi = xg + 4 < dd.x ? e1 : kOob;
      const unsigned eyl = y0 > 0 ? e1 - syb : e1, eyh = y0 + TY < dd.y ? e1 : kOob;
      const unsigned est = out_z ? e0 : kOob;
      const __amdgpu_buffer_rsrc_t rp = make_rsrc(pin, dd.numel() * 4),
                                   rd = make_rsrc(dst, dd.numel() * 4),
                                   rb = make_rsrc(objb ? objb : pin, dd.numel() * 4);
      const __amdgpu_buffer_rsrc_t rrr = make_rsrc(res_r ? res_r : dst, dd.numel() * 4),
                                   rrp = make_rsrc(res_p ? res_p : dst, dd.numel() * 4),
                                   rm = make_rsrc(res_M ? res_M : pin, dd.numel() * 4);
      const float *arow = acc + ((4 * grp + 1) * SY + 1) * SZ + gl;
      float pv[6][6];
#pragma unroll
      for (int sa = 0; sa < 6; ++sa)
#pragma unroll
        for (int la = 0; la < 6; ++la) {
          const bool halo_x = sa == 0 || sa == 5, halo_y = la == 0 || la == 5;
          pv[sa][la] = (halo_x && halo_y) ? 0.f
                       : sa == 0 ? buf_load(rp, elo, (unsigned)(la - 1) * syb)
                       : sa == 5 ? buf_load(rp, ehi, 4u * sxb + (unsigned)(la - 1) * syb)
                       : la == 0 ? buf_load(rp, eyl, (unsigned)(sa - 1) * sxb)
                       : la == 5 ? buf_load(rp, eyh, (unsigned)(sa - 1) * sxb + 4u * syb)
                                 : buf_load(rp, e1, (unsigned)(sa - 1) * sxb + (unsigned)(la - 1) * syb);
        }
#ifdef UNIRES_S2_PROF
      asm volatile("s_waitcnt vmcnt(0)" ::: "memory");
      if (pw && lane == 0 && ptile < 5) pw[5 + 5 * ptile] = wall_clock64();
#endif
      auto rows = [&](auto obj_tag) {
        constexpr bool OBJ = decltype(obj_tag)::value;
        float dxp[4];
#pragma unroll
        for (int la = 1; la <= 4; ++la) dxp[la - 1] = pv[1][la] - pv[0][la];
        double dt = 0.0, dt2 = 0.0;
#pragma unroll
        for (int sa = 1; sa <= 4; ++sa) {
          float dy[5], av[4];
#pragma unroll
          for (int la = 1; la <= 4; ++la) av[la - 1] = arow[((sa - 1) * SY + (la - 1)) * SZ];
          float ob[4];
          if (OBJ) {
#pragma unroll
            for (int la = 1; la <= 4; ++la) ob[la - 1] = buf_load(rb, e1, (unsigned)(sa - 1) * sxb + (unsigned)(la - 1) * syb);
          }
          float om[4] = {1.f, 1.f, 1.f, 1.f};
          if (OBJ && res_M) {
#pragma unroll
            for (int la = 1; la <= 4; ++la) om[la - 1] = buf_load(rm, e1, (unsigned)(sa - 1) * sxb + (unsigned)(la - 1) * syb);
          }
#pragma unroll
          for (int la = 0; la <= 4; ++la) dy[la] = pv[sa][la + 1] - pv[sa][la];
#pragma unroll
          for (int la = 1; la <= 4; ++la) {
            const float c = pv[sa][la];
            const float vzp = __int_as_float(__builtin_amdgcn_update_dpp(0, __float_as_int(c), 0x130, 0xf, 0xf, true));
            const float zf = vzp - c;
            const float zbk = __int_as_float(__builtin_amdgcn_update_dpp(0, __float_as_int(zf), 0x138, 0xf, 0xf, true));
            const float xf = pv[sa + 1][la] - c, xbk = dxp[la - 1];
            dxp[la - 1] = xf;
            const float yf = dy[la], ybk = dy[la - 1];
            const float st = kcx * (xbk - xf) + kcy * (ybk - yf) + kcz * (zbk - zf);
            const float q = av[la - 1] + (ka0 * c + st);
            if (OBJ && res_r) {
              const float r = __fsub_rn(ob[la - 1], q);
              const float z = res_M ? __fdiv_rn(r, om[la - 1]) : r;
              buf_store(r, rrr, est, (unsigned)(sa - 1) * sxb + (unsigned)(la - 1) * syb);
              buf_store(z, rrp, est, (unsigned)(sa - 1) * sxb + (unsigned)(la - 1) * syb);
              dt += (double)__fmul_rn(r, z);
              if (res_obj) dt2 += (double)obj_term(q, ob[la - 1], c);
            } else if (OBJ) {
              dt += (double)obj_term(q, ob[la - 1], c);
            } else {
              buf_store(q, rd, est, (unsigned)(sa - 1) * sxb + (unsigned)(la - 1) * syb);
              dt += (double)__fmul_rn(c, q);
            }
          }
        }
        dtile = out_z ? dt : 0.0;
        if (OBJ) dtile2 = out_z ? dt2 : 0.0;
      };
      rows(std::integral_constant<bool, OBJK>{});
    } else if (!S2_ABL(2)) {
      int lg = lane;
      asm volatile("" : "+v"(lg));
      const int gl = lg & (L - 1), grp = lg / L;
#pragma unroll 2
      for (int r = grp; r < TX * TY; r += G) {
        const int lx = r / TY, ly = r % TY, lz = gl;
        if (lx >= ex || ly >= ey || lz >= ez) continue;
        const int i = x0 + lx, j = y0 + ly, k = z0 + lz;
        const size_t idx = ((size_t)i * dd.y + j) * dd.z + k;
        float q = acc[((lx + 1) * SY + ly + 1) * SZ + lz + 1];
        float pc = 0.f;
        if (pin) {
          const float st = dtd_at(pin, idx, i, j, k, dd, kcx, kcy, kcz, pc);
          q += ka0 * pc + st;
        }
        if (accumulate) q += dst[idx];
        if (OBJK && res_r) {
          const float r = __fsub_rn(objb[idx], q);
          const float z = res_M ? __fdiv_rn(r, res_M[idx]) : r;
          res_r[idx] = r, res_p[idx] = z;
          dtile += (double)__fmul_rn(r, z);
          if (res_obj) dtile2 += (double)obj_term(q, objb[idx], pc);
          continue;
        }
        matvec_emit(dst, idx, q, pc, objb, P.partials != nullptr, dtile);
      }
    }
#ifdef UNIRES_S2_PROF
    asm volatile("s_waitcnt vmcnt(0)" ::: "memory");
    if (pw && lane == 0 && ptile < 5) pw[6 + 5 * ptile] = wall_clock64();
    ++ptile;
#endif
    dot += dtile;
    if (OBJK) dot2 += dtile2;
    t = t_next, rec = rec_next;
  }
#ifdef UNIRES_S2_PROF
  if (pw && lane == 0) pw[1] = wall_clock64(), pw[2] = (unsigned long long)ptile;
#endif
  if (P.partials) {
    const double tot = wave_sum(dot);
    if (lane == 0) P.partials[blockIdx.x * NW + wave] = tot;
  }
  if (OBJK && P.partials2) {
    const double tot2 = wave_sum(dot2);
    if (lane == 0) P.partials2[blockIdx.x * NW + wave] = tot2;
  }
}

int splat2_blocks(Dim3i dd, int grid_cap) { return s2_grid(dd, grid_cap) * kS2Waves; }

static int s2_active(int axis, int grid) {
  static std::map<int, int> cache;
  static std::mutex mu;
  std::lock_guard<std::mutex> lock(mu);
  auto it = cache.find(axis);
  if (it == cache.end()) {
    int per_cu = 0, dev = 0, ncu = 0;
    const void *fn = axis == 0   ? (const void *)k_splat2<0, kS2Waves, false>
                     : axis == 1 ? (const void *)k_splat2<1, kS2Waves, false>
                     : axis == 2 ? (const void *)k_splat2<2, kS2Waves, false>
                     : axis == 3 ? (const void *)k_splat2<3, kS2Waves, false>
                                 : (const void *)k_splat2<-1, kS2Waves, false>;
    static const int force = getenv("UNIRES_SPLAT2_RESIDENT") ? atoi(getenv("UNIRES_SPLAT2_RESIDENT")) : 0;
    if (hipOccupancyMaxActiveBlocksPerMultiprocessor(&per_cu, fn, kWave * kS2Waves, 0) != hipSuccess) per_cu = 0;
    if (force > 0) per_cu = force;
    (void)hipGetDevice(&dev);
    if (hipDeviceGetAttribute(&ncu, hipDeviceAttributeMultiprocessorCount, dev) != hipSuccess) ncu = 0;
    const int n = per_cu > 0 && ncu > 0 ? per_cu * ncu : 1 << 30;
    it = cache.emplace(axis, n).first;
  }
  int n = std::min(grid, it->second);
  if (n >= 8) n -= n % 8;
  return n;
}

int launch_splat2(const SplatSched &S, const float *src, size_t src_numel, const float4 *tab_dev, int gn,
                  unsigned row_stride, unsigned tab_step, unsigned xs_sy, unsigned xs_sx, const Affine &A,
                  float alpha,
                  const PushEpilogue &ep, float *dst, Dim3i dd, const int *done, hipStream_t st) {
  if (!S.valid || S.ntiles != s2_ntiles(dd) || !S.recs || !S.bwords) return 1;
  if (S.axis >= 0 && (!tab_dev || gn < 1)) return 1;
  if (S.axis == 3 && !S.ext) return 1;
  if (src_numel >= (1ull << 30)) return 1;
  if ((unsigned long long)row_stride * 4ull >= (1ull << 24)) return 1;
  S2Args P;
  P.src = src;
  P.src_bytes = src_numel * sizeof(float);
  P.tab = tab_dev, P.gn = gn;
  P.row_stride4 = 4u * row_stride, P.tab_step4 = 4u * tab_step;
  P.entries = S.entries, P.ent_bytes = S.cap_entries * sizeof(S2Entry), P.ext = S.ext, P.xs_sy4 = 4u * xs_sy, P.xs_sx4 = 4u * xs_sx, P.masks = S.masks, P.bwords = S.bwords, P.recs = S.recs, P.ntiles = S.ntiles;
  P.A = A, P.alpha = alpha;
  P.p = ep.p, P.a0 = ep.a0, P.cx = ep.cx, P.cy = ep.cy, P.cz = ep.cz;
  P.dst = dst, P.dd = dd, P.accumulate = ep.accumulate, P.partials = ep.partials, P.objb = ep.objb;
  P.res_r = nullptr, P.res_p = nullptr, P.res_M = nullptr, P.partials2 = nullptr;
  if (ep.res_r) {
    if (!ep.res_b || !ep.res_p || !ep.partials || ep.objb) return 1;
    P.objb = ep.res_b, P.res_r = ep.res_r, P.res_p = ep.res_p, P.res_M = ep.res_M, P.partials2 = ep.res_obj;
  }
  static const int dbg = getenv("UNIRES_S2_DBG") ? atoi(getenv("UNIRES_S2_DBG")) : 0;
  P.dbg = dbg;
  const dim3 grid(s2_grid(dd, ep.grid_cap)), block(kWave * kS2Waves);
  P.active = s2_active(S.axis, (int)grid.x);
  if (std::min(8, P.active) != std::min(8, S.nwg) || (P.active >= 8 && P.active % 8)) return 1;
  for (int x = 0; x <= 8; ++x) P.xlo[x] = S.pos_lo[x];
  static const int prio_rot = getenv("UNIRES_S2_PRIO") ? atoi(getenv("UNIRES_S2_PRIO")) : 1;
  P.prio_rot = prio_rot;
  P.prof = nullptr;
#ifdef UNIRES_S2_PROF
  static unsigned long long *prof_dev = nullptr;
  const size_t nprof = (size_t)grid.x * kS2Waves * 32;
  if (!prof_dev) (void)hipMalloc((void **)&prof_dev, 4096 * 4 * 32 * sizeof(unsigned long long));
  (void)hipMemsetAsync(prof_dev, 0, nprof * sizeof(unsigned long long), st);
  P.prof = prof_dev;
#endif
#define S2_LAUNCH(AX)                                                                          \
  do {                                                                                         \
    if (P.objb)                                                                                \
      hipLaunchKernelGGL((k_splat2<AX, kS2Waves, true>), grid, block, 0, st, P, done);         \
    else                                                                                       \
      hipLaunchKernelGGL((k_splat2<AX, kS2Waves, false>), grid, block, 0, st, P, done);        \
  } while (0)
  switch (S.axis) {
    case 0: S2_LAUNCH(0); break;
    case 1: S2_LAUNCH(1); break;
    case 2: S2_LAUNCH(2); break;
    case 3: S2_LAUNCH(3); break;
    default: S2_LAUNCH(-1); break;
  }
#undef S2_LAUNCH
#ifdef UNIRES_S2_PROF
  {
    static int shots = 0;
    if (++shots == 12 && getenv("UNIRES_S2_PROF_OUT")) {
      std::vector<unsigned long long> h(nprof);
      (void)hipStreamSynchronize(st);
      (void)hipMemcpy(h.data(), prof_dev, nprof * sizeof(unsigned long long), hipMemcpyDeviceToHost);
      FILE *f = fopen(getenv("UNIRES_S2_PROF_OUT"), "w");
      for (size_t w = 0; w < nprof / 32; ++w) {
        for (int i = 0; i < 32; ++i) fprintf(f, "%llu ", h[w * 32 + i]);
        fprintf(f, "\n");
      }
      fclose(f);
    }
  }
#endif
  return 0;
}

}
```

Before: 5241 cg_iters/s.

## Add no-stop CG path for fixed-iteration solves and skip redundant residual copy

For fixed-iteration CG (tol=0, no FFT preconditioner), adds kernel variants that never read or reset the device 'done' flag: update_xr writes only the residual and partial dot (x stays lazy), and update_p_ring/flush/x skip the stop checks and early-outs. With the identity preconditioner, the fused start no longer writes r separately from p, since they are equal. The first iteration's residual update then reads p instead of r. This removes a memset, some loads and branches, and one full-vector store, at the cost of extra kernel variants and more coupling in plan state that graph replay must capture.

```diff
diff --git a/include/unires_hip.h b/include/unires_hip.h
--- a/include/unires_hip.h
+++ b/include/unires_hip.h
@@ -143,6 +143,7 @@
 int unires_plan_matvec_time(unires_plan_t *plan, int32_t *launches, double *total_us);
 int unires_plan_cg_ring(unires_plan_t *plan, int32_t k, int32_t *last);
 int unires_plan_cg_ends(unires_plan_t *plan, int32_t *trimmed, int32_t *start_fused);
+int unires_plan_cg_form(unires_plan_t *plan, int32_t *nostop, int32_t *start_one);
 
 int unires_proj_apply(unires_plan_t *plan, int32_t n, int32_t op, const float *in, float *out,
                       void *stream);
diff --git a/unires_amd/_lib.py b/unires_amd/_lib.py
--- a/unires_amd/_lib.py
+++ b/unires_amd/_lib.py
@@ -71,6 +71,7 @@
     'unires_plan_matvec_time': (C.c_int, [C.c_void_p, C.POINTER(C.c_int32), C.POINTER(C.c_double)]),
     'unires_plan_cg_ring': (C.c_int, [C.c_void_p, C.c_int32, C.POINTER(C.c_int32)]),
     'unires_plan_cg_ends': (C.c_int, [C.c_void_p, C.POINTER(C.c_int32), C.POINTER(C.c_int32)]),
+    'unires_plan_cg_form': (C.c_int, [C.c_void_p, C.POINTER(C.c_int32), C.POINTER(C.c_int32)]),
     'unires_proj_apply': (C.c_int, [C.c_void_p, C.c_int32, C.c_int32, C.c_void_p, C.c_void_p,
                                     C.c_void_p]),
     'unires_ata_matvec': (C.c_int, [C.c_void_p, C.c_float, C.c_float, C.c_void_p, C.c_void_p,
diff --git a/unires_amd/_plan.py b/unires_amd/_plan.py
--- a/unires_amd/_plan.py
+++ b/unires_amd/_plan.py
@@ -118,6 +118,11 @@
         last = C.c_int32(0)
         check(self.lib.unires_plan_cg_ring(self._h, int(k), C.byref(last)))
         return int(last.value)
+
+    def cg_form(self):
+        a, b = C.c_int32(-1), C.c_int32(-1)
+        check(self.lib.unires_plan_cg_form(self._h, C.byref(a), C.byref(b)))
+        return bool(a.value), bool(b.value)
 
     @on_device
     def matvec_time(self):
diff --git a/unires_amd/csrc/api_cg.hip b/unires_amd/csrc/api_cg.hip
--- a/unires_amd/csrc/api_cg.hip
+++ b/unires_amd/csrc/api_cg.hip
@@ -11,17 +11,30 @@
   return on;
 }
 
-static int cg_enqueue_start(unires_plan *pl, const CgSolve &s, unsigned long long *hostw, hipStream_t st) {
+static bool cg_nostop_on() {
+  static const bool on = !(getenv("UNIRES_CG_NOSTOP") && getenv("UNIRES_CG_NOSTOP")[0] == '0');
+  return on;
+}
+static bool cg_start_one_on() {
+  static const bool on = !(getenv("UNIRES_CG_START_ONE") && getenv("UNIRES_CG_START_ONE")[0] == '0');
+  return on;
+}
+
+static int cg_enqueue_start(unires_plan *pl, const CgSolve &s, unsigned long long *hostw, hipStream_t st,
+                            bool whole = false) {
   const size_t ny = pl->dy.numel();
   const bool check = s.tol != 0.0;
+  const bool nostop = cg_nostop_on() && whole && !check && !s.fft && s.max_iter > 0;
+  const bool one = nostop && cg_start_one_on() && !s.M;
   CgState *S = pl->state;
   const int gv = vec_num_blocks(ny);
-  HIP_TRY(hipMemsetAsync(&S->done, 0, sizeof(int), st));
+  if (!nostop) HIP_TRY(hipMemsetAsync(&S->done, 0, sizeof(int), st));
   const bool want_obj0 = check && s.stop != UNIRES_STOP_RESIDUAL;
-  StartResidual res = {s.b, pl->r, pl->p, s.M, pl->part0, want_obj0 ? pl->part1 : nullptr, false};
+  StartResidual res = {s.b, one ? nullptr : pl->r, pl->p, s.M, pl->part0, want_obj0 ? pl->part1 : nullptr, false};
   const bool ask = cg_start_fused_on() && !s.fft;
   int g0 = matvec(pl, s.rho, s.lam, s.x, pl->ap, nullptr, nullptr, st, nullptr, ask ? &res : nullptr);
   pl->last_fused = ask && res.served;
+  pl->last_start_one = one && ask && res.served;
   if (!(ask && res.served)) {
     launch_residual_init(s.b, pl->ap, s.x, pl->r, pl->p, ny, pl->part0, want_obj0 ? pl->part1 : nullptr, s.M, st);
     g0 = gv;
@@ -50,12 +63,16 @@
   const bool check = s.tol != 0.0;
   const int ring = s.ring;
   CgState *S = pl->state;
-  const int *done = &S->done;
   const int gv = vec_num_blocks(ny);
   if (ring > 1 && (check || s.fft || dev_k || ring > kMaxRing || ring - 1 > pl->ring_slots))
     return fail(UNIRES_ERR_ARG, "deferred iterate update outside its scope");
   const bool trim = cg_trim_on() && !check && !s.fft && !dev_k && k_first == 1 && count == s.max_iter;
   pl->last_trim = trim && count > 0;
+  const bool nostop = cg_nostop_on() && !check && !s.fft && !dev_k && k_first == 1 && count == s.max_iter && count > 0;
+  pl->last_nostop = nostop;
+  const bool start_one = nostop && pl->last_start_one;
+  if (!nostop) pl->last_start_one = 0;
+  const int *done = nostop ? nullptr : &S->done;
   RingPtrs rp = {};
   for (int j = 0; j < ring && ring > 1; ++j) rp.p[j] = ring_slot(pl, j);
   for (int k = k_first; k < k_first + count; ++k) {
@@ -90,14 +107,17 @@
     if (trim && k == k_first + count - 1) {
       launch_sc_alpha(S, pl->part0, g, st, k);
       if (ring > 1)
-        launch_update_x_flush(S, rp, slot + 1, ny, s.x, st);
+        launch_update_x_flush(S, rp, slot + 1, ny, s.x, st, !nostop);
       else
-        launch_update_x(S, p, ny, s.x, st);
+        launch_update_x(S, p, ny, s.x, st, !nostop);
       break;
     }
     launch_sc_alpha(S, pl->part0, g, st);
-    launch_update_xr(S, p, pl->ap, lazy_x ? nullptr : s.x, pl->r, s.b, ny, pl->part0,
-                     recur ? pl->part1 : nullptr, s.M, st);
+    if (nostop)
+      launch_update_xr_nostop(S, pl->ap, start_one && k == k_first ? p : pl->r, pl->r, ny, pl->part0, s.M, st);
+    else
+      launch_update_xr(S, p, pl->ap, lazy_x ? nullptr : s.x, pl->r, s.b, ny, pl->part0,
+                       recur ? pl->part1 : nullptr, s.M, st);
     if (s.fft) {
       if (fftpre_apply(pl->fft, pl->r, pl->fft.z, st)) return fail(UNIRES_ERR_HIP, "hipFFT execution failed");
       launch_dot(pl->r, pl->fft.z, ny, pl->part0, done, st);
@@ -107,9 +127,9 @@
     else
       launch_sc_beta(S, pl->part0, pl->part1, gv, kk, obj_kind, s.tol, obj_kind ? hostw : nullptr, st);
     if (ring > 1 && (slot == ring - 1 || k == k_first + count - 1))
-      launch_update_p_flush(S, pl->r, rp, slot + 1, ring_slot(pl, (slot + 1) % ring), ny, s.M, s.x, st);
+      launch_update_p_flush(S, pl->r, rp, slot + 1, ring_slot(pl, (slot + 1) % ring), ny, s.M, s.x, st, !nostop);
     else if (ring > 1)
-      launch_update_p_ring(S, pl->r, p, ring_slot(pl, slot + 1), slot, ny, s.M, st);
+      launch_update_p_ring(S, pl->r, p, ring_slot(pl, slot + 1), slot, ny, s.M, st, !nostop);
     else
       launch_update_p(S, s.fft ? pl->fft.z : pl->r, pl->p, ny, s.M, lazy_x ? s.x : nullptr, st);
     if (check && s.stop == UNIRES_STOP_MAXGAIN) {
@@ -125,7 +145,7 @@
 }
 
 static int cg_enqueue(unires_plan *pl, const CgSolve &s, hipStream_t st) {
-  const int rc = cg_enqueue_start(pl, s, nullptr, st);
+  const int rc = cg_enqueue_start(pl, s, nullptr, st, true);
   if (rc) return rc;
   return cg_enqueue_iters(pl, s, 1, s.max_iter, false, nullptr, st);
 }
@@ -257,6 +277,7 @@
     }
   }
   pl->last_trim = 0;
+  pl->last_nostop = 0, pl->last_start_one = 0;
   if (R.use_graph) {
     pl->last_fused = pl->chunk_fused;
     HIP_TRY(hipGraphLaunch(pl->cg_start_exec, R.st));
@@ -269,6 +290,7 @@
   if (rc) return rc;
   if (R.enqueued >= R.s.max_iter) R.finished = true;
   pl->last_trim = 0;
+  pl->last_nostop = 0, pl->last_start_one = 0;
   return UNIRES_OK;
 }
 
@@ -418,6 +440,7 @@
   const bool graphable = cg_graphs_on() && !s.fft && max_iter > 0 && !pl->timing;
   if (graphable && pl->cg_exec && pl->cg_key.same_graph(s)) {
     pl->last_trim = pl->graph_trim, pl->last_fused = pl->graph_fused;
+    pl->last_nostop = pl->graph_nostop, pl->last_start_one = pl->graph_start_one;
     HIP_TRY(hipGraphLaunch(pl->cg_exec, st));
   } else {
     if (graphable && pl->cg_exec) drop_cg_graph(pl);
@@ -429,6 +452,7 @@
     if (rc == 0) {
       pl->cg_key = s;
       pl->graph_trim = pl->last_trim, pl->graph_fused = pl->last_fused;
+      pl->graph_nostop = pl->last_nostop, pl->graph_start_one = pl->last_start_one;
       if (hipGraphLaunch(pl->cg_exec, st) != hipSuccess) {
         cg_resync_gen(pl);
         return fail(UNIRES_ERR_HIP, "hipGraphLaunch failed");
diff --git a/unires_amd/csrc/api_internal.hpp b/unires_amd/csrc/api_internal.hpp
--- a/unires_amd/csrc/api_internal.hpp
+++ b/unires_amd/csrc/api_internal.hpp
@@ -182,6 +182,7 @@
   int ring_req = 0;
   int last_ring = 1;
   int last_trim = 0, last_fused = 0, graph_trim = 0, graph_fused = 0, chunk_fused = 0;
+  int last_nostop = 0, last_start_one = 0, graph_nostop = 0, graph_start_one = 0;
   unires::FftPre fft;
   float prec_rho = 0.f, prec_lam = 0.f;
   int prec_mode = UNIRES_PRECOND_IDENTITY;
diff --git a/unires_amd/csrc/api_operator.hip b/unires_amd/csrc/api_operator.hip
--- a/unires_amd/csrc/api_operator.hip
+++ b/unires_amd/csrc/api_operator.hip
@@ -103,7 +103,7 @@
 }
 
 static PushEpilogue without_residual(PushEpilogue ep) {
-  if (ep.res_r) ep.partials = nullptr;
+  if (ep.res_p) ep.partials = nullptr;
   ep.res_b = nullptr, ep.res_r = nullptr, ep.res_p = nullptr, ep.res_M = nullptr, ep.res_obj = nullptr;
   return ep;
 }
@@ -114,7 +114,7 @@
   const PushEpilogue ep = without_residual(ep_in);
   const PushEpilogue &ep2 = R.mid() ? ep : ep_in;
   const auto s2_done = [&] {
-    if (served) *served = ep2.res_r != nullptr;
+    if (served) *served = ep2.res_p != nullptr;
     return ep2.partials ? splat2_blocks(pl->dy, ep2.grid_cap) : 0;
   };
   if (served) *served = false;
diff --git a/unires_amd/csrc/api_plan.hip b/unires_amd/csrc/api_plan.hip
--- a/unires_amd/csrc/api_plan.hip
+++ b/unires_amd/csrc/api_plan.hip
@@ -474,6 +474,13 @@
   if (!plan) return fail(UNIRES_ERR_NULL, "null argument");
   if (trimmed) *trimmed = plan->last_trim;
   if (start_fused) *start_fused = plan->last_fused;
+  return UNIRES_OK;
+}
+
+extern "C" int unires_plan_cg_form(unires_plan_t *plan, int32_t *nostop, int32_t *start_one) {
+  if (!plan) return fail(UNIRES_ERR_NULL, "null argument");
+  if (nostop) *nostop = plan->last_nostop;
+  if (start_one) *start_one = plan->last_start_one;
   return UNIRES_OK;
 }
 
diff --git a/unires_amd/csrc/cg.hip b/unires_amd/csrc/cg.hip
--- a/unires_amd/csrc/cg.hip
+++ b/unires_amd/csrc/cg.hip
@@ -162,6 +162,39 @@
   }
 }
 
+__device__ __forceinline__ float late_scalar(double v) {
+  asm volatile("" : "+s"(v));
+  return (float)v;
+}
+
+__global__ void __launch_bounds__(kBlock)
+    k_update_xr_nostop(const CgState *__restrict__ st, const float *__restrict__ ap, const float *r_in, float *r_out,
+                       size_t n, double *__restrict__ part_rr, const float *__restrict__ M) {
+  const double alpha_d = st->alpha;
+  GRID_STRIDE_VEC4(n);
+  double rr = 0.0;
+  for (size_t i = tid0; i < n4; i += stride) {
+    const float4 va = ld4(ap, i);
+    float4 vr = ld4(r_in, i);
+    const float alpha = late_scalar(alpha_d);
+    vr.x = __fsub_rn(vr.x, __fmul_rn(alpha, va.x));
+    vr.y = __fsub_rn(vr.y, __fmul_rn(alpha, va.y));
+    vr.z = __fsub_rn(vr.z, __fmul_rn(alpha, va.z));
+    vr.w = __fsub_rn(vr.w, __fmul_rn(alpha, va.w));
+    st4(r_out, i, vr);
+    const float4 vz = zval4(vr, M, i);
+    rr += (double)__fmul_rn(vr.x, vz.x) + (double)__fmul_rn(vr.y, vz.y) +
+          (double)__fmul_rn(vr.z, vz.z) + (double)__fmul_rn(vr.w, vz.w);
+  }
+  for (size_t i = n4 * 4 + tid0; i < n; i += stride) {
+    const float vr = __fsub_rn(r_in[i], __fmul_rn((float)alpha_d, ap[i]));
+    r_out[i] = vr;
+    rr += (double)__fmul_rn(vr, zval1(vr, M, i));
+  }
+  const double t = block_sum(rr);
+  if (threadIdx.x == 0) part_rr[blockIdx.x] = t;
+}
+
 template <bool XUPD>
 __global__ void __launch_bounds__(kBlock)
     k_update_p(const CgState *__restrict__ st, const float *__restrict__ r, float *__restrict__ p,
@@ -215,11 +248,32 @@
     p_out[i] = __fadd_rn(__fmul_rn(beta, p_in[i]), zval1(r[i], M, i));
 }
 
-template <bool PUPD>
+__global__ void __launch_bounds__(kBlock)
+    k_update_p_ring_nostop(CgState *__restrict__ st, const float *__restrict__ r, const float *__restrict__ p_in,
+                           float *__restrict__ p_out, int slot, size_t n, const float *__restrict__ M) {
+  const double beta_d = st->beta;
+  GRID_STRIDE_VEC4(n);
+  for (size_t i = tid0; i < n4; i += stride) {
+    const float4 vz = zval4(ld4(r, i), M, i);
+    float4 vp = ld4_stream(p_in, i);
+    const float beta = late_scalar(beta_d);
+    vp.x = __fadd_rn(__fmul_rn(beta, vp.x), vz.x);
+    vp.y = __fadd_rn(__fmul_rn(beta, vp.y), vz.y);
+    vp.z = __fadd_rn(__fmul_rn(beta, vp.z), vz.z);
+    vp.w = __fadd_rn(__fmul_rn(beta, vp.w), vz.w);
+    st4(p_out, i, vp);
+  }
+  const float beta = (float)beta_d;
+  for (size_t i = n4 * 4 + tid0; i < n; i += stride)
+    p_out[i] = __fadd_rn(__fmul_rn(beta, p_in[i]), zval1(r[i], M, i));
+  if (blockIdx.x == 0 && threadIdx.x == 0) st->ahist[slot] = st->alpha, st->committed[slot] = 1;
+}
+
+template <bool PUPD, bool STOP>
 __global__ void __launch_bounds__(kBlock)
     k_update_p_flush(CgState *__restrict__ st, const float *__restrict__ r, RingPtrs ring, int m, float *p_out,
                      size_t n, const float *__restrict__ M, float *__restrict__ x) {
-  const int done = st->done;
+  const int done = STOP ? st->done : 0;
   const float beta = PUPD ? (float)st->beta : 0.f;
   float a[kMaxRing];
   bool c[kMaxRing];
@@ -231,7 +285,7 @@
     if (j == m - 1) c[j] = !done, a[j] = (float)st->alpha;
     any = any || c[j];
   }
-  if (!any) return;
+  if (STOP && !any) return;
   GRID_STRIDE_VEC4(n);
   for (size_t i = tid0; i < n4; i += stride) {
     float4 vz = make_float4(0.f, 0.f, 0.f, 0.f);
@@ -287,6 +341,24 @@
     vx.w = __fadd_rn(vx.w, __fmul_rn(alpha, vp.w));
     st4_stream(x, i, vx);
   }
+  for (size_t i = n4 * 4 + tid0; i < n; i += stride) x[i] = __fadd_rn(x[i], __fmul_rn(alpha, p[i]));
+}
+
+__global__ void __launch_bounds__(kBlock)
+    k_update_x_nostop(const CgState *__restrict__ st, const float *__restrict__ p, size_t n, float *__restrict__ x) {
+  const double alpha_d = st->alpha;
+  GRID_STRIDE_VEC4(n);
+  for (size_t i = tid0; i < n4; i += stride) {
+    const float4 vp = ld4_stream(p, i);
+    float4 vx = ld4_stream(x, i);
+    const float alpha = late_scalar(alpha_d);
+    vx.x = __fadd_rn(vx.x, __fmul_rn(alpha, vp.x));
+    vx.y = __fadd_rn(vx.y, __fmul_rn(alpha, vp.y));
+    vx.z = __fadd_rn(vx.z, __fmul_rn(alpha, vp.z));
+    vx.w = __fadd_rn(vx.w, __fmul_rn(alpha, vp.w));
+    st4_stream(x, i, vx);
+  }
+  const float alpha = (float)alpha_d;
   for (size_t i = n4 * 4 + tid0; i < n; i += stride) x[i] = __fadd_rn(x[i], __fmul_rn(alpha, p[i]));
 }
 
@@ -518,20 +590,37 @@
   else
     hipLaunchKernelGGL(k_update_p<false>, dim3(vec_blocks(n)), dim3(kBlock), 0, st, s, r, p, n, M, x);
 }
+void launch_update_xr_nostop(const CgState *s, const float *ap, const float *r_in, float *r_out, size_t n,
+                             double *part_rr, const float *M, hipStream_t st) {
+  hipLaunchKernelGGL(k_update_xr_nostop, dim3(vec_blocks(n)), dim3(kBlock), 0, st, s, ap, r_in, r_out, n, part_rr, M);
+}
 void launch_update_p_ring(CgState *s, const float *r, const float *p_in, float *p_out, int slot, size_t n,
-                          const float *M, hipStream_t st) {
-  hipLaunchKernelGGL(k_update_p_ring, dim3(vec_blocks(n)), dim3(kBlock), 0, st, s, r, p_in, p_out, slot, n, M);
+                          const float *M, hipStream_t st, bool stop) {
+  if (stop)
+    hipLaunchKernelGGL(k_update_p_ring, dim3(vec_blocks(n)), dim3(kBlock), 0, st, s, r, p_in, p_out, slot, n, M);
+  else
+    hipLaunchKernelGGL(k_update_p_ring_nostop, dim3(vec_blocks(n)), dim3(kBlock), 0, st, s, r, p_in, p_out, slot, n, M);
 }
 void launch_update_p_flush(CgState *s, const float *r, const RingPtrs &ring, int m, float *p_out, size_t n,
-                           const float *M, float *x, hipStream_t st) {
-  hipLaunchKernelGGL(k_update_p_flush<true>, dim3(vec_blocks(n)), dim3(kBlock), 0, st, s, r, ring, m, p_out, n, M, x);
-}
-void launch_update_x_flush(CgState *s, const RingPtrs &ring, int m, size_t n, float *x, hipStream_t st) {
-  hipLaunchKernelGGL(k_update_p_flush<false>, dim3(vec_blocks(n)), dim3(kBlock), 0, st, s, (const float *)nullptr, ring, m,
-                     (float *)nullptr, n, (const float *)nullptr, x);
-}
-void launch_update_x(const CgState *s, const float *p, size_t n, float *x, hipStream_t st) {
-  hipLaunchKernelGGL(k_update_x, dim3(vec_blocks(n)), dim3(kBlock), 0, st, s, p, n, x);
+                           const float *M, float *x, hipStream_t st, bool stop) {
+  if (stop)
+    hipLaunchKernelGGL((k_update_p_flush<true, true>), dim3(vec_blocks(n)), dim3(kBlock), 0, st, s, r, ring, m, p_out, n, M, x);
+  else
+    hipLaunchKernelGGL((k_update_p_flush<true, false>), dim3(vec_blocks(n)), dim3(kBlock), 0, st, s, r, ring, m, p_out, n, M, x);
+}
+void launch_update_x_flush(CgState *s, const RingPtrs &ring, int m, size_t n, float *x, hipStream_t st, bool stop) {
+  if (stop)
+    hipLaunchKernelGGL((k_update_p_flush<false, true>), dim3(vec_blocks(n)), dim3(kBlock), 0, st, s, (const float *)nullptr, ring,
+                       m, (float *)nullptr, n, (const float *)nullptr, x);
+  else
+    hipLaunchKernelGGL((k_update_p_flush<false, false>), dim3(vec_blocks(n)), dim3(kBlock), 0, st, s, (const float *)nullptr, ring,
+                       m, (float *)nullptr, n, (const float *)nullptr, x);
+}
+void launch_update_x(const CgState *s, const float *p, size_t n, float *x, hipStream_t st, bool stop) {
+  if (stop)
+    hipLaunchKernelGGL(k_update_x, dim3(vec_blocks(n)), dim3(kBlock), 0, st, s, p, n, x);
+  else
+    hipLaunchKernelGGL(k_update_x_nostop, dim3(vec_blocks(n)), dim3(kBlock), 0, st, s, p, n, x);
 }
 __global__ void __launch_bounds__(kBlock) k_scale_shift(float a, float c, float *__restrict__ y, size_t n) {
   const size_t stride = (size_t)gridDim.x * blockDim.x;
diff --git a/unires_amd/csrc/cg.hpp b/unires_amd/csrc/cg.hpp
--- a/unires_amd/csrc/cg.hpp
+++ b/unires_amd/csrc/cg.hpp
@@ -38,11 +38,13 @@
 void launch_update_p(const CgState *s, const float *r, float *p, size_t n, const float *M, float *x,
                      hipStream_t st);
 void launch_update_p_ring(CgState *s, const float *r, const float *p_in, float *p_out, int slot, size_t n,
-                          const float *M, hipStream_t st);
+                          const float *M, hipStream_t st, bool stop = true);
 void launch_update_p_flush(CgState *s, const float *r, const RingPtrs &ring, int m, float *p_out, size_t n,
-                           const float *M, float *x, hipStream_t st);
-void launch_update_x_flush(CgState *s, const RingPtrs &ring, int m, size_t n, float *x, hipStream_t st);
-void launch_update_x(const CgState *s, const float *p, size_t n, float *x, hipStream_t st);
+                           const float *M, float *x, hipStream_t st, bool stop = true);
+void launch_update_x_flush(CgState *s, const RingPtrs &ring, int m, size_t n, float *x, hipStream_t st, bool stop = true);
+void launch_update_x(const CgState *s, const float *p, size_t n, float *x, hipStream_t st, bool stop = true);
+void launch_update_xr_nostop(const CgState *s, const float *ap, const float *r_in, float *r_out, size_t n,
+                             double *part_rr, const float *M, hipStream_t st);
 void launch_scale_shift(float a, float c, float *y, size_t n, hipStream_t st);
 void launch_fill(float v, float *y, size_t n, hipStream_t st);
 void launch_div(const float *a, const float *m, float *y, size_t n, hipStream_t st);
diff --git a/unires_amd/csrc/splat2.hip b/unires_amd/csrc/splat2.hip
--- a/unires_amd/csrc/splat2.hip
+++ b/unires_amd/csrc/splat2.hip
@@ -1140,7 +1140,7 @@
       const __amdgpu_buffer_rsrc_t rp = make_rsrc(pin, dd.numel() * 4),
                                    rd = make_rsrc(dst, dd.numel() * 4),
                                    rb = make_rsrc(objb ? objb : pin, dd.numel() * 4);
-      const __amdgpu_buffer_rsrc_t rrr = make_rsrc(res_r ? res_r : dst, dd.numel() * 4),
+      const __amdgpu_buffer_rsrc_t rrr = make_rsrc(res_r ? res_r : dst, res_r ? dd.numel() * 4 : 0),
                                    rrp = make_rsrc(res_p ? res_p : dst, dd.numel() * 4),
                                    rm = make_rsrc(res_M ? res_M : pin, dd.numel() * 4);
       const float *arow = acc + ((4 * grp + 1) * SY + 1) * SZ + gl;
@@ -1195,7 +1195,7 @@
             const float yf = dy[la], ybk = dy[la - 1];
             const float st = kcx * (xbk - xf) + kcy * (ybk - yf) + kcz * (zbk - zf);
             const float q = av[la - 1] + (ka0 * c + st);
-            if (OBJ && res_r) {
+            if (OBJ && res_p) {
               const float r = __fsub_rn(ob[la - 1], q);
               const float z = res_M ? __fdiv_rn(r, om[la - 1]) : r;
               buf_store(r, rrr, est, (unsigned)(sa - 1) * sxb + (unsigned)(la - 1) * syb);
@@ -1231,10 +1231,11 @@
           q += ka0 * pc + st;
         }
         if (accumulate) q += dst[idx];
-        if (OBJK && res_r) {
+        if (OBJK && res_p) {
           const float r = __fsub_rn(objb[idx], q);
           const float z = res_M ? __fdiv_rn(r, res_M[idx]) : r;
-          res_r[idx] = r, res_p[idx] = z;
+          if (res_r) res_r[idx] = r;
+          res_p[idx] = z;
           dtile += (double)__fmul_rn(r, z);
           if (res_obj) dtile2 += (double)obj_term(q, objb[idx], pc);
           continue;
@@ -1310,8 +1311,8 @@
   P.p = ep.p, P.a0 = ep.a0, P.cx = ep.cx, P.cy = ep.cy, P.cz = ep.cz;
   P.dst = dst, P.dd = dd, P.accumulate = ep.accumulate, P.partials = ep.partials, P.objb = ep.objb;
   P.res_r = nullptr, P.res_p = nullptr, P.res_M = nullptr, P.partials2 = nullptr;
-  if (ep.res_r) {
-    if (!ep.res_b || !ep.res_p || !ep.partials || ep.objb) return 1;
+  if (ep.res_p) {
+    if (!ep.res_b || !ep.partials || ep.objb) return 1;
     P.objb = ep.res_b, P.res_r = ep.res_r, P.res_p = ep.res_p, P.res_M = ep.res_M, P.partials2 = ep.res_obj;
   }
   static const int dbg = getenv("UNIRES_S2_DBG") ? atoi(getenv("UNIRES_S2_DBG")) : 0;
```

New measurement: 5287 cg_iters/s, median of 6. About the same (+0.9%).
